# nv-tlabs/ASE

Measured on AMD Instinct MI355X. Metric: ASE PPO-update samples/sec (4096 envs x horizon 32), higher is better.
Workload: dtype f16; 1 GPU; BASELINE configs[1]: ASE agent, 4096 envs x horizon 32, obs 253 / act 31 / amp obs 1400 / latent 64, [1024,1024,512] MLPs + disc + shared-trunk encoder, minibatch 16384 (amp 4096) x 6 mini-epochs = 48 optimisation steps per update; random-init weights; precision_choice=auto without an oracle leg: the first candidate, replay=program, parallelism=single GPU

## Files before the change

### ase_amd/backend.py

```python
import ctypes as C

import torch

from . import lib as L


_HOSTFN = C.CFUNCTYPE(None, C.c_void_p)


def _ptr(t):
    return None if t is None else C.c_void_p(t.data_ptr())


def _ld(t):
    return 0 if t is None else int(t.stride(0))


def _code(dtype):
    if dtype == torch.bfloat16:
        return L.BF16
    if dtype == torch.float32:
        return L.F32
    if dtype == torch.float16:
        return L.F16
    raise L.AseHipError(f"unsupported storage dtype {dtype}")


class HipBackend:
    name = "hip"

    def __init__(self, device=None, x3=False):
        self.x3 = x3 if x3 == 'f16' else bool(x3)
        self._recording, self._host_keep, self._host_error = None, {}, None
        self.tn_workspace = True
        if not torch.cuda.is_available():
            raise L.AseHipError("HipBackend needs a ROCm GPU (torch.cuda.is_available() is False); "
                                "the update path has no CPU fallback")
        self.device = torch.device(device if device is not None else f"cuda:{torch.cuda.current_device()}")
        self.lib = L.get()
        self._head_scratch = torch.zeros(L.PPO_SCRATCH, dtype=torch.float64, device=self.device)
        self._head_scratch_ls = None

    def _stream(self):
        return C.c_void_p(torch.cuda.current_stream(self.device).cuda_stream)

    def zero_(self, t):
        assert t.is_contiguous()
        L.check(self.lib.ase_hip_memset(_ptr(t), 0, t.numel() * t.element_size(), self._stream()), "memset")

    def copy_(self, dst, src):
        assert dst.is_contiguous() and src.is_contiguous() and dst.dtype == src.dtype and dst.numel() == src.numel()
        L.check(self.lib.ase_hip_memcpy(_ptr(dst), _ptr(src), dst.numel() * dst.element_size(), self._stream()), "memcpy")

    def mark(self):
        ev = C.c_int(0)
        L.check(self.lib.ase_hip_mark(self._stream(), C.byref(ev)), "mark")
        return ev.value

    def wait(self, ev):
        L.check(self.lib.ase_hip_wait(self._stream(), int(ev)), "wait")

    def prog_create(self):
# ... 16 lines not shown
            return

        def trampoline(_arg, fn=fn):
            try:
                fn()
            except BaseException as e:
                self._host_error = e
        cb = _HOSTFN(trampoline)
        self._host_keep[self._recording].append(cb)
        L.check(self.lib.ase_hip_prog_host(C.cast(cb, C.c_void_p), None), "prog_host")

    def prog_launch(self, prog):
        L.check(self.lib.ase_hip_prog_launch(prog), "prog_launch")
        if self._host_error is not None:
            e, self._host_error = self._host_error, None
            raise e

    def prog_size(self, prog):
        return self.lib.ase_hip_prog_size(prog)

    def prog_destroy(self, prog):
        self.lib.ase_hip_prog_destroy(prog)
        self._host_keep.pop(prog.value, None)

    def _gemm_code(self, dtype, exps=None):
        c = _code(dtype)
        if self.x3 and c == L.F32:
            if self.x3 == 'f16' and exps is not None:
                return L.F32H3 | (int(exps[0]) << 8) | (int(exps[1]) << 16)
            return L.F32X3
        return c

    def gemm_nt(self, A, B, Cm, M, N, K, bias=None, aux=None, aux_mode=L.AUX_NONE, colsum=None, colsum_n=0,
                act=L.ACT_NONE, alpha=1.0, aux_split=0, aux_delta=0, mask_out=None, x3_exps=None, alpha_dev=None):
        dt = self._gemm_code(A.dtype, x3_exps)
        assert B.dtype == A.dtype
        if aux_mode == L.AUX_RELU_BITS:
            assert aux.dtype == torch.int32
        else:
            assert aux is None or aux.dtype == A.dtype
        assert mask_out is None or mask_out.dtype == (A.dtype if act >= L.ACT_SILU else torch.int32)
        out_f32 = int(Cm.dtype == torch.float32 and A.dtype != torch.float32)
        L.check(self.lib.ase_hip_gemm_nt(_ptr(A), _ld(A), _ptr(B), _ld(B), _ptr(Cm), _ld(Cm), _ptr(bias), _ptr(aux),
                                         _ld(aux), int(aux_split), int(aux_delta), _ptr(colsum), int(colsum_n),
                                         _ptr(mask_out), _ld(mask_out), M, N, K, act, aux_mode, out_f32,
                                         float(alpha), _ptr(alpha_dev), dt, self._stream()), "gemm_nt")

    def gemm_tn(self, A, B, G, M, N, K, n_real, k_real, split_src, split_dst, alpha=1.0, gbias=None, bias_rows=0, alpha_dev=None):
        L.check(self.lib.ase_hip_gemm_tn(_ptr(A), _ld(A), _ptr(B), _ld(B), _ptr(G), _ptr(gbias), int(bias_rows), M, N, K,
                                         n_real, k_real,
                                         split_src, split_dst, float(alpha), _ptr(alpha_dev), self._gemm_code(A.dtype), self._stream()),
                "gemm_tn")

    def grouped_tn_ok(self, dtype, M, n_real, K, bias_rows):
        return dtype in (torch.bfloat16, torch.float16) and M % 64 == 0 and bias_rows % 64 == 0

    def make_tn_plan(self, problems, target_wg=0, alpha_dev=None):
        import struct
        n = len(problems)
        tab = (C.c_int64 * (16 * n))()
        for i, (A, B, G, gb, br, M, N, K, nr, kr, ss, sd, alpha) in enumerate(problems):
            assert A.dtype in (torch.bfloat16, torch.float16) and B.dtype == A.dtype and G.dtype == torch.float32
            row = [A.data_ptr(), _ld(A), B.data_ptr(), _ld(B), G.data_ptr(), 0 if gb is None else gb.data_ptr(), int(br),
                   M, N, K, nr, kr, ss, sd, struct.unpack('<i', struct.pack('<f', float(alpha)))[0], 0]
            for j, v in enumerate(row):
                tab[16 * i + j] = int(v)
        max_work = 8192
        work = (C.c_int32 * (4 * max_work))()
        red = (C.c_int32 * (4 * max_work))()
        n_work, n_red = C.c_int(0), C.c_int(0)
        L.check(self.lib.ase_hip_gemm_tn_grouped_plan(tab, n, int(target_wg), work, max_work, C.byref(n_work), red, max_work,
                                                      C.byref(n_red)), "gemm_tn_grouped_plan")
        nw, nr = n_work.value, n_red.value
        dev_tab = torch.tensor(list(tab), dtype=torch.int64, device=self.device)
        dev_work = torch.tensor(list(work[:4 * nw]), dtype=torch.int32, device=self.device)
        dev_red = torch.tensor(list(red[:4 * nr]), dtype=torch.int32, device=self.device)
        ws = torch.empty(nw * L.TN_SLAB, dtype=torch.float32, device=self.device) if self.tn_workspace else None
        return {'problems': dev_tab, 'work': dev_work, 'n_work': nw, 'red': dev_red, 'n_red': nr, 'ws': ws, 'keep': problems,
                'dtype': _code(problems[0][0].dtype), 'alpha_dev': alpha_dev}

    def gemm_tn_grouped(self, plan):
        L.check(self.lib.ase_hip_gemm_tn_grouped(_ptr(plan['problems']), _ptr(plan['work']), plan['n_work'], _ptr(plan['red']),
                                                 plan['n_red'], _ptr(plan['ws']), _ptr(plan.get('alpha_dev')), plan['dtype'],
                                                 self._stream()),
                "gemm_tn_grouped")

    def refresh_shadow(self, W, Ws, Wts, split_src, split_dst, x3_exp=None):
        n, k = W.shape
        ref = Ws if Ws is not None else Wts
        code = _code(ref.dtype)
        if x3_exp is not None:
            assert ref.dtype == torch.float32
            code = L.F32H3 | (int(x3_exp) << 16)
        L.check(self.lib.ase_hip_refresh_shadow(_ptr(W), n, k, _ptr(Ws), _ld(Ws), _ptr(Wts), _ld(Wts), split_src,
                                                split_dst, code, self._stream()), "refresh_shadow")

    def refresh_shadow_multi(self, desc, items, dtype):
        L.check(self.lib.ase_hip_refresh_shadow_multi(_ptr(desc), desc.shape[0], _code(dtype), self._stream()),
                "refresh_shadow_multi")

    def apply_multi(self, desc, items, dtype, opt_state, acc):
        L.check(self.lib.ase_hip_apply_multi(_ptr(desc), desc.shape[0], _ptr(opt_state), _ptr(acc), _code(dtype),
                                             self._stream()), "apply_multi")

    def gather_multi(self, desc, items, idx, remap, M):
        L.check(self.lib.ase_hip_gather_multi(_ptr(desc), desc.shape[0], _ptr(idx), remap[0], remap[1], M,
                                              self._stream()), "gather_multi")

    def build_amp_obs(self, root_pos, root_rot, root_vel, root_ang_vel, dof_pos, dof_vel, key_body_pos, dof_offsets,
                      local_root_obs, root_height_obs, hist, shift=True):
        n, S, F = hist.shape
        offs = (C.c_int32 * len(dof_offsets))(*[int(x) for x in dof_offsets])
        for t in (root_pos, root_rot, root_vel, root_ang_vel, dof_pos, dof_vel, key_body_pos, hist):
            assert t.dtype == torch.float32 and t.is_contiguous()
        L.check(self.lib.ase_hip_build_amp_obs(_ptr(root_pos), _ptr(root_rot), _ptr(root_vel), _ptr(root_ang_vel), _ptr(dof_pos),
                                               _ptr(dof_vel), _ptr(key_body_pos), n, dof_pos.shape[1], key_body_pos.shape[1], offs,
                                               len(dof_offsets) - 1, int(local_root_obs), int(root_height_obs), _ptr(hist), S,
                                               int(shift), self._stream()), "build_amp_obs")

    def motion_state(self, clips, motion_ids, times):
        n, B = motion_ids.shape[0], clips['gts'].shape[1]
        D, J, K = clips['dof_offsets'][-1], len(clips['dof_body_ids']), len(clips['key_body_ids'])
        ia = lambda xs: (C.c_int32 * len(xs))(*[int(x) for x in xs])
        f = lambda *shape: torch.empty(*shape, dtype=torch.float32, device=self.device)
        out = (f(n, 3), f(n, 4), f(n, D), f(n, 3), f(n, 3), f(n, D), f(n, K, 3))
        assert motion_ids.dtype == torch.int32 and times.dtype == torch.float32
        L.check(self.lib.ase_hip_motion_state(_ptr(clips['gts']), _ptr(clips['grs']), _ptr(clips['lrs']), _ptr(clips['grvs']),
                                              _ptr(clips['gravs']), _ptr(clips['dvs']), B, _ptr(clips['lengths']),
                                              _ptr(clips['num_frames']), _ptr(clips['dt']), _ptr(clips['length_starts']),
                                              _ptr(motion_ids), _ptr(times), n, ia(clips['dof_body_ids']), ia(clips['dof_offsets']), J,
                                              ia(clips['key_body_ids']), K, *[_ptr(o) for o in out], self._stream()), "motion_state")
        return out

    def clip_frames(self, rotation, root_translation, root_velocity, root_angular_velocity, local_translation, parent_indices,
                    clip_first, clip_num_frames, clip_fps, frame_clip, dof_body_ids, dof_offsets, out=None):
        T, B = rotation.shape[0], rotation.shape[1]
# ... 116 lines not shown
                                           dof_pos.stride(1), _ptr(body_pos), _ptr(body_rot), _ptr(body_vel), _ptr(body_ang_vel), n,
                                           int(local_root_obs), int(root_height_obs), float(env_dt), _ptr(hist), S, self._stream()),
                "amp_reset")

    def rms_moments(self, src, D, idx, remap, M, state, sums):
        L.check(self.lib.ase_hip_rms_moments(_ptr(src), _ld(src), D, _ptr(idx), remap[0], remap[1], M, _ptr(state),
                                             _ptr(sums), self._stream()), "rms_moments")

    @staticmethod
    def _stream_arrays(streams):
        n = len(streams)
        srcs = (C.c_void_p * n)(*[s[0].data_ptr() for s in streams])
        lds = (C.c_int64 * n)(*[int(s[0].stride(0)) for s in streams])
        idxs = (C.c_void_p * n)(*[None if s[1] is None else s[1].data_ptr() for s in streams])
        rh = (C.c_int * n)(*[int(s[2][0]) for s in streams])
        rn = (C.c_int * n)(*[int(s[2][1]) for s in streams])
        return n, srcs, lds, idxs, rh, rn

    def rms_moments_multi(self, streams, D, M, state, sums_list):
        n, srcs, lds, idxs, rh, rn = self._stream_arrays(streams)
        sums = (C.c_void_p * n)(*[t.data_ptr() for t in sums_list])
        L.check(self.lib.ase_hip_rms_moments_multi(srcs, lds, idxs, rh, rn, sums, n, D, M, _ptr(state), self._stream()),
                "rms_moments_multi")

    def rms_normalize_multi(self, streams, D, M, means, stds, outs):
        n, srcs, lds, idxs, rh, rn = self._stream_arrays(streams)
        mp = (C.c_void_p * n)(*[t.data_ptr() for t in means])
        sp = (C.c_void_p * n)(*[t.data_ptr() for t in stds])
        op = (C.c_void_p * n)(*[t.data_ptr() for t in outs])
        lo = (C.c_int64 * n)(*[int(t.stride(0)) for t in outs])
        L.check(self.lib.ase_hip_rms_normalize_multi(srcs, lds, idxs, rh, rn, mp, sp, op, lo, n, D, M, _code(outs[0].dtype),
                                                     self._stream()), "rms_normalize_multi")

    def rms_finalize(self, state, D, sums, count, n_streams, mean_out, std_out):
        counts = (C.c_int32 * max(n_streams, 1))(*([int(count)] * max(n_streams, 1)))
        L.check(self.lib.ase_hip_rms_finalize(_ptr(state), D, _ptr(sums), counts, n_streams, _ptr(mean_out),
                                              _ptr(std_out), self._stream()), "rms_finalize")

    def rms_normalize(self, src, D, idx, remap, M, mean, std, outs):
        outs = list(outs) + [None] * (3 - len(outs))
        dt = _code(outs[0].dtype)
        L.check(self.lib.ase_hip_rms_normalize(_ptr(src), _ld(src), D, _ptr(idx), remap[0], remap[1], M, _ptr(mean),
                                               _ptr(std), _ptr(outs[0]), _ld(outs[0]), _ptr(outs[1]), _ld(outs[1]),
                                               _ptr(outs[2]), _ld(outs[2]), dt, self._stream()), "rms_normalize")

    def rms_unnormalize(self, state, x, y):
        L.check(self.lib.ase_hip_rms_unnormalize(_ptr(state), _ptr(x), _ptr(y), x.numel(), self._stream()),
                "rms_unnormalize")

    def gather_rows(self, src, D, idx, remap, M, dst):
        L.check(self.lib.ase_hip_gather_rows(_ptr(src), _ld(src), D, _ptr(idx), remap[0], remap[1], M, _ptr(dst),
                                             _ld(dst), _code(dst.dtype), self._stream()), "gather_rows")

    def reduce_sum(self, x, n, square, acc, slot):
        L.check(self.lib.ase_hip_reduce_sum(_ptr(x), n, int(square), _ptr(acc), slot, self._stream()), "reduce_sum")

    def ppo_head(self, mu, value, mb, new_z, logstd, d_mu, d_value, db_mu, db_value, acc, M, m_global, act_dim,
                 z_dim, masked, div_on, mu_tanh, clip_value, e_clip, critic_coef, bounds_coef, div_coef, div_tar,
                 mu_out=None, grad_scale=1.0, dyn=None, ls_mode=L.LS_FROZEN, d_logstd=None, db_logstd=None, entropy_coef=0.0):
        scratch = self._head_scratch if ls_mode == L.LS_FROZEN else self.reserve_learned_logstd()
        L.check(self.lib.ase_hip_ppo_head(
            _ptr(mu), _ld(mu), _ptr(value), _ld(value), _ptr(mb['actions']), _ptr(mb['mu']), _ptr(mb['sigma']),
            _ptr(mb['old_logp_actions']), _ptr(mb['advantages']), _ptr(mb.get('old_values')), _ptr(mb['returns']),
            _ptr(mb.get('rand_action_mask')), _ptr(mb.get('ase_latents')), _ptr(new_z), _ptr(logstd),
            _ptr(d_mu), _ld(d_mu), _ptr(d_value), _ld(d_value), _ptr(db_mu), _ptr(db_value), _ptr(mu_out), _ptr(acc),
            _ptr(scratch),
# ... 135 lines not shown
```

### ase_amd/csrc/common.h

```cpp
#pragma once
#include <hip/hip_runtime.h>
#include <hip/hip_bf16.h>
#include <stdint.h>
#include <stdio.h>
#include "../../include/ase_hip.h"
#include "prog.h"

typedef __bf16 bf16_t;
typedef __attribute__((ext_vector_type(8))) __bf16 bf16x8;
typedef __attribute__((ext_vector_type(4))) __bf16 bf16x4;
typedef _Float16 f16_t;
typedef __attribute__((ext_vector_type(8))) _Float16 f16x8;
typedef __attribute__((ext_vector_type(4))) _Float16 f16x4;
typedef __attribute__((ext_vector_type(16))) float f32x16;
typedef __attribute__((ext_vector_type(4))) float f32x4;

void ase_set_error(const char* fmt, ...);

#define ASE_CHECK_ARG(cond, ...)                 \
    do {                                         \
        if (!(cond)) {                           \
            ase_set_error(__VA_ARGS__);          \
            return ASE_EINVAL;                   \
        }                                        \
    } while (0)

#define ASE_CHECK_LAUNCH(name)                                              \
    do {                                                                    \
        hipError_t e__ = hipGetLastError();                                 \
        if (e__ != hipSuccess) {                                            \
            ase_set_error("%s: launch failed: %s", name, hipGetErrorString(e__)); \
            return ASE_ELAUNCH;                                             \
        }                                                                   \
    } while (0)

struct f32s_t { float v; };
struct f32h_t { float v; };

__device__ __forceinline__ float to_f32(float x) { return x; }
__device__ __forceinline__ float to_f32(bf16_t x) { return (float)x; }
__device__ __forceinline__ float to_f32(f32s_t x) { return x.v; }
__device__ __forceinline__ float to_f32(f32h_t x) { return x.v; }
__device__ __forceinline__ float to_f32(f16_t x) { return (float)x; }

template <typename T> __device__ __forceinline__ T from_f32(float x);
template <> __device__ __forceinline__ float from_f32<float>(float x) { return x; }
template <> __device__ __forceinline__ bf16_t from_f32<bf16_t>(float x) { return (bf16_t)x; }
template <> __device__ __forceinline__ f32s_t from_f32<f32s_t>(float x) { return f32s_t{x}; }
template <> __device__ __forceinline__ f32h_t from_f32<f32h_t>(float x) { return f32h_t{x}; }
template <> __device__ __forceinline__ f16_t from_f32<f16_t>(float x) { return (f16_t)__builtin_amdgcn_fmed3f(x, -65504.f, 65504.f); }

template <typename T> struct V16;
template <> struct V16<bf16_t> { typedef bf16x8 x8; typedef bf16x4 x4; };
template <> struct V16<f16_t> { typedef f16x8 x8; typedef f16x4 x4; };
template <> struct V16<float> { typedef bf16x8 x8; typedef bf16x4 x4; };
template <typename T> __device__ __forceinline__ f32x16 mfma16(typename V16<T>::x8 a, typename V16<T>::x8 b, f32x16 c);
template <> __device__ __forceinline__ f32x16 mfma16<bf16_t>(bf16x8 a, bf16x8 b, f32x16 c) {
    return __builtin_amdgcn_mfma_f32_32x32x16_bf16(a, b, c, 0, 0, 0);
}
template <> __device__ __forceinline__ f32x16 mfma16<f16_t>(f16x8 a, f16x8 b, f32x16 c) {
    return __builtin_amdgcn_mfma_f32_32x32x16_f16(a, b, c, 0, 0, 0);
}

template <typename T> struct StorageTag { typedef T type; };
template <typename F> inline int ase_dispatch_storage(int dtype, F&& f) {
    switch (dtype) {
        case ASE_F32: return f(StorageTag<float>{});
        case ASE_BF16: return f(StorageTag<bf16_t>{});
        case ASE_F16: return f(StorageTag<f16_t>{});
        default: return ASE_EUNSUPPORTED;
    }
}
inline int ase_elem_size(int dtype) { return (dtype == ASE_BF16 || dtype == ASE_F16) ? 2 : 4; }

__device__ __forceinline__ int64_t map_row(int r, const int32_t* __restrict__ idx, int remap_h, int remap_n) {
    uint32_t p = idx ? (uint32_t)idx[r] : (uint32_t)r;
    if (remap_h > 0) {
        const uint32_t env = p / (uint32_t)remap_h;
        const uint32_t t = p - env * (uint32_t)remap_h;
        p = t * (uint32_t)remap_n + env;
    }
    return (int64_t)p;
}
// ... 51 lines not shown
```

### ase_amd/csrc/gemm.hip

```cpp
#include "gemm_nt.h"
#include <math.h>

namespace ase_nt {

unsigned long long* g_nt_prof = nullptr;
int g_nt_prof_clk = 0;

int nt_choice(int M, int N, int K, int es, bool b16) {
    if (N <= 64) return 0;
    const int t256 = ((M + 255) / 256) * ((N + 255) / 256);
    const bool big = N % 256 == 0 && t256 >= 192 && (t256 <= 256 || t256 % 256 == 0 || t256 >= 1024);
    if (big) {
        if (!(b16 && (K * es) % 128 == 0)) return 3;
        const int t192 = ((M + 191) / 192) * (N / 256);
        return (t256 < 256 && t192 <= 256 && t192 > t256) ? 6 : 2;
    }
    if ((K * es) % 128 != 0) return 1;
    const int t128 = ((M + 127) / 128) * ((N + 127) / 128), t64x128 = ((M + 63) / 64) * ((N + 127) / 128);
    if (t128 >= 512) return 1;
    if (t64x128 >= 512) return 4;
    return 5;
}

}

using namespace ase_nt;

extern "C" int ase_hip_debug_nt_profile(void* buf) {
    g_nt_prof = reinterpret_cast<unsigned long long*>(buf);
    return ASE_OK;
}

extern "C" int ase_hip_debug_nt_profile_clock(int shader_clock) {
    g_nt_prof_clk = shader_clock ? 1 : 0;
    return ASE_OK;
}

extern "C" int ase_hip_gemm_nt_kernel_id(int M, int N, int K, int dtype) {
    dtype &= 0xFF;
    return nt_choice(M, N, K, ase_elem_size(dtype), ase_elem_size(dtype) == 2);
}

extern "C" int ase_hip_gemm_nt(const void* A, int64_t lda, const void* B, int64_t ldb, void* C, int64_t ldc,
                               const float* bias, const void* aux, int64_t ldaux, int aux_split, int aux_delta,
                               float* colsum, int colsum_n, void* mask_out, int64_t ldmask, int M, int N, int K, int act,
                               int aux_mode, int out_f32, float alpha, float* alpha_dev, int dtype_word, void* stream) {
    const int dtype = dtype_word & 0xFF, ea = (dtype_word >> 8) & 0xFF, eb = (dtype_word >> 16) & 0xFF;
    const int es = ase_elem_size(dtype);
    ASE_CHECK_ARG(dtype == ASE_F32 || dtype == ASE_BF16 || dtype == ASE_F32X3 || dtype == ASE_F16 || dtype == ASE_F32H3,
                  "gemm_nt: bad dtype %d", dtype);
    ASE_CHECK_ARG(ea >= 0 && ea <= 24 && eb >= 0 && eb <= 24 && (dtype == ASE_F32H3 || (ea | eb) == 0),
                  "gemm_nt: operand scale exponents (bits 8-15 / 16-23 of dtype) are 0..24 and belong to ASE_F32H3 only");
    ASE_CHECK_ARG(A && B && C && M > 0 && N > 0 && K > 0, "gemm_nt: null/empty operand (M=%d N=%d K=%d)", M, N, K);
    ASE_CHECK_ARG((K * es) % 64 == 0, "gemm_nt: K=%d is not a multiple of %d elements", K, 64 / es);
    ASE_CHECK_ARG(lda >= K && ldb >= K && ldc >= N, "gemm_nt: leading dimension too small");
    ASE_CHECK_ARG(((uintptr_t)A % 16) == 0 && ((uintptr_t)B % 16) == 0 && (lda * es) % 16 == 0 && (ldb * es) % 16 == 0,
                  "gemm_nt: A/B must be 16-byte aligned with 16-byte row pitch");
    ASE_CHECK_ARG(aux_mode == ASE_AUX_NONE || aux != nullptr, "gemm_nt: aux_mode %d without aux", aux_mode);
    const bool bits = aux_mode == ASE_AUX_RELU_BITS;
    ASE_CHECK_ARG(N % 4 == 0 && ((uintptr_t)C % 16) == 0 && (ldc * (out_f32 ? 4 : es)) % 8 == 0 &&
                      (aux == nullptr || bits || (((uintptr_t)aux % 8) == 0 && (ldaux * es) % 8 == 0)),
                  "gemm_nt: C / aux must allow 8/16-byte row-vector access (N %% 4 == 0, aligned pitches)");
    ASE_CHECK_ARG(!bits || (((uintptr_t)aux % 4) == 0 && ldaux * 32 >= N), "gemm_nt: bit mask needs ldaux >= N / 32 words");
    const bool smooth = act >= ASE_ACT_SILU;
    ASE_CHECK_ARG(act >= ASE_ACT_NONE && act <= ASE_ACT_SOFTPLUS, "gemm_nt: unknown activation %d", act);
    ASE_CHECK_ARG((aux_mode & 0xFF) <= ASE_AUX_PREACT && ((aux_mode & 0xFF) == ASE_AUX_PREACT || (aux_mode >> 8) == 0) &&
                      (aux_mode >> 8) <= ASE_ACT_SOFTPLUS, "gemm_nt: bad aux_mode 0x%x", aux_mode);
    ASE_CHECK_ARG(mask_out == nullptr || smooth || (N % 32 == 0 && ((uintptr_t)mask_out % 4) == 0 && ldmask * 32 >= N),
                  "gemm_nt: mask_out needs N %% 32 == 0 and ldmask >= N / 32 words");
    ASE_CHECK_ARG(mask_out == nullptr || !smooth || (ldmask >= N && ((uintptr_t)mask_out % 16) == 0 && (ldmask * es) % 8 == 0),
                  "gemm_nt: the pre-activation twin needs ldmask >= N elements, 16-byte alignment");
    NTParams p;
    p.A = (const char*)A; p.lda = lda * es;
    p.B = (const char*)B; p.ldb = ldb * es;
    p.C = (char*)C; p.ldc = ldc * (out_f32 ? 4 : es);
    p.mask_out = smooth ? nullptr : (uint32_t*)mask_out; p.ldmask = ldmask;
    p.pre_out = smooth ? (char*)mask_out : nullptr; p.ldpre = ldmask * es;
    p.bias = bias; p.aux = (const char*)aux; p.ldaux = bits ? ldaux * 4 : ldaux * es; p.aux_split = aux_split > 0 ? aux_split : M; p.aux_delta = aux_delta; p.colsum = colsum; p.colsum_n = colsum ? colsum_n : 0;
    p.M = M; p.N = N; p.K = K; p.act = act; p.aux_mode = aux_mode; p.out_f32 = out_f32; p.alpha = alpha; p.alpha_dev = alpha_dev;
    p.tiles_m = p.tiles_n = 0;
    p.prof = nullptr;
    p.prof_clk = 0;
    p.sa = 1.f;
    if (dtype == ASE_BF16) return dispatch_nt_bf16(p, (hipStream_t)stream);
    if (dtype == ASE_F16) return dispatch_nt_f16(p, (hipStream_t)stream);
    if (dtype == ASE_F32X3) return dispatch_nt_x3(p, (hipStream_t)stream);
    if (dtype == ASE_F32H3) {
        p.sa = ldexpf(1.f, ea);
        p.alpha = ldexpf(alpha, -(ea + eb));
        return dispatch_nt_h3(p, (hipStream_t)stream);
    }
    return dispatch_nt_f32(p, (hipStream_t)stream);
}
```

### ase_amd/csrc/gemm_nt.h

```cpp
#pragma once
#include "common.h"
#include "act.h"
#include <type_traits>

namespace ase_nt {


__device__ __forceinline__ int xcd_remap(int bid, int nwg) {
    const int q = nwg >> 3, r = nwg & 7, xcd = bid & 7, loc = bid >> 3;
    const int base = (xcd < r) ? xcd * (q + 1) : r * (q + 1) + (xcd - r) * q;
    return base + loc;
}


template <int RB> __device__ __forceinline__ int lds_swz(int r) { return RB == 128 ? ((r >> 1) & 7) : ((r >> 2) & 3); }

typedef __attribute__((address_space(1))) const void gptr_t;
typedef __attribute__((address_space(3))) void lptr_t;

template <int N> __device__ __forceinline__ void wait_vmcnt() { asm volatile("s_waitcnt vmcnt(%0)" ::"n"(N) : "memory"); }

struct NTParams {
    const char* A; int64_t lda;
    const char* B; int64_t ldb;
    char* C; int64_t ldc;
    const float* bias;
    const char* aux; int64_t ldaux;
    int aux_split, aux_delta;
    float* colsum; int colsum_n;
    uint32_t* mask_out; int64_t ldmask;
    char* pre_out; int64_t ldpre;
    int M, N, K;
    int act, aux_mode, out_f32;
    float alpha;
    float* alpha_dev;
    float sa;
    int tiles_m, tiles_n;
    unsigned long long* prof;
    int prof_clk;
};


typedef __attribute__((ext_vector_type(4))) int i32x4;

template <typename T, bool SW>
__device__ __forceinline__ f32x16 nt8_mfma(const i32x4& a, const i32x4& b, const f32x16& c) {
    typedef typename V16<T>::x8 x8;
    if constexpr (SW) return mfma16<T>(__builtin_bit_cast(x8, b), __builtin_bit_cast(x8, a), c);
    else return mfma16<T>(__builtin_bit_cast(x8, a), __builtin_bit_cast(x8, b), c);
}


#define NT8_BARRIER()                        \
    do {                                     \
        __builtin_amdgcn_sched_barrier(0);   \
        __builtin_amdgcn_s_barrier();        \
        __builtin_amdgcn_sched_barrier(0);   \
    } while (0)


typedef float f32x2 __attribute__((ext_vector_type(2)));
typedef short i16x2 __attribute__((ext_vector_type(2)));
typedef int i32x2 __attribute__((ext_vector_type(2)));
typedef unsigned short u16x2 __attribute__((ext_vector_type(2)));
typedef __bf16 bf16x2 __attribute__((ext_vector_type(2)));
typedef _Float16 f16x2 __attribute__((ext_vector_type(2)));

template <typename T> __device__ __forceinline__ uint32_t cvt_pk16(f32x2 v);
template <> __device__ __forceinline__ uint32_t cvt_pk16<bf16_t>(f32x2 v) {
    return __builtin_bit_cast(uint32_t, __builtin_convertvector(v, bf16x2));
}
template <> __device__ __forceinline__ uint32_t cvt_pk16<f16_t>(f32x2 v) {
// ... 136 lines not shown
```

### ase_amd/csrc/gemm_nt_kernels.h

```cpp
#pragma once
#include "gemm_nt.h"
#include <stdlib.h>

namespace {

using namespace ase_nt;

template <typename T> struct Mma;

template <typename T> struct Mma16 {
    typedef typename V16<T>::x8 x8;
    template <int FM, int FN, int RB, bool SW = false>
    static __device__ __forceinline__ void tile(const char* sA, const char* sB, int lane, f32x16 (&acc)[FM][FN]) {
        const int r = lane & 31, h = lane >> 5, sw = lds_swz<RB>(r);
#pragma unroll
        for (int ks = 0; ks < RB / 32; ++ks) {
            x8 a[FM], b[FN];
            const int off = r * RB + (((ks * 2 + h) ^ sw) << 4);
#pragma unroll
            for (int i = 0; i < FM; ++i)
                a[i] = *reinterpret_cast<const x8*>(sA + i * 32 * RB + off);
#pragma unroll
            for (int j = 0; j < FN; ++j)
                b[j] = *reinterpret_cast<const x8*>(sB + j * 32 * RB + off);
// ... 129 lines not shown
template <> struct AuxReg<f32s_t, 1> { f32x4 v; };
template <> struct AuxReg<f32h_t, 1> { f32x4 v; };
template <typename T> struct AuxReg<T, 2> { uint32_t v; };

__device__ __forceinline__ uint32_t or8_dpp(uint32_t x) {
    x |= (uint32_t)__builtin_amdgcn_update_dpp(0, (int)x, 0xB1, 0xF, 0xF, true);
    x |= (uint32_t)__builtin_amdgcn_update_dpp(0, (int)x, 0x4E, 0xF, 0xF, true);
    x |= (uint32_t)__builtin_amdgcn_update_dpp(0, (int)x, 0x141, 0xF, 0xF, true);
    return x;
}

template <typename T, int FM, int FN, int FMC, int FNC, int AUXK>
__device__ __forceinline__ void nt_aux_load(const NTParams& p, int ch, int lane, int mrow0, int ncol0,
                                            AuxReg<T, AUXK> (&dst)[(FMC * 32) / (64 / (FNC * 8))]) {
    constexpr int ELPR = FNC * 8, RPI = 64 / ELPR, NIT = (FMC * 32) / RPI;
    if constexpr (AUXK != 0) {
        const int c4 = lane % ELPR, rsub = lane / ELPR;
        const int jc = (ch / (FM / FMC)) * FNC, ic = (ch % (FM / FMC)) * FMC;
        const int n0 = ncol0 + jc * 32 + c4 * 4;
#pragma unroll
        for (int it = 0; it < NIT; ++it) {
            const int m = mrow0 + ic * 32 + it * RPI + rsub;
            if (n0 < p.N && m < p.M) {
                const int ma = (m >= p.aux_split) ? m - p.aux_delta : m;
                if constexpr (AUXK == 2)
                    dst[it].v = *reinterpret_cast<const uint32_t*>(p.aux + (int64_t)ma * p.ldaux + (n0 >> 5) * 4);
                else
                    dst[it].v = *reinterpret_cast<const decltype(dst[it].v)*>(p.aux + (int64_t)ma * p.ldaux + (int64_t)n0 * sizeof(T));
            }
        }
    }
}

template <typename T, int FM, int FN, int FMC, int FNC, int AUXK, bool PRE = false>
__device__ __forceinline__ void nt_epilogue_impl(const NTParams& p, f32x16 (&acc)[FM][FN], float* slab, int lane,
                                                 int mrow0, int ncol0,
                                                 AuxReg<T, AUXK> (*pre)[(FMC * 32) / (64 / (FNC * 8))] = nullptr) {
    constexpr int WCOLS = FNC * 32, WROWS = FMC * 32;
    const int col_in = lane & 31, row_hi = (lane >> 5) * 4;
    constexpr int ELPR = WCOLS / 4;
    constexpr int RPI = 64 / ELPR;
    constexpr int NIT = WROWS / RPI;
    constexpr int NCH = (FN / FNC) * (FM / FMC);
    constexpr bool AHEAD = AUXK != 0 && sizeof(AuxReg<T, AUXK>) <= 8;
    const int c4 = lane % ELPR, rsub = lane / ELPR;
    AuxReg<T, AUXK> areg[AHEAD ? 2 : 1][NIT];
    bool bad = false;

    auto load_aux = [&](int ch, AuxReg<T, AUXK> (&dst)[NIT]) {
        nt_aux_load<T, FM, FN, FMC, FNC, AUXK>(p, ch, lane, mrow0, ncol0, dst);
    };

    if constexpr (PRE) {
#pragma unroll
        for (int it = 0; it < NIT; ++it) areg[0][it] = (*pre)[it];
    } else if constexpr (AUXK != 0) {
        load_aux(0, areg[0]);
    }
#pragma unroll
    for (int ch = 0; ch < NCH; ++ch) {
        const int jc = (ch / (FM / FMC)) * FNC, ic = (ch % (FM / FMC)) * FMC;
        const int n0 = ncol0 + jc * 32 + c4 * 4;
        if constexpr (AHEAD) {
            if (ch + 1 < NCH) load_aux(ch + 1, areg[(ch + 1) & 1]);
        } else if constexpr (AUXK != 0) {
            if (ch > 0) load_aux(ch, areg[0]);
        }
        AuxReg<T, AUXK> (&cur)[NIT] = areg[AHEAD ? (ch & 1) : 0];
#pragma unroll
        for (int jj = 0; jj < FNC; ++jj) {
            const int j = jc + jj;
            const int n = ncol0 + j * 32 + col_in;
            const float bias = (p.bias && n < p.N) ? p.bias[n] : 0.f;
#pragma unroll
            for (int ii = 0; ii < FMC; ++ii) {
#pragma unroll
                for (int e = 0; e < 16; ++e) {
                    float v = p.alpha * acc[ic + ii][j][e] + bias;
                    if (p.act == ASE_ACT_RELU) v = fmaxf(v, 0.f);
                    else if (p.act == ASE_ACT_TANH) v = tanhf(v);
                    slab[(ii * 32 + row_hi + (e & 3) + 8 * (e >> 2)) * WCOLS + jj * 32 + col_in] = v;
                }
            }
        }
        float cs[4] = {0.f, 0.f, 0.f, 0.f};
        if (n0 < p.N) {
#pragma unroll
            for (int it = 0; it < NIT; ++it) {
                const int row = it * RPI + rsub;
                const int m = mrow0 + ic * 32 + row;
                if (m >= p.M) continue;
                f32x4 v = *reinterpret_cast<const f32x4*>(slab + row * WCOLS + c4 * 4);
                if (p.act >= ASE_ACT_SILU) {
                    if (p.pre_out) {
                        if constexpr (sizeof(T) == 2) {
                            typename V16<T>::x4 zt;
#pragma unroll
                            for (int q = 0; q < 4; ++q) {
                                zt[q] = from_f32<T>(v[q]);
                                bad |= ovf_hit1(zt[q]);
                            }
                            *reinterpret_cast<typename V16<T>::x4*>(p.pre_out + (int64_t)m * p.ldpre + (int64_t)n0 * 2) = zt;
                        } else {
#pragma unroll
                            for (int q = 0; q < 4; ++q) bad |= ovf_hit1(v[q]);
                            *reinterpret_cast<f32x4*>(p.pre_out + (int64_t)m * p.ldpre + (int64_t)n0 * 4) = v;
                        }
                    }
#pragma unroll
                    for (int q = 0; q < 4; ++q) v[q] = act_apply(p.act, v[q]);
                }
                if constexpr (AUXK == 2) {
                    const uint32_t nib = cur[it].v >> (n0 & 31);
#pragma unroll
                    for (int q = 0; q < 4; ++q) v[q] = ((nib >> q) & 1u) ? v[q] : 0.f;
                } else if constexpr (AUXK == 1) {
#pragma unroll
                    for (int q = 0; q < 4; ++q) {
                        const float a = (float)cur[it].v[q];
                        if (p.aux_mode == ASE_AUX_RELU_MASK) v[q] = a > 0.f ? v[q] : 0.f;
                        else if (p.aux_mode == ASE_AUX_TANH_GRAD) v[q] = v[q] * (1.f - a * a);
                        else v[q] = v[q] * act_grad(p.aux_mode >> 8, a);
                    }
                }
                if (p.out_f32 || sizeof(T) == 4) {
#pragma unroll
                    for (int q = 0; q < 4; ++q) bad |= ovf_hit1(v[q]);
                    *reinterpret_cast<f32x4*>(p.C + (int64_t)m * p.ldc + (int64_t)n0 * 4) = v;
                } else {
                    typedef typename std::conditional<sizeof(T) == 2, T, bf16_t>::type S;
                    typename V16<S>::x4 o;
#pragma unroll
                    for (int q = 0; q < 4; ++q) {
                        o[q] = from_f32<S>(v[q]);
                        bad |= ovf_hit1(o[q]);
                        v[q] = (float)o[q];
                    }
                    *reinterpret_cast<typename V16<S>::x4*>(p.C + (int64_t)m * p.ldc + (int64_t)n0 * 2) = o;
                }
#pragma unroll
                for (int q = 0; q < 4; ++q) cs[q] += v[q];
                if (p.mask_out) {
                    uint32_t bits = 0;
#pragma unroll
                    for (int q = 0; q < 4; ++q) bits |= (v[q] > 0.f ? 1u : 0u) << q;
                    bits = or8_dpp(bits << (n0 & 31));
                    if ((c4 & 7) == 0) p.mask_out[(int64_t)m * p.ldmask + (n0 >> 5)] = bits;
                }
            }
        }
        if (p.colsum) {
#pragma unroll
            for (int q = 0; q < 4; ++q) {
#pragma unroll
                for (int o = ELPR; o < 64; o <<= 1) cs[q] += __shfl_xor(cs[q], o, 64);
            }
            if (lane < ELPR) {
#pragma unroll
                for (int q = 0; q < 4; ++q)
                    if (n0 + q < p.colsum_n) atomic_add_f32(p.colsum + n0 + q, cs[q]);
            }
        }
    }
    ovf_report(p.alpha_dev, bad);
}

template <typename T, int FM, int FN, int FMC, int FNC>
__device__ __forceinline__ void nt_epilogue(const NTParams& p, f32x16 (&acc)[FM][FN], float* slab, int lane, int mrow0,
                                            int ncol0) {
    if (p.aux_mode == ASE_AUX_NONE) nt_epilogue_impl<T, FM, FN, FMC, FNC, 0>(p, acc, slab, lane, mrow0, ncol0);
    else if (p.aux_mode == ASE_AUX_RELU_BITS) nt_epilogue_impl<T, FM, FN, FMC, FNC, 2>(p, acc, slab, lane, mrow0, ncol0);
    else nt_epilogue_impl<T, FM, FN, FMC, FNC, 1>(p, acc, slab, lane, mrow0, ncol0);
}

template <typename T, int FM, int FN, int AUXK, bool MASK>
__device__ __forceinline__ void nt_epilogue_rows_impl(const NTParams& p, f32x16 (&acc)[FM][FN], int lane, int mrow0, int ncol0,
                                                      const uint32_t (&bits)[FM][FN]) {
    const int r = lane & 31, h = lane >> 5;
    const f32x2 al = {p.alpha, p.alpha};
    const short lo = (p.act == ASE_ACT_RELU) ? (short)0 : (short)-32768;
    const i16x2 relu_lo = {lo, lo};
    uint32_t ovf = 0;
#pragma unroll
    for (int j = 0; j < FN; ++j) {
        f32x4 bias[4];
#pragma unroll
        for (int g = 0; g < 4; ++g) {
            if (p.bias) bias[g] = *reinterpret_cast<const f32x4*>(p.bias + ncol0 + j * 32 + 8 * g + 4 * h);
            else bias[g] = f32x4{0.f, 0.f, 0.f, 0.f};
        }
#pragma unroll
        for (int i = 0; i < FM; ++i) {
            const int m = mrow0 + i * 32 + r;
            const bool row_ok = m < p.M;
            char* crow = p.C + (int64_t)m * p.ldc + (int64_t)(ncol0 + j * 32) * 2 + h * 16;
            uint32_t pk[4][2];
            const uint32_t mb = rows_frag<T, AUXK, MASK>(acc[i][j], bias, AUXK == 2 ? bits[i][j] >> (4 * h) : 0u, al, relu_lo, h, pk);
#pragma unroll
            for (int g = 0; g < 4; g += 2) {
                const auto s0 = __builtin_amdgcn_permlane32_swap(pk[g][0], pk[g + 1][0], false, false);
                const auto s1 = __builtin_amdgcn_permlane32_swap(pk[g][1], pk[g + 1][1], false, false);
                if (row_ok) *reinterpret_cast<uint4*>(crow + 8 * g * 2) = make_uint4(s0[0], s1[0], s0[1], s1[1]);
                ovf = ovf_fold(ovf_fold(ovf_fold(ovf_fold(ovf, s0[0]), s1[0]), s0[1]), s1[1]);
            }
            if constexpr (MASK) {
                const auto w = __builtin_amdgcn_permlane32_swap(mb, mb, false, false);
                if (row_ok && h == 0) p.mask_out[(int64_t)m * p.ldmask + ((ncol0 + j * 32) >> 5)] = w[0] | w[1];
            }
        }
    }
    ovf_report(p.alpha_dev, ovf_hit<T>(ovf));
}

template <typename T, int FM, int FN, int AUXK>
__device__ __forceinline__ void nt_epilogue_rows(const NTParams& p, f32x16 (&acc)[FM][FN], int lane, int mrow0, int ncol0,
                                                 const uint32_t (&bits)[FM][FN]) {
    if (ncol0 >= p.N) return;
    if (p.mask_out) nt_epilogue_rows_impl<T, FM, FN, AUXK, true>(p, acc, lane, mrow0, ncol0, bits);
    else nt_epilogue_rows_impl<T, FM, FN, AUXK, false>(p, acc, lane, mrow0, ncol0, bits);
}

template <typename T, int WGM, int WGN, int FM, int FN, int RB, int S, int WPE = 1, bool SW = false>
__global__ __launch_bounds__(WGM * WGN * 64, WPE) void gemm_nt_kernel(NTParams p) {
    constexpr int BM = WGM * FM * 32, BN = WGN * FN * 32;
    constexpr int BK = RB / (int)sizeof(T);
    constexpr int LPR = RB / 16;
    constexpr int RPW = 64 / LPR;
    constexpr int RPP = WGM * WGN * RPW;
    constexpr int A_PASSES = BM / RPP, B_PASSES = BN / RPP;
    constexpr int P = A_PASSES + B_PASSES;
    static_assert(BM % RPP == 0 && BN % RPP == 0, "tile rows must be a multiple of the rows staged per pass");
    extern __shared__ __attribute__((aligned(16))) char smem[];
    constexpr int kBuf = (BM + BN) * RB;
    if (p.alpha_dev) p.alpha *= *p.alpha_dev;

    const int tid = threadIdx.x, lane = tid & 63, wid = tid >> 6;
    const int wm = wid / WGN, wn = wid % WGN;
    const int nwg = p.tiles_m * p.tiles_n;
    const int tile = xcd_remap(blockIdx.x, nwg);
    const int bm0 = (tile / p.tiles_n) * BM, bn0 = (tile % p.tiles_n) * BN;

    const int srow = tid / LPR, sslot = tid % LPR;
    const char* srcA[A_PASSES];
    const char* srcB[B_PASSES];
#pragma unroll
    for (int i = 0; i < A_PASSES; ++i) {
        const int r = i * RPP + srow;
        srcA[i] = p.A + (int64_t)min(bm0 + r, p.M - 1) * p.lda + ((sslot ^ lds_swz<RB>(r)) << 4);
    }
#pragma unroll
    for (int i = 0; i < B_PASSES; ++i) {
        const int r = i * RPP + srow;
        srcB[i] = p.B + (int64_t)min(bn0 + r, p.N - 1) * p.ldb + ((sslot ^ lds_swz<RB>(r)) << 4);
    }
    char* const ldsA = smem + (wid * RPW) * RB;
// ... 29 lines not shown
            nt_stage<A_PASSES, RPP, RB>(srcA, (int64_t)t * RB, ldsA + t * kBuf);
            nt_stage<B_PASSES, RPP, RB>(srcB, (int64_t)t * RB, ldsB + t * kBuf);
        }
    }
    int buf = 0;
    for (int kt = 0; kt < nk; ++kt) {
        if (kt + S - 2 < nk) wait_vmcnt<P*(S - 2)>();
        else wait_vmcnt<0>();
        __builtin_amdgcn_s_barrier();
        if (kt + S - 1 < nk) {
            const int nb = (buf == 0) ? S - 1 : buf - 1;
            nt_stage<A_PASSES, RPP, RB>(srcA, (int64_t)(kt + S - 1) * RB, ldsA + nb * kBuf);
            nt_stage<B_PASSES, RPP, RB>(srcB, (int64_t)(kt + S - 1) * RB, ldsB + nb * kBuf);
        }
        const char* sA = smem + buf * kBuf + (wm * FM * 32) * RB;
        const char* sB = smem + buf * kBuf + (BM + wn * FN * 32) * RB;
        if constexpr (SW && sizeof(T) == 2) Mma<T>::template tile<FM, FN, RB, true>(sA, sB, lane, acc);
        else if constexpr (std::is_same<T, f32h_t>::value) Mma<T>::template tile<FM, FN, RB>(sA, sB, lane, acc, p.sa);
        else Mma<T>::template tile<FM, FN, RB>(sA, sB, lane, acc);
        buf = (buf + 1 == S) ? 0 : buf + 1;
    }
    if constexpr (SW) {
        if constexpr (S != 2) load_bits();
        if constexpr (sizeof(T) == 2) {
            if (p.aux_mode == ASE_AUX_RELU_BITS) nt_epilogue_rows<T, FM, FN, 2>(p, acc, lane, bm0 + wm * FM * 32, bn0 + wn * FN * 32, row_bits);
            else nt_epilogue_rows<T, FM, FN, 0>(p, acc, lane, bm0 + wm * FM * 32, bn0 + wn * FN * 32, row_bits);
        }
        return;
    }
    __syncthreads();

    constexpr int FNC = (FN > 2) ? 2 : FN;
    float* slab = reinterpret_cast<float*>(smem) + wid * (FM * 32 * FNC * 32);
    nt_epilogue<T, FM, FN, FM, FNC>(p, acc, slab, lane, bm0 + wm * FM * 32, bn0 + wn * FN * 32);
}

template <typename T, int WGM, int WGN, int FM, int FN, int RB, int S, int WPE = 1, bool SW = false>
int launch_nt(const NTParams& p0, hipStream_t stream) {
    constexpr int BM = WGM * FM * 32, BN = WGN * FN * 32;
    constexpr int ring = S * (BM + BN) * RB;
    constexpr int slab = WGM * WGN * (FM * 32) * ((FN > 2 ? 2 : FN) * 32) * 4;
    constexpr int lds = ring > slab ? ring : slab;
    static_assert(lds <= 160 * 1024, "LDS budget");
    static bool attr_done = false;
    auto kern = gemm_nt_kernel<T, WGM, WGN, FM, FN, RB, S, WPE, SW>;
    if (!attr_done) {
        hipError_t e = hipFuncSetAttribute(reinterpret_cast<const void*>(kern),
                                           hipFuncAttributeMaxDynamicSharedMemorySize, lds);
        if (e != hipSuccess) {
            ase_set_error("gemm_nt: hipFuncSetAttribute failed: %s", hipGetErrorString(e));
            return ASE_ELAUNCH;
        }
        attr_done = true;
    }
    NTParams p = p0;
    p.tiles_m = (p.M + BM - 1) / BM;
    p.tiles_n = (p.N + BN - 1) / BN;
    ASE_LAUNCH(kern, dim3(p.tiles_m * p.tiles_n), dim3(WGM * WGN * 64), lds, stream, p);
    ASE_CHECK_LAUNCH("gemm_nt");
    return ASE_OK;
}


struct NT8Lane {
    uint32_t voff[4][2];
    uint32_t dst[4][2];
    int roff[4];
    i32x4 rsA, rsB;
};

__device__ __forceinline__ void nt8_dma(uint32_t lds_s, uint32_t voff, i32x4 rs, uint32_t soff) {
    asm volatile("s_mov_b32 m0, %0\n\tbuffer_load_dwordx4 %1, %2, %3 offen lds" : : "s"(lds_s), "v"(voff), "s"(rs), "s"(soff) : "memory");
}
template <int KIND>
__device__ __forceinline__ void nt8_piece(const NT8Lane& L, int g, int tile) {
    constexpr bool isB = (KIND == 1 || KIND == 2);
    nt8_dma(__builtin_amdgcn_readfirstlane(L.dst[KIND][g] + (uint32_t)(tile & 1) * 65536u), L.voff[KIND][g], isB ? L.rsB : L.rsA,
            (uint32_t)tile * 128u);
// ... 215 lines not shown
    if (!attr_done) {
        hipError_t e = hipFuncSetAttribute(reinterpret_cast<const void*>(kern),
                                           hipFuncAttributeMaxDynamicSharedMemorySize, lds);
        if (e != hipSuccess) {
            ase_set_error("gemm_nt8: hipFuncSetAttribute failed: %s", hipGetErrorString(e));
            return ASE_ELAUNCH;
        }
        attr_done = true;
    }
    NTParams p = p0;
    p.prof = g_nt_prof;
    p.prof_clk = g_nt_prof_clk;
    p.tiles_m = (p.M + BM - 1) / BM;
    p.tiles_n = (p.N + 255) / 256;
    ASE_LAUNCH(kern, dim3(p.tiles_m * p.tiles_n), dim3(512), lds, stream, p);
    ASE_CHECK_LAUNCH("gemm_nt8");
    return ASE_OK;
}

}
#include "gemm_nt4.h"
namespace {

inline bool rows_epi(const NTParams& p, int wave_cols) {
    return !p.out_f32 && p.N % wave_cols == 0 && p.colsum == nullptr && p.act <= ASE_ACT_RELU &&
           (p.aux_mode == ASE_AUX_NONE || p.aux_mode == ASE_AUX_RELU_BITS);
}

template <typename T> int dispatch_nt(const NTParams& p, hipStream_t s) {
    const bool k128 = (p.K * (int)sizeof(T)) % 128 == 0;
    const bool fits32 = (int64_t)p.M * p.lda < (int64_t)0x7FFFFFFF && (int64_t)p.N * p.ldb < (int64_t)0x7FFFFFFF;
    int choice = nt_choice(p.M, p.N, p.K, (int)sizeof(T), sizeof(T) == 2);
    if ((choice == 2 || choice == 6) && !fits32) choice = 3;
    switch (choice) {
        case 0: return launch_nt<T, 2, 2, 1, 1, 64, 4>(p, s);
        case 6:
            if constexpr (sizeof(T) == 2) if (rows_epi(p, 64)) return launch_nt8<T, true, 192>(p, s);
            [[fallthrough]];
        case 2:
            if constexpr (sizeof(T) == 2) {
                if (p.M >= 65536 && rows_epi(p, 128)) return launch_nt4<T>(p, s);
                if (rows_epi(p, 64)) return launch_nt8<T, true>(p, s);
                return launch_nt8<T, false>(p, s);
            }
            [[fallthrough]];
        case 3:
            if (k128) return launch_nt<T, 4, 2, 2, 4, 128, 2>(p, s);
            return launch_nt<T, 4, 2, 2, 4, 64, 4>(p, s);
        case 4:
            if constexpr (sizeof(T) == 2) if (rows_epi(p, 64)) return launch_nt<T, 2, 2, 1, 2, 128, 2, 2, true>(p, s);
            return launch_nt<T, 2, 2, 1, 2, 128, 2, 2>(p, s);
        case 5:
            if constexpr (sizeof(T) == 2) if (rows_epi(p, 32)) return launch_nt<T, 2, 2, 1, 1, 128, 4, 2, true>(p, s);
            return launch_nt<T, 2, 2, 1, 1, 128, 4, 2>(p, s);
        default:
            if constexpr (sizeof(T) == 2) if (k128 && rows_epi(p, 64)) return launch_nt<T, 2, 2, 2, 2, 128, 2, 1, true>(p, s);
            if (k128) return launch_nt<T, 2, 2, 2, 2, 128, 2>(p, s);
            return launch_nt<T, 2, 2, 2, 2, 64, 4>(p, s);
    }
}

}
```

### ase_amd/csrc/gemm_tn.hip

```cpp
#include "gemm_nt.h"
#include <stdlib.h>
#include <math.h>
#include <algorithm>
#include <vector>

using namespace ase_nt;

namespace {

constexpr int kThreads = 256;

__device__ __forceinline__ void split_bf16(const f32x4& x0, const f32x4& x1, bf16x8& hi, bf16x8& lo) {
#pragma unroll
    for (int q = 0; q < 4; ++q) {
        hi[q] = (bf16_t)x0[q];
        hi[q + 4] = (bf16_t)x1[q];
        lo[q] = (bf16_t)(x0[q] - (float)hi[q]);
        lo[q + 4] = (bf16_t)(x1[q] - (float)hi[q + 4]);
    }
}

struct TNParams {
    const char* A; int64_t lda;
    const char* B; int64_t ldb;
// ... 660 lines not shown
    return ASE_OK;
}

template <typename T>
__global__ void refresh_shadow_kernel(const float* __restrict__ W, int n_real, int k_real, T* __restrict__ Ws,
                                      int64_t ldws, T* __restrict__ Wts, int64_t ldwts, int split_src, int gap) {
    __shared__ float tile[32][33];
    const int k0 = blockIdx.x * 32, n0 = blockIdx.y * 32;
    const int tx = threadIdx.x & 31, ty = threadIdx.x >> 5;
#pragma unroll
    for (int i = 0; i < 4; ++i) {
        const int n = n0 + ty + 8 * i, k = k0 + tx;
        float v = 0.f;
        if (n < n_real && k < k_real) v = W[(int64_t)n * k_real + k];
        tile[ty + 8 * i][tx] = v;
        if (Ws && n < n_real && k < k_real) {
            const int kd = (k < split_src) ? k : k + gap;
            Ws[(int64_t)n * ldws + kd] = from_f32<T>(v);
        }
    }
    __syncthreads();
    if (Wts) {
#pragma unroll
        for (int i = 0; i < 4; ++i) {
            const int k = k0 + ty + 8 * i, n = n0 + tx;
            if (k < k_real && n < n_real) {
                const int kd = (k < split_src) ? k : k + gap;
                Wts[(int64_t)kd * ldwts + n] = from_f32<T>(tile[tx][ty + 8 * i]);
            }
        }
    }
}

__device__ __forceinline__ void store_split(char* row, int col, float v, float scale) {
    const float s = __builtin_amdgcn_fmed3f(v * scale, -65504.f, 65504.f);
    const f16_t hi = (f16_t)s, lo = (f16_t)(s - (float)hi);
    char* g = row + (col >> 3) * 32 + (col & 7) * 2;
    *reinterpret_cast<f16_t*>(g) = hi;
    *reinterpret_cast<f16_t*>(g + 16) = lo;
}
__global__ void refresh_shadow_split_kernel(const float* __restrict__ W, int n_real, int k_real, char* __restrict__ Ws, int64_t ldws,
                                            char* __restrict__ Wts, int64_t ldwts, int split_src, int gap, float scale) {
    __shared__ float tile[32][33];
    const int k0 = blockIdx.x * 32, n0 = blockIdx.y * 32;
    const int tx = threadIdx.x & 31, ty = threadIdx.x >> 5;
#pragma unroll
    for (int i = 0; i < 4; ++i) {
        const int n = n0 + ty + 8 * i, k = k0 + tx;
        float v = 0.f;
        if (n < n_real && k < k_real) v = W[(int64_t)n * k_real + k];
        tile[ty + 8 * i][tx] = v;
        if (Ws && n < n_real && k < k_real) store_split(Ws + (int64_t)n * ldws * 4, (k < split_src) ? k : k + gap, v, scale);
    }
    __syncthreads();
    if (Wts) {
#pragma unroll
        for (int i = 0; i < 4; ++i) {
            const int k = k0 + ty + 8 * i, n = n0 + tx;
            if (k < k_real && n < n_real)
                store_split(Wts + (int64_t)((k < split_src) ? k : k + gap) * ldwts * 4, n, tile[tx][ty + 8 * i], scale);
        }
    }
}

template <typename T>
__global__ __launch_bounds__(256) void refresh_multi_kernel(const int64_t* __restrict__ desc) {
    __shared__ float tile[32][33];
    const int64_t* d = desc + 12 * blockIdx.y;
    const float* W = reinterpret_cast<const float*>(d[0]);
    const int n_real = (int)d[1], k_real = (int)d[2];
    T* Ws = reinterpret_cast<T*>(d[3]);
    const int64_t ldws = d[4];
    T* Wts = reinterpret_cast<T*>(d[5]);
// ... 243 lines not shown
```

### ase_amd/csrc/optim.hip

```cpp
#include "common.h"

namespace {

__global__ void begin_step_kernel(double* __restrict__ opt_state, double* __restrict__ acc, int n_acc,
                                  double* __restrict__ zero2, int n_zero2, unsigned long long* __restrict__ rng_bump) {
    for (int i = threadIdx.x; i < n_acc; i += blockDim.x) acc[i] = 0.0;
    for (int i = threadIdx.x; i < n_zero2; i += blockDim.x) zero2[i] = 0.0;
    if (threadIdx.x == 0 && rng_bump) rng_bump[1] += 1;
    if (threadIdx.x == 0 && opt_state) {
        const double step = opt_state[0] + 1.0;
        opt_state[0] = step;
        opt_state[5] = 1.0 - pow(opt_state[2], step);
        opt_state[6] = 1.0 - pow(opt_state[3], step);
    }
}

__global__ __launch_bounds__(256) void adam_kernel(float* __restrict__ w, const float* __restrict__ g,
                                                   float* __restrict__ m, float* __restrict__ v, int64_t n,
                                                   const double* __restrict__ st) {
    const float one_m_b1 = (float)(1.0 - st[2]);
    const float b2 = (float)st[3], one_m_b2 = (float)(1.0 - st[3]);
    const float eps = (float)st[4];
    const float step_size = (float)(st[1] / st[5]);
    const float bc2_sqrt = (float)sqrt(st[6]);
    for (int64_t i = blockIdx.x * (int64_t)blockDim.x + threadIdx.x; i < n; i += (int64_t)gridDim.x * blockDim.x) {
        const float gi = g[i];
        float mi = m[i], vi = v[i];
        mi = mi + one_m_b1 * (gi - mi);
        vi = vi * b2;
        vi = vi + one_m_b2 * (gi * gi);
        const float denom = sqrtf(vi) / bc2_sqrt + eps;
        w[i] = w[i] - step_size * (mi / denom);
        m[i] = mi;
// ... 4 lines not shown
__global__ __launch_bounds__(256) void axpy_kernel(float* __restrict__ g, const float* __restrict__ w, int64_t n, float c) {
    for (int64_t i = blockIdx.x * (int64_t)blockDim.x + threadIdx.x; i < n; i += (int64_t)gridDim.x * blockDim.x)
        g[i] = g[i] + c * w[i];
}

__device__ __forceinline__ float adam_elem(float w, float gi, float& mi, float& vi, float one_m_b1, float b2,
                                           float one_m_b2, float eps, float step_size, float bc2_sqrt) {
    mi = mi + one_m_b1 * (gi - mi);
    vi = vi * b2;
    vi = vi + one_m_b2 * (gi * gi);
    const float denom = sqrtf(vi) / bc2_sqrt + eps;
    return w - step_size * (mi / denom);
}

typedef float f4u __attribute__((ext_vector_type(4), aligned(4)));

template <typename T> __device__ __forceinline__ void store_shadow4(T* p, const float (&w)[4]);
template <> __device__ __forceinline__ void store_shadow4<bf16_t>(bf16_t* p, const float (&w)[4]) {
    bf16x4 v;
#pragma unroll
    for (int c = 0; c < 4; ++c) v[c] = (bf16_t)w[c];
    *reinterpret_cast<bf16x4*>(p) = v;
}
template <> __device__ __forceinline__ void store_shadow4<f16_t>(f16_t* p, const float (&w)[4]) {
    f16x4 v;
#pragma unroll
    for (int c = 0; c < 4; ++c) v[c] = from_f32<f16_t>(w[c]);
    *reinterpret_cast<f16x4*>(p) = v;
}
template <> __device__ __forceinline__ void store_shadow4<float>(float* p, const float (&w)[4]) {
    *reinterpret_cast<f32x4*>(p) = f32x4{w[0], w[1], w[2], w[3]};
}

template <typename T>
__global__ __launch_bounds__(256) void apply_multi_kernel(const int64_t* __restrict__ desc, const double* __restrict__ st,
                                                          double* __restrict__ acc) {
    __shared__ float tile[32][129];
    __shared__ double red[16];
    const int64_t* d = desc + 24 * blockIdx.y;
    float* W = reinterpret_cast<float*>(d[0]);
    const int n_real = (int)d[1], k_real = (int)d[2];
    T* Ws = reinterpret_cast<T*>(d[3]);
    const int64_t ldws = d[4];
    T* Wts = reinterpret_cast<T*>(d[5]);
    const int64_t ldwts = d[6];
    const int split_src = (int)d[7], gap = (int)d[8];
    const int tiles_k = (int)d[11];
    float* gW = reinterpret_cast<float*>(d[12]);
    float* mW = reinterpret_cast<float*>(d[13]);
    float* vW = reinterpret_cast<float*>(d[14]);
    const float wd = __builtin_bit_cast(float, (int)d[18]);
    const int slot_a = (int)d[19], slot_b = (int)d[20];
    const bool adam = st != nullptr;
    float one_m_b1 = 0.f, b2 = 0.f, one_m_b2 = 0.f, eps = 0.f, step_size = 0.f, bc2_sqrt = 1.f;
    if (adam) {
        one_m_b1 = (float)(1.0 - st[2]); b2 = (float)st[3]; one_m_b2 = (float)(1.0 - st[3]);
        eps = (float)st[4]; step_size = (float)(st[1] / st[5]); bc2_sqrt = (float)sqrt(st[6]);
    }
    const int tiles = tiles_k * ((n_real + 31) / 32);
    const int tx = threadIdx.x & 31, ty = threadIdx.x >> 5;
    if (blockIdx.x == 0 && d[9]) {
        float* b = reinterpret_cast<float*>(d[9]);
        float* bs = reinterpret_cast<float*>(d[10]);
        float* gb = reinterpret_cast<float*>(d[15]);
        float* mb = reinterpret_cast<float*>(d[16]);
        float* vb = reinterpret_cast<float*>(d[17]);
        for (int i = threadIdx.x; i < n_real; i += 256) {
            float w = b[i];
            if (adam) {
                float mi = mb[i], vi = vb[i];
                w = adam_elem(w, gb[i], mi, vi, one_m_b1, b2, one_m_b2, eps, step_size, bc2_sqrt);
                b[i] = w; mb[i] = mi; vb[i] = vi;
// ... 31 lines not shown
                            *reinterpret_cast<f4u*>(gW + o) = gv;
                        }
                        f4u wn;
#pragma unroll
                        for (int c = 0; c < 4; ++c) {
                            float mi = mv[c], vi = vv[c];
                            w[c] = adam_elem(w[c], gv[c], mi, vi, one_m_b1, b2, one_m_b2, eps, step_size, bc2_sqrt);
                            mv[c] = mi; vv[c] = vi; wn[c] = w[c];
                        }
                        *reinterpret_cast<f4u*>(W + o) = wn;
                        *reinterpret_cast<f4u*>(mW + o) = mv;
                        *reinterpret_cast<f4u*>(vW + o) = vv;
                    }
                    store_shadow4<T>(Ws + (int64_t)n * ldws + ((k < split_src) ? k : k + gap), w);
                }
#pragma unroll
                for (int c = 0; c < 4; ++c) tile[vy + 8 * i][4 * vx + c] = w[c];
            }
            __syncthreads();
            const int kk = threadIdx.x >> 1, half = threadIdx.x & 1;
            const int k = k0 + kk, nb = n0 + 16 * half;
            if (k < k_real && nb < n_real) {
                T* dst = Wts + (int64_t)((k < split_src) ? k : k + gap) * ldwts + nb;
                if (nb + 16 <= n_real) {
#pragma unroll
                    for (int q = 0; q < 16; q += 4) {
                        const float w4[4] = {tile[16 * half + q][kk], tile[16 * half + q + 1][kk], tile[16 * half + q + 2][kk],
                                             tile[16 * half + q + 3][kk]};
                        store_shadow4<T>(dst + q, w4);
                    }
                } else {
                    for (int q = 0; q < 16 && nb + q < n_real; ++q) dst[q] = from_f32<T>(tile[16 * half + q][kk]);
                }
            }
        }
    } else
    for (int t = blockIdx.x; t < tiles; t += gridDim.x) {
        const int k0 = (t % tiles_k) * 32, n0 = (t / tiles_k) * 32;
        __syncthreads();
#pragma unroll
        for (int i = 0; i < 4; ++i) {
            const int n = n0 + ty + 8 * i, k = k0 + tx;
            float w = 0.f;
            if (n < n_real && k < k_real) {
                const int64_t o = (int64_t)n * k_real + k;
                w = W[o];
                if (adam) {
                    if (slot_a >= 0) w2[0] += (double)w * (double)w;
                    float gi = gW[o];
                    if (wd != 0.f) {
                        gi = gi + wd * w;
                        gW[o] = gi;
                    }
                    float mi = mW[o], vi = vW[o];
                    w = adam_elem(w, gi, mi, vi, one_m_b1, b2, one_m_b2, eps, step_size, bc2_sqrt);
                    W[o] = w; mW[o] = mi; vW[o] = vi;
                }
                Ws[(int64_t)n * ldws + ((k < split_src) ? k : k + gap)] = from_f32<T>(w);
            }
            tile[ty + 8 * i][tx] = w;
        }
        __syncthreads();
#pragma unroll
        for (int i = 0; i < 4; ++i) {
            const int k = k0 + ty + 8 * i, n = n0 + tx;
            if (k < k_real && n < n_real)
                Wts[(int64_t)((k < split_src) ? k : k + gap) * ldwts + n] = from_f32<T>(tile[tx][ty + 8 * i]);
        }
    }
    if (adam && slot_a >= 0) {
        __syncthreads();
        block_sum<1>(w2, red);
        if (threadIdx.x == 0 && w2[0] != 0.0) {
            atomic_add_f64(acc + slot_a, w2[0]);
            if (slot_b >= 0) atomic_add_f64(acc + slot_b, w2[0]);
        }
    }
}

inline int grid_for(int64_t n) {
    int64_t g = (n + 255) / 256;
    return (int)(g < 1 ? 1 : (g > 4096 ? 4096 : g));
}

__global__ __launch_bounds__(256) void clip_scale_kernel(float* __restrict__ g, int64_t n, const double* __restrict__ sqnorm,
                                                         float max_norm) {
    const float total = (float)sqrt(*sqnorm);
    const float coef = fminf(max_norm / (total + 1e-6f), 1.0f);
    for (int64_t i = blockIdx.x * (int64_t)blockDim.x + threadIdx.x; i < n; i += (int64_t)gridDim.x * blockDim.x) g[i] *= coef;
}

}

extern "C" int ase_hip_clip_scale(float* g, int64_t n, const double* sqnorm, float max_norm, void* stream) {
    ASE_CHECK_ARG(g && sqnorm && n > 0 && max_norm > 0.f, "clip_scale: bad operand");
    ASE_LAUNCH(clip_scale_kernel, dim3(grid_for(n)), dim3(256), 0, (hipStream_t)stream, g, n, sqnorm, max_norm);
    ASE_CHECK_LAUNCH("clip_scale");
    return ASE_OK;
}

extern "C" int ase_hip_begin_step(double* opt_state, double* acc, int n_acc, double* zero2, int n_zero2,
                                  uint64_t* rng_bump, void* stream) {
    ASE_CHECK_ARG((opt_state || acc || zero2 || rng_bump) && n_acc >= 0 && n_zero2 >= 0, "begin_step: nothing to do");
    ASE_LAUNCH(begin_step_kernel, dim3(1), dim3(1024), 0, (hipStream_t)stream, opt_state, acc, acc ? n_acc : 0, zero2,
                       zero2 ? n_zero2 : 0, (unsigned long long*)rng_bump);
    ASE_CHECK_LAUNCH("begin_step");
    return ASE_OK;
}

extern "C" int ase_hip_adam(float* w, const float* g, float* m, float* v, int64_t n, const double* opt_state,
                            void* stream) {
    ASE_CHECK_ARG(w && g && m && v && opt_state && n > 0, "adam: null/empty operand");
    ASE_LAUNCH(adam_kernel, dim3(grid_for(n)), dim3(256), 0, (hipStream_t)stream, w, g, m, v, n, opt_state);
    ASE_CHECK_LAUNCH("adam");
    return ASE_OK;
}

extern "C" int ase_hip_axpy(float* g, const float* w, int64_t n, float c, void* stream) {
    ASE_CHECK_ARG(g && w && n > 0, "axpy: null/empty operand");
    ASE_LAUNCH(axpy_kernel, dim3(grid_for(n)), dim3(256), 0, (hipStream_t)stream, g, w, n, c);
    ASE_CHECK_LAUNCH("axpy");
    return ASE_OK;
}

extern "C" int ase_hip_apply_multi(const int64_t* desc, int n_layers, const double* opt_state, double* acc, int dtype,
                                   void* stream) {
    ASE_CHECK_ARG(desc && n_layers > 0, "apply_multi: null/empty operand");
    ASE_CHECK_ARG(opt_state == nullptr || acc != nullptr, "apply_multi: optimizer step without the accumulator array");
    const dim3 grid(256, n_layers);
    const int rc = ase_dispatch_storage(dtype, [&](auto tag) {
        typedef typename decltype(tag)::type T;
        ASE_LAUNCH(apply_multi_kernel<T>, grid, dim3(256), 0, (hipStream_t)stream, desc, opt_state, acc);
        return ASE_OK;
    });
    ASE_CHECK_ARG(rc == ASE_OK, "apply_multi: bad dtype %d", dtype);
    ASE_CHECK_LAUNCH("apply_multi");
    return ASE_OK;
}
```

### ase_amd/csrc/rms.hip

```cpp
#include "common.h"

namespace {

constexpr int kRowsPerBlock = 64;

__global__ __launch_bounds__(256) void rms_moments4_kernel(const float* __restrict__ src, int64_t ld_src, int D,
                                                           const int32_t* __restrict__ idx, int remap_h, int remap_n,
                                                           int M, const double* __restrict__ state,
                                                           double* __restrict__ sums) {
    __shared__ double red[3][8][64];
    const int tx = threadIdx.x & 63, ty = threadIdx.x >> 6;
    const int j = (blockIdx.x * 64 + tx) * 4;
    const int r0 = blockIdx.y * kRowsPerBlock;
    const int r1 = min(M, r0 + kRowsPerBlock);
    double s1[4] = {0, 0, 0, 0}, s2[4] = {0, 0, 0, 0};
    if (j < D) {
        float shift[4];
#pragma unroll
        for (int c = 0; c < 4; ++c) shift[c] = (float)state[j + c];
        for (int r = r0 + ty; r < r1; r += 16) {
            f32x4 x[4];
#pragma unroll
            for (int q = 0; q < 4; ++q) {
                const int rr = r + 4 * q;
// ... 6 lines not shown
#pragma unroll
            for (int q = 0; q < 4; ++q)
#pragma unroll
                for (int c = 0; c < 4; ++c) {
                    const double d = (double)(x[q][c] - shift[c]);
                    s1[c] += d;
                    s2[c] += d * d;
                }
        }
    }
    if (ty > 0) {
#pragma unroll
        for (int c = 0; c < 4; ++c) {
            red[ty - 1][c][tx] = s1[c];
            red[ty - 1][4 + c][tx] = s2[c];
        }
    }
    __syncthreads();
    if (ty == 0 && j < D) {
#pragma unroll
        for (int c = 0; c < 4; ++c) {
            const double a = ((s1[c] + red[0][c][tx]) + red[1][c][tx]) + red[2][c][tx];
            const double b = ((s2[c] + red[0][4 + c][tx]) + red[1][4 + c][tx]) + red[2][4 + c][tx];
            atomic_add_f64(sums + j + c, a);
            atomic_add_f64(sums + D + j + c, b);
        }
    }
}

struct RmsStreams {
    const float* src[4]; int64_t ld[4]; const int32_t* idx[4]; int rh[4], rn[4];
    double* sums[4];
    const float* mean[4]; const float* stdv[4]; void* out[4]; int64_t ld_out[4];
};

__global__ __launch_bounds__(256) void rms_moments_multi_kernel(RmsStreams S, int D, int M, const double* __restrict__ state) {
    __shared__ double red[2][4][64];
    const int s = blockIdx.z;
    const float* __restrict__ src = S.src[s];
    const int32_t* __restrict__ idx = S.idx[s];
    const int64_t ld_src = S.ld[s];
    const int tx = threadIdx.x & 63, ty = threadIdx.x >> 6;
    const int j = blockIdx.x * 64 + tx;
    const int r0 = blockIdx.y * kRowsPerBlock;
    const int r1 = min(M, r0 + kRowsPerBlock);
    double s1 = 0.0, s2 = 0.0;
    if (j < D) {
        const float shift = (float)state[j];
        int64_t p[16];
        float x[16];
#pragma unroll
        for (int q = 0; q < 16; ++q) {
            const int rr = r0 + ty + 4 * q;
            p[q] = (rr < r1) ? map_row(rr, idx, S.rh[s], S.rn[s]) : -1;
        }
#pragma unroll
        for (int q = 0; q < 16; ++q) x[q] = (p[q] >= 0) ? src[p[q] * ld_src + j] : shift;
#pragma unroll
        for (int q = 0; q < 16; ++q) {
            const double d = (double)(x[q] - shift);
            s1 += d;
            s2 += d * d;
        }
    }
    red[0][ty][tx] = s1;
    red[1][ty][tx] = s2;
    __syncthreads();
    if (ty == 0 && j < D) {
        s1 = red[0][0][tx] + red[0][1][tx] + red[0][2][tx] + red[0][3][tx];
        s2 = red[1][0][tx] + red[1][1][tx] + red[1][2][tx] + red[1][3][tx];
        atomic_add_f64(S.sums[s] + j, s1);
        atomic_add_f64(S.sums[s] + D + j, s2);
    }
}

template <typename T>
__global__ __launch_bounds__(256) void rms_normalize_multi_kernel(RmsStreams S, int D, int M) {
    const int s = blockIdx.z;
    const int tx = threadIdx.x & 63, ty = threadIdx.x >> 6;
    const int r = blockIdx.y * 4 + ty;
    const int j = (blockIdx.x * 64 + tx) * 4;
    if (r >= M || j >= D) return;
    const int64_t p = map_row(r, S.idx[s], S.rh[s], S.rn[s]);
    const f32x4 x = *reinterpret_cast<const f32x4*>(S.src[s] + p * S.ld[s] + j);
    const f32x4 mu = *reinterpret_cast<const f32x4*>(S.mean[s] + j), sd = *reinterpret_cast<const f32x4*>(S.stdv[s] + j);
    f32x4 y;
#pragma unroll
    for (int c = 0; c < 4; ++c) y[c] = fminf(fmaxf((x[c] - mu[c]) / sd[c], -5.f), 5.f);
    if constexpr (sizeof(T) == 2) {
        typename V16<T>::x4 v;
#pragma unroll
        for (int c = 0; c < 4; ++c) v[c] = from_f32<T>(y[c]);
        *reinterpret_cast<typename V16<T>::x4*>(reinterpret_cast<T*>(S.out[s]) + (int64_t)r * S.ld_out[s] + j) = v;
    } else {
        *reinterpret_cast<f32x4*>(reinterpret_cast<float*>(S.out[s]) + (int64_t)r * S.ld_out[s] + j) = y;
    }
}

__global__ __launch_bounds__(1024) void rms_finalize_kernel(double* __restrict__ state, int D,
                                                           const double* __restrict__ sums, int count,
                                                           int n_streams, float* __restrict__ mean_out,
                                                           float* __restrict__ std_out) {
    const double count0 = state[2 * D];
    __syncthreads();
    for (int j = threadIdx.x; j < D; j += blockDim.x) {
        double mean = state[j], var = state[D + j], cnt = count0;
        const float shift = (float)mean;
        if (n_streams == 0) {
            mean_out[j] = (float)mean;
            std_out[j] = sqrtf((float)var + 1e-5f);
        }
        for (int s = 0; s < n_streams; ++s) {
            const double n = (double)count;
            const double s1 = sums[(int64_t)s * 2 * D + j], s2 = sums[(int64_t)s * 2 * D + D + j];
            const double bm = (double)(float)((double)shift + s1 / n);
            const double bv = (double)(float)((s2 - s1 * s1 / n) / (n - 1.0));
            const double delta = bm - mean;
            const double tot = cnt + n;
            const double new_mean = mean + delta * n / tot;
            const double m2 = var * cnt + bv * n + delta * delta * cnt * n / tot;
            mean = new_mean;
// ... 160 lines not shown
extern "C" int ase_hip_rms_moments(const float* src, int64_t ld_src, int D, const int32_t* idx, int remap_h,
                                   int remap_n, int M, const double* state, double* sums, void* stream) {
    ASE_CHECK_ARG(src && state && sums && D > 0 && M > 0, "rms_moments: null/empty operand");
    if (idx == nullptr && D % 4 == 0 && ld_src % 4 == 0 && ((uintptr_t)src % 16) == 0) {
        const dim3 grid((D / 4 + 63) / 64, (M + kRowsPerBlock - 1) / kRowsPerBlock);
        ASE_LAUNCH(rms_moments4_kernel, grid, dim3(256), 0, (hipStream_t)stream, src, ld_src, D, idx, remap_h,
                           remap_n, M, state, sums);
    } else {
        RmsStreams S = {};
        S.src[0] = src; S.ld[0] = ld_src; S.idx[0] = idx; S.rh[0] = remap_h; S.rn[0] = remap_n; S.sums[0] = sums;
        const dim3 grid((D + 63) / 64, (M + kRowsPerBlock - 1) / kRowsPerBlock, 1);
        ASE_LAUNCH(rms_moments_multi_kernel, grid, dim3(256), 0, (hipStream_t)stream, S, D, M, state);
    }
    ASE_CHECK_LAUNCH("rms_moments");
    return ASE_OK;
}

extern "C" int ase_hip_rms_moments_multi(const float* const* srcs, const int64_t* ld_srcs, const int32_t* const* idxs,
                                         const int* remap_h, const int* remap_n, double* const* sums, int n_streams, int D,
                                         int M, const double* state, void* stream) {
    ASE_CHECK_ARG(srcs && ld_srcs && idxs && remap_h && remap_n && sums && state && n_streams >= 1 && n_streams <= 4 && D > 0 && M > 0,
                  "rms_moments_multi: null/empty operand (1..4 streams)");
    RmsStreams S = {};
    for (int s = 0; s < n_streams; ++s) {
        ASE_CHECK_ARG(srcs[s] && sums[s], "rms_moments_multi: stream %d: null operand", s);
        S.src[s] = srcs[s]; S.ld[s] = ld_srcs[s]; S.idx[s] = idxs[s]; S.rh[s] = remap_h[s]; S.rn[s] = remap_n[s]; S.sums[s] = sums[s];
    }
    const dim3 grid((D + 63) / 64, (M + kRowsPerBlock - 1) / kRowsPerBlock, n_streams);
    ASE_LAUNCH(rms_moments_multi_kernel, grid, dim3(256), 0, (hipStream_t)stream, S, D, M, state);
    ASE_CHECK_LAUNCH("rms_moments_multi");
    return ASE_OK;
}

extern "C" int ase_hip_rms_normalize_multi(const float* const* srcs, const int64_t* ld_srcs, const int32_t* const* idxs,
                                           const int* remap_h, const int* remap_n, const float* const* means,
                                           const float* const* stds, void* const* outs, const int64_t* ld_outs, int n_streams,
                                           int D, int M, int dtype, void* stream) {
    ASE_CHECK_ARG(srcs && ld_srcs && idxs && remap_h && remap_n && means && stds && outs && ld_outs && n_streams >= 1 &&
                      n_streams <= 4 && D > 0 && M > 0, "rms_normalize_multi: null/empty operand (1..4 streams)");
    ASE_CHECK_ARG(dtype == ASE_BF16 || dtype == ASE_F32 || dtype == ASE_F16, "rms_normalize_multi: bad dtype %d", dtype);
    const int es = ase_elem_size(dtype);
    RmsStreams S = {};
    for (int s = 0; s < n_streams; ++s) {
        ASE_CHECK_ARG(srcs[s] && means[s] && stds[s] && outs[s], "rms_normalize_multi: stream %d: null operand", s);
        ASE_CHECK_ARG(D % 4 == 0 && ld_srcs[s] % 4 == 0 && ((uintptr_t)srcs[s] % 16) == 0 && ((uintptr_t)means[s] % 16) == 0 &&
                          ((uintptr_t)stds[s] % 16) == 0 && ld_outs[s] % 4 == 0 && ((uintptr_t)outs[s] % (4 * es)) == 0,
                      "rms_normalize_multi: stream %d needs 16-byte rows (D %% 4 == 0, aligned pointers / pitches)", s);
        S.src[s] = srcs[s]; S.ld[s] = ld_srcs[s]; S.idx[s] = idxs[s]; S.rh[s] = remap_h[s]; S.rn[s] = remap_n[s];
        S.mean[s] = means[s]; S.stdv[s] = stds[s]; S.out[s] = outs[s]; S.ld_out[s] = ld_outs[s];
    }
    const dim3 grid((D / 4 + 63) / 64, (M + 3) / 4, n_streams);
    ase_dispatch_storage(dtype, [&](auto tag) {
        typedef typename decltype(tag)::type T;
        ASE_LAUNCH(rms_normalize_multi_kernel<T>, grid, dim3(256), 0, (hipStream_t)stream, S, D, M);
        return ASE_OK;
    });
    ASE_CHECK_LAUNCH("rms_normalize_multi");
    return ASE_OK;
}

extern "C" int ase_hip_rms_finalize(double* state, int D, const double* sums, const int32_t* counts, int n_streams,
                                    float* mean_out, float* std_out, void* stream) {
    ASE_CHECK_ARG(state && mean_out && std_out && D > 0 && n_streams >= 0, "rms_finalize: null/empty operand");
    int count = 0;
    if (n_streams > 0) {
        ASE_CHECK_ARG(sums && counts, "rms_finalize: sums/counts missing");
        count = counts[0];
        for (int s = 1; s < n_streams; ++s)
            ASE_CHECK_ARG(counts[s] == count, "rms_finalize: all streams of one call must have the same row count");
        ASE_CHECK_ARG(count > 1, "rms_finalize: need at least 2 rows for an unbiased variance");
    }
    ASE_LAUNCH(rms_finalize_kernel, dim3(1), dim3(D > 256 ? 1024 : 256), 0, (hipStream_t)stream, state, D, sums, count,
                       n_streams, mean_out, std_out);
    ASE_CHECK_LAUNCH("rms_finalize");
    return ASE_OK;
}

extern "C" int ase_hip_rms_normalize(const float* src, int64_t ld_src, int D, const int32_t* idx, int remap_h,
                                     int remap_n, int M, const float* mean, const float* stdv, void* out0,
                                     int64_t ld0, void* out1, int64_t ld1, void* out2, int64_t ld2, int dtype,
                                     void* stream) {
    ASE_CHECK_ARG(src && mean && stdv && out0 && D > 0 && M > 0, "rms_normalize: null/empty operand");
    const int es = ase_elem_size(dtype);
    auto ok = [&](void* o, int64_t ld) { return o == nullptr || (ld % 4 == 0 && ((uintptr_t)o % (4 * es)) == 0); };
    const bool wide = D % 4 == 0 && ld_src % 4 == 0 && ((uintptr_t)src % 16) == 0 && ((uintptr_t)mean % 16) == 0 &&
                      ((uintptr_t)stdv % 16) == 0 && ok(out0, ld0) && ok(out1, ld1) && ok(out2, ld2);
    const dim3 g4((D / 4 + 63) / 64, (M + 3) / 4), grid((D + 255) / 256, (M + 3) / 4);
    const int rc = ase_dispatch_storage(dtype, [&](auto tag) {
        typedef typename decltype(tag)::type T;
        if (wide)
            ASE_LAUNCH(rms_normalize4_kernel<T>, g4, dim3(256), 0, (hipStream_t)stream, src, ld_src, D, idx, remap_h, remap_n, M, mean,
// ... 36 lines not shown
```

### ase_amd/engine.py

```python
import math

import torch

from . import lib as L


def P(x, m=64):
    return (int(x) + m - 1) // m * m


_ACT = {'relu': L.ACT_RELU, 'tanh': L.ACT_TANH, 'None': L.ACT_NONE, 'none': L.ACT_NONE, None: L.ACT_NONE,
        'swish': L.ACT_SILU, 'silu': L.ACT_SILU, 'elu': L.ACT_ELU, 'gelu': L.ACT_GELU, 'sigmoid': L.ACT_SIGMOID,
        'selu': L.ACT_SELU, 'softplus': L.ACT_SOFTPLUS}
_AUX = {L.ACT_RELU: L.AUX_RELU_MASK, L.ACT_TANH: L.AUX_TANH_GRAD, L.ACT_NONE: L.AUX_NONE}
_AUX.update({a: L.AUX_PREACT | (a << 8) for a in range(L.ACT_SILU, L.ACT_SOFTPLUS + 1)})


class Dense:

    def __init__(self, parts, k_in, act, split=None):
        self.parts = parts
        self.K = k_in
        self.act = _ACT[act] if not isinstance(act, int) else act
        if split is None:
            self.split_src = self.split_dst = k_in
            self.k_pad = P(k_in)
        else:
            self.split_src, self.split_dst, self.k_pad = split
        self.n_pad = max(off + P(n) for _, n, off in parts)
        self.N = parts[0][1]

    @property
# ... 35 lines not shown
                assert sc[k] > 0 and math.log2(sc[k]) == round(math.log2(sc[k])), f"loss_scaler.{k} must be a power of two"
            assert sc['growth_factor'] >= 1.0 and sc['backoff_factor'] <= 1.0 and int(sc['growth_interval']) >= 1
            self.loss_scaler = sc
            if not scale_given:
                grad_scale = float(sc['init_scale'])
        self._gs_init = float(grad_scale)
        self.gs = 1.0 if self.dyn_scale else float(grad_scale)
        self.truncate = bool(cfg.get('truncate_grads', False))
        self.grad_norm = float(cfg.get('grad_norm', 1.0))
        self.norm_value = bool(cfg.get('normalize_value', False))
        self.bounds_coef = float(cfg.get('bounds_loss_coef') or 0.0)
        self.adaptive_lr = cfg.get('lr_schedule', 'constant') == 'adaptive'
        self.kl_threshold = float(cfg.get('kl_threshold', 0.008))
        self.obs, self.act = net.obs_size, net.actions_num
        self.z = net.latent_dim if kind == 'ase' else 0
        self.amp = net.amp_obs_size if kind in ('amp', 'ase') else 0
        self.masked = kind in ('amp', 'ase')
        self.has_disc = kind in ('amp', 'ase')
        self.has_enc = kind == 'ase'
        self.div_on = kind == 'ase' and cfg.get('amp_diversity_bonus', 0) != 0
        self.enc_sep = bool(getattr(net, 'enc_separate', False))
        self.enc_gp = kind == 'ase' and cfg.get('enc_grad_penalty', 0) != 0 and cfg.get('enc_coef', 0) != 0
        self.mu_tanh = kind == 'ppo' and getattr(net, 'mu_tanh', False)
        self.sigma_mode = getattr(net, 'sigma_mode', 'frozen')
        self.ls_mode = {'frozen': L.LS_FROZEN, 'vector': L.LS_VECTOR, 'head': L.LS_ROWS}[self.sigma_mode]
        self.gp32 = bool(cfg.get('gp_f32', False)) and self.has_disc and dtype in (torch.float16, torch.bfloat16) and \
            cfg.get('disc_coef', 0) * cfg.get('disc_grad_penalty', 0) != 0
        self._scratch = {}
        self.multi_stream = bool(cfg.get('multi_stream', True)) and getattr(backend, 'name', '') == 'hip'
        self._side_streams = None
        o = dict(tn_grouped=True, tn_wg_side=64, tn_early=False, disc_early=True, short_prologue=True, style_early=False,
                 relu_bits=True, fused_apply=True, apply_wide=True, side_streams=2, gp_scale_split=True, xstep=True,
                 gp_stream='auto', style_side=0, style_wg=0, side_priority=None, prefetch=True, disc_after_style=False, gp_split='f16',
                 stream_offset=0, gp_value_late=False)
        unknown = set(cfg.get('engine_opts', {}) or {}) - set(o)
        assert not unknown, f"unknown engine_opts {sorted(unknown)}"
        o.update(cfg.get('engine_opts', {}) or {})
        self.engine_opts = o
        self._tn_defer = bool(getattr(backend, 'grouped_tn_ok', None)) and bool(o['tn_grouped'])
        self._tn_queue, self._tn_plans = [], {}
        self._tn_wg_side = int(o['tn_wg_side'])
        self._tn_early = bool(o['tn_early'])
        self._disc_early = bool(o['disc_early'])
        self._early_fork = None
        self._short_prologue = bool(o['short_prologue']) and cfg.get('graph_capture') != 'hipgraph'
        self._prep = self._lat_ready = self._fill_done = None
        self._style_early = bool(o['style_early'])
        self._n_side = max(1, min(int(o['side_streams']), 2))
        self._apply_groups = None
        self._use_bits = bool(o['relu_bits'])
        self._fused_apply = hasattr(backend, 'apply_multi') and bool(o['fused_apply'])
        self._xstep = bool(o['xstep']) and cfg.get('graph_capture') != 'hipgraph'
        gp_side = (self.dyn_scale or self.M < 8192) if o['gp_stream'] == 'auto' else bool(o['gp_stream'])
        self._gp_side = gp_side and cfg.get('graph_capture') != 'hipgraph'
        self._style_side = int(o['style_side'])
        self._disc_after_style = bool(o['disc_after_style'])
        self._disc_split = False
        self._enc_z_ready = False
        self._prefetch = bool(o['prefetch'])
        self._par, self._par_set, self._last_par, self._fenced = 0, False, None, False
        self._stats_exchanged = False
        self._style_wg = int(o['style_wg'])
        sp = o['side_priority']
        if sp is None:
            sp = [0, -1, 0] if (self.gp32 or self.dyn_scale) else [-1, 0, 0]
        self._side_prio = [int(x) for x in sp] if isinstance(sp, (list, tuple)) else [int(sp)] * 3
        self._gp_stream_obj = None
        self._xs = False
        self._disc_fwd_out = self._gp_value_done = self._pre_done = None
        self._apply_wide = bool(o['apply_wide'])
        self._apply_desc = self._apply_items = None
        self.force_dist = bool(cfg.get('force_dist', False))
        self.dp_grad_dtype = cfg.get('dp_grad_dtype', 'f32')
        assert self.dp_grad_dtype in ('f32', 'bf16'), self.dp_grad_dtype
        self._xbuf = {}
        self._disc_acc_mark = None
        self._merged_stats = False
        self._acc_in_bucket = False
        self._refresh_desc = None
        self._mb_desc = None
        self._mb_desc_key = None
        self._build_layers()
        self._bind_params()
        self._alloc(infer_rows)
        self.refresh_shadows()

    def _build_layers(self):
# ... 137 lines not shown
        self.dMU = zt(Ra, self.mu_head.n_pad)
        self.V = zt(M, self.value_head.n_pad, f32)
        self.dV = zt(M, self.value_head.n_pad)
        if self.style:
            self._Zs2 = [zt(Ra, P(self.z)) for _ in range(nset)]
            self.Zs = self._Zs2[0]
            self.Hs, self.dZs = chain_bufs(self.style[:-1], Ra)
            self.dStyle = zt(Ra, P(self.z))
            self.new_z = zt(M, self.z, f32)
            seed = int(self.cfg.get('seed', 0)) + (0 if self.shard else 7919 * self.rank)
            self.rng_state = torch.tensor([seed ^ 0x5EED, 0], dtype=torch.int64, device=dev)
            self.div_rng = torch.tensor([seed ^ 0xD1755EED, 0], dtype=torch.int64, device=dev)
        if self.has_disc:
            Rd = 3 * AMB
            self.Xd4 = zt(4 * AMB, self.disc[0].k_pad)
            self.Xd = self.Xd4[:Rd]
            self.G0 = self.Xd4[Rd:]
            self.Hd4 = [with_bits(zt(4 * AMB, d.n_pad), d) for d in self.disc]
            self.dZd4 = [zt(4 * AMB, d.n_pad) for d in self.disc]
            self.Hd = [h[:Rd] for h in self.Hd4]
            self.dGp = [h[Rd:] for h in self.Hd4]
            self.dZd = [z[:Rd] for z in self.dZd4]
            self.Gp = [z[Rd:] for z in self.dZd4]
            self.HD = zt(Rd, self.disc_head.n_pad, f32)
            self.dHD = zt(Rd, self.disc_head.n_pad)
            self.GpTop = zt(AMB, self.disc[-1].n_pad, f32)
            if self.gp32:
                assert all(d.act == L.ACT_RELU for d in self.disc), "gp_f32 is built for ReLU discriminators"
                import types
                g = self._gp32 = types.SimpleNamespace()
                g.X = zt(AMB, self.disc[0].k_pad, f32)
                g.Ws = [zt(d.n_pad, d.k_pad, f32) for d in self.disc]
                g.Wts = [zt(d.k_pad, d.n_pad, f32) for d in self.disc]
                g.H = [zt(AMB, d.n_pad, f32) for d in self.disc]
                g.bits = [torch.zeros(AMB, d.n_pad // 32, dtype=torch.int32, device=dev) for d in self.disc]
                g.Gp = [zt(AMB, d.n_pad, f32) for d in self.disc]
                g.G0 = zt(AMB, self.disc[0].k_pad, f32)
                g.cast = None
            if self.enc_chain:
                self.He, self.dZe = chain_bufs(self.enc_chain, AMB)
                self.E = zt(AMB, self.enc_head.n_pad, f32)
                self.dE = zt(AMB, self.enc_head.n_pad)
            if self.has_enc:
                self.enc_z = zt(AMB, self.z, f32)
            if self.enc_gp:
                ech = self.enc_chain if self.enc_chain else self.disc
                ehead = self.enc_head if self.enc_chain else self.disc_head
                self.Ue = zt(AMB, ehead.n_pad)
                self.Re = [zt(AMB, d.n_pad) for d in ech]
                self.Ge = zt(AMB, ech[0].k_pad)
                self.Qe = [zt(AMB, d.n_pad) for d in ech]
                self.DUe = zt(AMB, ehead.n_pad, f32)
            self.amp_mean = zt(3, self.amp, f32)
            self.amp_std = zt(3, self.amp, f32)
            self.amp_state = torch.zeros(2 * self.amp + 1, dtype=torch.float64, device=dev)
            self.amp_state[self.amp:] = 1.0
        n_amp = 3 * 2 * self.amp if self.has_disc else 0
        self.stats_flat = torch.zeros(n_amp + 2 * self.obs + 1, dtype=torch.float64, device=dev)
        self.obs_sums = self.stats_flat[n_amp:n_amp + 2 * self.obs]
        if self.has_disc:
            self.amp_sums_flat = self.stats_flat[:n_amp]
            self.amp_sums = self.amp_sums_flat.view(3, 2 * self.amp)
        self.obs_mean = zt(1, self.obs, f32)
        self.obs_std = zt(1, self.obs, f32)
        self.obs_state = torch.zeros(2 * self.obs + 1, dtype=torch.float64, device=dev)
        self.obs_state[self.obs:] = 1.0
        self.val_state = torch.tensor([0.0, 1.0, 1.0], dtype=torch.float64, device=dev)
        self.acc = torch.zeros(L.ACC_COUNT, dtype=torch.float64, device=dev)
        self.set_result_slots(1)
        self.mb = {'actions': zt(M, self.act, f32), 'mu': zt(M, self.act, f32), 'sigma': zt(M, self.act, f32),
# ... 5 lines not shown
            self.mb['ase_latents'] = zt(M, self.z, f32)

    def set_result_slots(self, n):
        dev = self.dev
        self.res_ring = torch.zeros(n, L.RES_COUNT, dtype=torch.float32, device=dev)
        self.logit_ring = torch.zeros(n, 3 * self.AMB, dtype=torch.float32, device=dev) if self.has_disc else None
        self.use_slot(0)

    def use_slot(self, i):
        self.slot = i
        self.use_parity(i)
        self.res = self.res_ring[i]
        self.logit_slot = self.logit_ring[i].view(-1, 1) if self.logit_ring is not None else None

    def use_parity(self, p):
        self._par = p = p % len(self._Xa2)
        self._par_set = True
        self.Xa, self.Xc = self._Xa2[p], self._Xc2[p]
        if self.style:
            self.Zs = self._Zs2[p]

    def refresh_shadows(self):
        if self._refresh_desc is None:
            rows, items = [], []
            for d in self.layers:
                for (name, nr, off), W, b in zip(d.parts, d.W, d.b):
                    ws, wts, bs = d.Ws[off:], d.Wts[:, off:], d.bs[off:off + nr]
                    rows.append([W.data_ptr(), nr, d.K, ws.data_ptr(), ws.stride(0), wts.data_ptr(), wts.stride(0),
                                 d.split_src, d.split_dst - d.split_src, b.data_ptr(), bs.data_ptr(), (d.K + 31) // 32])
                    items.append((W, ws, wts, d.split_src, d.split_dst, b, bs))
            self._refresh_desc = torch.tensor(rows, dtype=torch.int64, device=self.dev)
            self._refresh_items = items
        self.be.refresh_shadow_multi(self._refresh_desc, self._refresh_items, self.dtype)

    def _build_apply_desc(self):
        if self._apply_desc is not None:
            return
        import struct
        c = self.cfg
        terms = {}
        for W, gW, coef, slot in self.l2_terms:
            t = terms.setdefault(W.data_ptr(), [0.0, []])
            t[0] += coef
            if slot is not None and slot not in t[1]:
                t[1].append(slot)
        if self.has_disc:
            t = terms.setdefault(self.disc_head.W[0].data_ptr(), [0.0, []])
            t[1].insert(0, L.ACC_LOGIT_W2)
            if c['disc_weight_decay'] != 0 and L.ACC_DISC_W2 not in t[1]:
                t[1].append(L.ACC_DISC_W2)
        base = self.params.data_ptr()
        rows, items = [], []
        for d in self.layers:
            for (name, nr, off), W, b, gW, gb in zip(d.parts, d.W, d.b, d.gW, d.gb):
                ws, wts, bs = d.Ws[off:], d.Wts[:, off:], d.bs[off:off + nr]
                ow, ob = (W.data_ptr() - base) // 4, (b.data_ptr() - base) // 4
                mW, vW = self.adam_m[ow:ow + W.numel()], self.adam_v[ow:ow + W.numel()]
                mb, vb = self.adam_m[ob:ob + nr], self.adam_v[ob:ob + nr]
                coef, slots = terms.get(W.data_ptr(), [0.0, []])
                assert len(slots) <= 2, slots
                sa = slots[0] if len(slots) > 0 else -1
                sb = slots[1] if len(slots) > 1 else -1
                gap = d.split_dst - d.split_src
                wide = int(self._apply_wide and d.K % 4 == 0 and ws.stride(0) % 4 == 0 and wts.stride(0) % 4 == 0
                           and (d.split_src >= d.K or (d.split_src % 4 == 0 and gap % 4 == 0))
                           and ws.data_ptr() % 16 == 0 and wts.data_ptr() % 16 == 0)
                rows.append([W.data_ptr(), nr, d.K, ws.data_ptr(), ws.stride(0), wts.data_ptr(), wts.stride(0), d.split_src,
                             gap, b.data_ptr(), bs.data_ptr(), (d.K + 31) // 32, gW.data_ptr(),
                             mW.data_ptr(), vW.data_ptr(), gb.data_ptr(), mb.data_ptr(), vb.data_ptr(),
                             struct.unpack('<i', struct.pack('<f', float(coef)))[0], sa, sb, wide, 0, 0])
                items.append((W, ws, wts, d.split_src, d.split_dst, b, bs, gW.view(-1).view_as(W), mW.view_as(W), vW.view_as(W),
                              gb, mb, vb, float(coef), sa, sb))
        n_pol = sum(len(d.parts) for d in self.style + self.actor + [self.mu_head] + self.critic + [self.value_head])
        if self.sigma_mode == 'vector':
            b = self.logstd
            ob = (b.data_ptr() - base) // 4
            gb, mb, vb = self.glogstd, self.adam_m[ob:ob + b.numel()], self.adam_v[ob:ob + b.numel()]
            W = self.params[ob:ob]
            rows.insert(n_pol, [W.data_ptr(), b.numel(), 0, 0, 0, 0, 0, 0, 0, b.data_ptr(), b.data_ptr(), 0, gb.data_ptr(),
                                mb.data_ptr(), vb.data_ptr(), gb.data_ptr(), mb.data_ptr(), vb.data_ptr(), 0, -1, -1, 0, 0, 0])
            items.insert(n_pol, (W.view(0, 0), None, None, 0, 0, b, b, self.grads[ob:ob].view(0, 0), self.adam_m[ob:ob].view(0, 0),
                                 self.adam_v[ob:ob].view(0, 0), gb, mb, vb, 0.0, -1, -1))
            n_pol += 1
        n_cov = sum(it[0].numel() + it[5].numel() for it in items)
        assert n_cov == self.n_train, (n_cov, self.n_train)
        self._apply_desc = torch.tensor(rows, dtype=torch.int64, device=self.dev)
        self._apply_items = items

        def span(its):
            ts = [t for it in its for t in (it[0], it[5]) if t.numel()]
            lo = min((t.data_ptr() - base) // 4 for t in ts)
            hi = max((t.data_ptr() - base) // 4 + t.numel() for t in ts)
            assert hi - lo == sum(it[0].numel() + it[5].numel() for it in its), "a parameter bucket must be contiguous"
            return lo, hi
        self._apply_groups = {'policy': (0, n_pol) + span(items[:n_pol])}
        if len(items) > n_pol:
            self._apply_groups['disc'] = (n_pol, len(items)) + span(items[n_pol:])

    def _fwd(self, d, X, Y, rows, act=None):
        act = d.act if act is None else act
        self._nt(X, d.Ws, Y, rows, d.n_pad, d.k_pad, bias=d.bs, act=act,
                        mask_out=self._mask_of(Y) if (act == L.ACT_RELU or act >= L.ACT_SILU) else None)

    def _aux(self, aux, mode):
        if mode == L.AUX_RELU_MASK:
            bits = self._mask_of(aux)
            if bits is not None:
                return bits, L.AUX_RELU_BITS
        elif (mode & 0xFF) == L.AUX_PREACT:
            pre = self._mask_of(aux)
            assert pre is not None, "a smooth activation's data gradient needs the pre-activation twin of its buffer"
            return pre, mode
        return (aux if mode else None), mode

    def _mask_of(self, h):
        e = self._bits.get(h.untyped_storage().data_ptr()) if h is not None else None
        if e is None:
            return None
        base, bits = e
        off = (h.data_ptr() - base.data_ptr()) // base.element_size()
# ... 300 lines not shown
                if after is not None:
                    self.eng.be.wait(after)
            return self

        def __exit__(self, *a):
            if self.stream is not None:
                self.done = self.eng.be.mark()
                self.ctx.__exit__(*a)

    def _join_branch(self, br):
        if br.stream is not None:
            self.be.wait(br.done)

    def _mark(self):
        return self.be.mark() if self.multi_stream else None

    def _finish_branch(self, group, inline_apply, last=False):
        self._flush_tn(0 if last else self._tn_wg_side)
        if inline_apply:
            a, b, lo, hi = self._apply_groups[group]
            if self._dist_on():
                with_acc = bool(last and self.shard and self.dp_grad_dtype == 'f32')
                if with_acc and self._disc_acc_mark is not None:
                    self.be.wait(self._disc_acc_mark)
                self._exchange_bucket(group, lo, hi, with_acc)
                self._acc_in_bucket = with_acc
                if not self.shard:
                    self._host(lambda: self.grads[lo:hi].mul_(1.0 / self.R))
            if self.dyn_scale:
                self._dyn_check(group, lo, hi)
                if last:
                    self._dyn_apply()
            else:
                self.be.apply_multi(self._apply_desc[a:b], self._apply_items[a:b], self.dtype, self.opt_state, self.acc)

    def _disc_forward(self, amp_streams, ds=None):
        self._disc_inputs(amp_streams, ds)
        return self._disc_matrices()

    def _disc_inputs(self, amp_streams, ds=None):
        be, c, AMB = self.be, self.cfg, self.AMB
        Rd = 3 * AMB
        norm_amp = self.has_disc and c.get('normalize_amp_input', True)
        amb_den = self.AMBg if self.shard else self.AMB
        if self._amp_stats_in_branch():
            self._amp_moments(amp_streams)
            self._exchange_amp_sums()
        if norm_amp:
            be.rms_finalize(self.amp_state, self.amp, self.amp_sums, amb_den, 3, self.amp_mean, self.amp_std)
        else:
            self._identity_stats(self.amp_mean, self.amp_std)
        gp_fork = self._mark() if (self.gp32 and self._gp_side) else None
        self._enc_z_ready = False
        if self.has_enc and ds is not None:
            src, sidx, srm = amp_streams[0]
            zsrc = ds['ase_latents'].view(ds['ase_latents'].shape[0], -1)
            be.gather_rows(zsrc, self.z, sidx, srm, AMB, self.enc_z)
            self._enc_z_ready = True
        xd = [self.Xd[s * AMB:(s + 1) * AMB] for s in range(3)]
        if self.amp % 4 == 0 and all(src.stride(0) % 4 == 0 for src, _, _ in amp_streams):
            be.rms_normalize_multi(amp_streams, self.amp, AMB, [self.amp_mean[s] for s in range(3)],
                                   [self.amp_std[s] for s in range(3)], xd)
        else:
            for s, (src, sidx, srm) in enumerate(amp_streams):
                be.rms_normalize(src, self.amp, sidx, srm, AMB, self.amp_mean[s], self.amp_std[s], [xd[s]])
        self._gp_value_done = None
        if self.gp32:
            gp_coef = c['disc_coef'] * c['disc_grad_penalty']
            if gp_fork is not None:
                with self._Branch(self, self._gp_stream(), gp_fork) as br:
                    self._gp_value(amp_streams, gp_coef)
                self._gp_value_done = br
            elif self.engine_opts['gp_value_late']:
                self._gp_value_pending = (amp_streams, gp_coef)
            else:
                self._gp_value(amp_streams, gp_coef)

    def _disc_matrices(self):
        be, AMB = self.be, self.AMB
        Rd = 3 * AMB
        hd = self._fwd_chain(self.disc, self.Xd, self.Hd, Rd)
        self._fwd(self.disc_head, hd, self.HD, Rd)
        if self.logit_slot is not None:
            be.gather_rows(self.HD, 1, None, (0, 0), Rd, self.logit_slot)
        he = None
        if self.enc_chain:
            he = self._fwd_chain(self.enc_chain, self.Xd[:AMB], self.He, AMB)
            self._fwd(self.enc_head, he, self.E, AMB)
        return hd, he

    def _gp_stream(self):
        if not self.multi_stream:
            return None
# ... 152 lines not shown
                    defer, self._tn_defer = self._tn_defer, False
                    style_backward()
                    self._tn_defer = defer
                else:
                    style_backward()
                    self._flush_tn(self._style_wg)
            self._tn_queue = wide
            self._flush_tn(0)
            self._join_branch(br_style)
        else:
            if self.style:
                style_backward()
            self._join_branch(br_cb)
            if not self._tn_early:
                self._tn_queue = tn_actor + self._tn_queue
        self._finish_branch('policy', inline_apply, last=True)
        if br_disc is not None:
            self._join_branch(br_disc)

    def phase_finish(self):
        c = self.cfg
        if self._dist_on() and self.shard and not self._acc_in_bucket:
            self._ar(self.acc[1:L.ACC_LOGIT_W2])
        self._acc_in_bucket = False
        self._average_kl()
        self.be.finalize_scalars(self.acc, self.res, self.Mg if self.shard else self.M, self.AMBg if self.shard else self.AMB,
                                 self.masked, self.has_disc, self.has_enc, self.div_on, c,
                                 opt_state=self.opt_state if (self.adaptive_lr and self._lr_live) else None, kl_threshold=self.kl_threshold)

    def phase_apply(self, apply=True):
        be, c = self.be, self.cfg
        if apply and self._fused_apply and not self.truncate and not self.dyn_scale:
            self._build_apply_desc()
            be.apply_multi(self._apply_desc, self._apply_items, self.dtype, self.opt_state, self.acc)
        else:
            if self.has_disc:
                for W, gW, coef, slot in self.l2_terms:
                    if coef != 0:
                        be.axpy(gW.view(-1), W.view(-1), coef)
                wl = self.disc_head.W[0]
                be.reduce_sum(wl.view(-1), wl.numel(), True, self.acc, L.ACC_LOGIT_W2)
                if c['disc_weight_decay'] != 0:
                    for d in self.disc:
                        be.reduce_sum(d.W[0].view(-1), d.W[0].numel(), True, self.acc, L.ACC_DISC_W2)
                    be.reduce_sum(wl.view(-1), wl.numel(), True, self.acc, L.ACC_DISC_W2)
                if self.has_enc and c.get('enc_weight_decay', 0) != 0:
                    for W, gW, coef, slot in self.l2_terms:
                        if slot == L.ACC_ENC_W2:
                            be.reduce_sum(W.view(-1), W.numel(), True, self.acc, L.ACC_ENC_W2)
            if apply and self.dyn_scale:
                g = self.grads[:self.n_train]
                self._dyn_check('all', 0, self.n_train)
                if self._dist_on():
                    be.scaler_fold(self.scaler, self.scale_tab)
                    self._ar(self.scaler[:1])
                be.scaler_step(self.scaler, self.opt_state, self.opt_eff, g, scale_tab=self.scale_tab)
            elif self.dyn_scale:
                self._host(lambda: self.scale_tab[1::2].zero_())
            if apply and self.truncate:
                g = self.grads[:self.n_train]
                be.reduce_sum(g, g.numel(), True, self.acc, L.ACC_GRAD_SQ)
                be.clip_scale(g, self.acc, L.ACC_GRAD_SQ, self.grad_norm)
            if apply:
                be.adam(self.params[:self.n_train], self.grads[:self.n_train], self.adam_m[:self.n_train],
                        self.adam_v[:self.n_train], self.opt_eff if self.dyn_scale else self.opt_state)
                self.refresh_shadows()
        self._average_kl()
# ... 19 lines not shown
            elif gp_on:
                need += ['Gp']
                if any(d.act != L.ACT_RELU for d in self.disc):
                    need += ['dZd4']
            if self.enc_gp:
                need += ['Ue']
            for name in need:
                assert hasattr(self, name), f"_scaler_bufs: the engine has no buffer '{name}' (renamed?)"
                add(getattr(self, name))
            if gp_on and self.gp32:
                add(self._gp32.Gp[-1])
            self._scaler_list = {'disc': out, 'policy': []}
        return self._scaler_list

    def _dyn_check(self, group, lo, hi):
        bufs = self._scaler_bufs()
        key = (group, lo, hi)
        tab = self._check_tabs.get(key)
        if tab is None:
            lst = (bufs['disc'] + bufs['policy']) if group == 'all' else list(bufs[group])
            lst.append(self.grads[lo:hi])
            tab = self._check_tabs[key] = (lst, self.be.make_check_table(lst) if hasattr(self.be, 'make_check_table') else None)
        self.be.scaler_check_multi(tab[0], self.scaler, table=tab[1])

    def _dyn_apply(self):
        be = self.be
        g = self.grads[:self.n_train]
        side = self._side(1) if (self.multi_stream and self.has_disc) else None
        with self._Branch(self, side) as br:
            if self._dist_on():
                be.scaler_fold(self.scaler, self.scale_tab)
                self._ar(self.scaler[:1])
            be.scaler_step(self.scaler, self.opt_state, self.opt_eff, g, scale_tab=self.scale_tab)
            be.apply_multi(self._apply_desc, self._apply_items, self.dtype, self.opt_eff, self.acc)
        self._join_branch(br)

    @property
    def _dS(self):
        return self.scale_tab[0:2] if self.dyn_scale else None

    @property
    def _dI(self):
        return self.scale_tab[2:4] if self.dyn_scale else None

    @property
    def _dI2(self):
        return self.scale_tab[4:6] if self.dyn_scale else None

    @property
    def _dOne(self):
        return self.scale_tab[6:8] if self.dyn_scale else None

    def _nt(self, *a, alpha_dev=None, **kw):
        if alpha_dev is None and self.dyn_scale:
            alpha_dev = self._dOne
        self.be.gemm_nt(*a, alpha_dev=alpha_dev, **kw)

    def set_grad_scale(self, s):
        assert s > 0 and math.log2(s) == round(math.log2(s)), s
        if self.dyn_scale:
            s = float(s)
            self.scaler[4:5] = torch.tensor([s], dtype=torch.float64)
            self.scale_tab.copy_(torch.tensor([s, 0.0, 1.0 / s, 0.0, 1.0 / (s * s), 0.0, 1.0, 0.0], dtype=torch.float32))
        else:
            self.gs = float(s)

    def scaler_state(self):
# ... 74 lines not shown
        s = math.sqrt(cg)
        top = self.disc[-1]
        Sc, Sr = self._gp_scales()
        be.gp_seed(self.Hd[-1][2 * AMB:], self.disc_head.W[0].view(-1), self.Gp[-1], AMB, top.N, scale=s * Sc)
        for l in range(nl - 1, 0, -1):
            d, pl = self.disc[l], self.disc[l - 1]
            aux, mode = self._aux(self.Hd4[l - 1], _AUX[pl.act])
            self._nt(self.dZd4[l], d.Wts, self.dZd4[l - 1], 4 * AMB, d.k_pad, d.n_pad, aux=aux, aux_mode=mode,
                       aux_split=Rd, aux_delta=AMB)
        d0 = self.disc[0]
        self._nt(self.Gp[0], d0.Wts, self.G0, AMB, d0.k_pad, d0.n_pad, alpha=Sr / Sc, alpha_dev=self._dS)
        be.sqnorm(self.G0, AMB, d0.k_pad, self.acc, L.ACC_GP, scale=1.0 / (cg * Sr * Sr), dyn=self._dI2)
        aux, mode = self._aux(self.Hd[0][2 * AMB:], L.AUX_RELU_MASK)
        self._nt(self.G0, d0.Ws, self.dGp[0], AMB, d0.n_pad, d0.k_pad, aux=aux, aux_mode=mode)
        for l in range(1, nl):
            d = self.disc[l]
            last = l == nl - 1
            aux, mode = self._aux(self.Hd[l][2 * AMB:], L.AUX_RELU_MASK)
            self._nt(self.dGp[l - 1], d.Ws, self.GpTop if last else self.dGp[l], AMB, d.n_pad, d.k_pad, aux=aux,
                       aux_mode=mode, alpha=s / Sr if last else 1.0, alpha_dev=self._dI if last else None)
            if last:
                be.colsum(self.GpTop, AMB, d.N, self.disc_head.gW[0].view(-1))
        for l in range(nl):
            d = self.disc[l]
            X = self.Xd4 if l == 0 else self.Hd4[l - 1]
            self._tn(self.dZd4[l], X, d.gW[0], 4 * AMB, d.n_pad, d.k_pad, d.N, d.K, d.split_src, d.split_dst,
                     gbias=d.gb[0], bias_rows=Rd)

    def _gp_value(self, amp_streams, gp_coef):
        be, AMB, g = self.be, self.AMB, self._gp32
        nl, S = len(self.disc), self.gs
        s = math.sqrt(gp_coef * 2.0 / self.AMBg)
        bits = L.AUX_RELU_BITS
        src, sidx, srm = amp_streams[2]
        be.rms_normalize(src, self.amp, sidx, srm, AMB, self.amp_mean[2], self.amp_std[2], [g.X])
        x3_prev = getattr(be, 'x3', None)
        mode = self.cfg.get('gp_f32')
        half = mode == 'x3' and x3_prev is not None and self.engine_opts['gp_split'] == 'f16'
        if mode == 'x3' and x3_prev is not None:
            be.x3 = 'f16' if half else True
        ex = (lambda ea: {'x3_exps': (ea, 11)}) if half else (lambda ea: {})
        for l, d in enumerate(self.disc):
            be.refresh_shadow(d.W[0], g.Ws[l], g.Wts[l], d.split_src, d.split_dst, **({'x3_exp': 11} if half else {}))
        x = g.X
        for l, d in enumerate(self.disc):
            self._nt(x, g.Ws[l], g.H[l], AMB, d.n_pad, d.k_pad, bias=d.bs, act=L.ACT_RELU, mask_out=g.bits[l],
                       **ex(12 if l == 0 else 6))
            x = g.H[l]
        top = self.disc[-1]
        be.gp_seed(g.H[-1], self.disc_head.W[0].view(-1), g.Gp[-1], AMB, top.N, scale=s)
        for l in range(nl - 1, 0, -1):
            d = self.disc[l]
            self._nt(g.Gp[l], g.Wts[l], g.Gp[l - 1], AMB, d.k_pad, d.n_pad, aux=g.bits[l - 1], aux_mode=bits, **ex(12))
        d0 = self.disc[0]
        self._nt(g.Gp[0], g.Wts[0], g.G0, AMB, d0.k_pad, d0.n_pad, alpha=S, alpha_dev=self._dS, **ex(12))
        if x3_prev is not None:
            be.x3 = x3_prev

    def _gp_f32(self, gp_coef):
        be, AMB, g = self.be, self.AMB, self._gp32
        Rd, nl, S = 3 * AMB, len(self.disc), self.gs
        cg = gp_coef * 2.0 / self.AMBg
        s = math.sqrt(cg)
        bits = L.AUX_RELU_BITS
        d0 = self.disc[0]
        if self._gp_value_done is not None:
            self._join_branch(self._gp_value_done)
            self._gp_value_done = None
        if getattr(self, '_gp_value_pending', None) is not None:
            self._gp_value(*self._gp_value_pending)
            self._gp_value_pending = None
        be.sqnorm(g.G0, AMB, d0.k_pad, self.acc, L.ACC_GP, scale=1.0 / (cg * S * S), dyn=self._dI2)
        if g.cast is None:
            code = {torch.bfloat16: L.BF16, torch.float16: L.F16}[self.dtype]
            items = [(g.Gp[l], self.disc[l].n_pad, self.Gp[l]) for l in range(nl)] + [(g.G0, d0.k_pad, self.G0)]
            rows = [[src.data_ptr(), src.stride(0), c, dst.data_ptr(), dst.stride(0), code] for src, c, dst in items]
            g.cast = (torch.tensor(rows, dtype=torch.int64, device=self.dev), items)
        be.gather_multi(g.cast[0], g.cast[1], None, (0, 0), AMB)
        for l in range(nl - 1, 0, -1):
            self._dgrad(self.disc[l], self.dZd[l], self.dZd[l - 1], Rd, self.Hd[l - 1], self.disc[l - 1].act)
        self._nt(self.G0, d0.Ws, self.dGp[0], AMB, d0.n_pad, d0.k_pad, aux=g.bits[0], aux_mode=bits)
        for l in range(1, nl):
            d = self.disc[l]
            last = l == nl - 1
            self._nt(self.dGp[l - 1], d.Ws, self.GpTop if last else self.dGp[l], AMB, d.n_pad, d.k_pad, aux=g.bits[l],
                       aux_mode=bits, alpha=s / S if last else 1.0, alpha_dev=self._dI if last else None)
            if last:
                be.colsum(self.GpTop, AMB, d.N, self.disc_head.gW[0].view(-1))
        for l in range(nl):
            d = self.disc[l]
            X = self.Xd4 if l == 0 else self.Hd4[l - 1]
            self._tn(self.dZd4[l], X, d.gW[0], 4 * AMB, d.n_pad, d.k_pad, d.N, d.K, d.split_src, d.split_dst,
                     gbias=d.gb[0], bias_rows=Rd)

    def _disc_backward_curved(self, gp_coef):
        be, c, AMB = self.be, self.cfg, self.AMB
        Rd, nl, S = 3 * AMB, len(self.disc), self.gs
        cg = gp_coef * 2.0 / self.AMBg
        s = math.sqrt(cg)
        demo = slice(2 * AMB, 3 * AMB)
        top = self.disc[-1]
        Sc, Sr = self._gp_scales()
        be.gp_seed(self._twin(self.Hd[-1][demo], top), self.disc_head.W[0].view(-1), self.Gp[-1], AMB, top.N, scale=s * Sc,
                   act=top.act)
        for l in range(nl - 1, 0, -1):
            d, pl = self.disc[l], self.disc[l - 1]
            aux, mode = self._aux(self.Hd[l - 1][demo], _AUX[pl.act])
            self._nt(self.Gp[l], d.Wts, self.Gp[l - 1], AMB, d.k_pad, d.n_pad, aux=aux, aux_mode=mode)
        d0 = self.disc[0]
        self._nt(self.Gp[0], d0.Wts, self.G0, AMB, d0.k_pad, d0.n_pad, alpha=Sr / Sc, alpha_dev=self._dS)
        be.sqnorm(self.G0, AMB, d0.k_pad, self.acc, L.ACC_GP, scale=1.0 / (cg * Sr * Sr), dyn=self._dI2)
# ... 328 lines not shown
```

### ase_amd/lib.py

```python
import ctypes as C
import os

_HERE = os.path.dirname(os.path.abspath(__file__))
LIB_PATH = os.path.join(_HERE, "csrc", "libase_hip.so")

ABI_VERSION = 9
PPO_SCRATCH = 1024 * 72 + 8
PPO_SCRATCH_LS = 1024 * 136 + 8
LS_FROZEN, LS_VECTOR, LS_ROWS = 0, 1, 2
TN_SLAB = 65536 + 256
F32, BF16, F32X3, F16, F32H3 = 0, 1, 2, 3, 4
ACT_NONE, ACT_RELU, ACT_TANH, ACT_SILU, ACT_ELU, ACT_GELU, ACT_SIGMOID, ACT_SELU, ACT_SOFTPLUS = range(9)
AUX_NONE, AUX_RELU_MASK, AUX_TANH_GRAD, AUX_RELU_BITS, AUX_PREACT = 0, 1, 2, 3, 4
TASK_HEADING, TASK_LOCATION, TASK_REACH, TASK_STRIKE = range(4)
TASK_OBS_COLS = (5, 2, 3, 15)
RESET_FRAME, RESET_TABLE, RESET_MOTION = range(3)
RESET_HAS_TABLE, RESET_HAS_MOTION = 1, 2

(ACC_MASK_SUM, ACC_A_LOSS, ACC_B_LOSS, ACC_ENTROPY, ACC_CLIPPED, ACC_C_LOSS, ACC_KL, ACC_DIV, ACC_BCE_AGENT,
 ACC_BCE_DEMO, ACC_AGENT_ACC, ACC_DEMO_ACC, ACC_GP, ACC_ENC, ACC_ENC_GP, ACC_LOGIT_W2, ACC_DISC_W2, ACC_ENC_W2,
 ACC_GRAD_SQ) = range(19)
ACC_COUNT = 24
(RES_A_LOSS, RES_C_LOSS, RES_B_LOSS, RES_ENTROPY, RES_CLIP_FRAC, RES_KL, RES_DISC_LOSS, RES_DISC_GP,
 RES_DISC_LOGIT_LOSS, RES_DISC_AGENT_ACC, RES_DISC_DEMO_ACC, RES_ENC_LOSS, RES_DIV_LOSS, RES_LOSS,
 RES_MASK_SUM, RES_ENC_GP, RES_LR) = range(17)
RES_COUNT = 20

_p, _i, _i64, _f, _d = C.c_void_p, C.c_int, C.c_int64, C.c_float, C.c_double

SIGNATURES = {
    "ase_hip_gemm_nt": [_p, _i64, _p, _i64, _p, _i64, _p, _p, _i64, _i, _i, _p, _i, _p, _i64, _i, _i, _i, _i, _i, _i, _f, _p, _i, _p],
    "ase_hip_gemm_tn": [_p, _i64, _p, _i64, _p, _p, _i, _i, _i, _i, _i, _i, _i, _i, _f, _p, _i, _p],
    "ase_hip_refresh_shadow": [_p, _i, _i, _p, _i64, _p, _i64, _i, _i, _i, _p],
    "ase_hip_refresh_shadow_multi": [_p, _i, _i, _p],
    "ase_hip_gather_multi": [_p, _i, _p, _i, _i, _i, _p],
    "ase_hip_rms_moments": [_p, _i64, _i, _p, _i, _i, _i, _p, _p, _p],
    "ase_hip_rms_finalize": [_p, _i, _p, _p, _i, _p, _p, _p],
    "ase_hip_rms_normalize": [_p, _i64, _i, _p, _i, _i, _i, _p, _p, _p, _i64, _p, _i64, _p, _i64, _i, _p],
    "ase_hip_rms_unnormalize": [_p, _p, _p, _i64, _p],
    "ase_hip_gather_rows": [_p, _i64, _i, _p, _i, _i, _i, _p, _i64, _i, _p],
    "ase_hip_reduce_sum": [_p, _i64, _i, _p, _i, _p],
    "ase_hip_ppo_head": [_p, _i64, _p, _i64] + [_p] * 11 + [_p, _i64, _p, _i64, _p, _p, _p, _p, _p] + [_i] * 8 + [_f] * 6 + [_p]
                        + [_i, _i64, _p, _i64, _p, _f] + [_i, _p],
    "ase_hip_disc_head": [_p, _i64, _p, _i64, _p, _p, _i, _i, _f, _f, _p, _i, _p],
    "ase_hip_enc_head": [_p, _i64, _p, _i64, _p, _i64, _p, _p, _p, _i, _i, _i, _f, _f, _p, _i, _p],
    "ase_hip_gp_seed": [_p, _i64, _p, _p, _i64, _i, _i, _f, _i, _i, _p],
    "ase_hip_gp_second": [_p, _i64, _p, _i64, _p, _i64, _p, _i64, _i, _i, _i, _i, _p],
    "ase_hip_colsum": [_p, _i64, _i, _i, _f, _p, _p],
    "ase_hip_sqnorm": [_p, _i64, _i, _i, _p, _i, _d, _p, _i, _p],
    "ase_hip_finalize_scalars": [_p, _p, _i, _i, _i, _i, _i, _i] + [_f] * 11 + [_p, _f, _p],
    "ase_hip_enc_gp_seed": [_p, _i64, _p, _i64, _p, _i64, _i, _i, _f, _i, _p],
    "ase_hip_enc_gp_back": [_p, _i64, _p, _i64, _p, _i64, _p, _i64, _p, _i, _i, _f, _p, _i, _p],
    "ase_hip_clip_scale": [_p, _i64, _p, _f, _p],
    "ase_hip_begin_step": [_p, _p, _i, _p, _i, _p, _p],
    "ase_hip_adam": [_p, _p, _p, _p, _i64, _p, _p],
    "ase_hip_axpy": [_p, _p, _i64, _f, _p],
    "ase_hip_scaler_check": [_p, _i64, _i, _p, _p],
    "ase_hip_scaler_check_multi": [_p, _i, _i, _p, _p],
    "ase_hip_scaler_fold": [_p, _p, _p],
    "ase_hip_scaler_step": [_p, _p, _p, _p, _i64, _p, _p],
    "ase_hip_disc_reward": [_p, _i64, _p, _i64, _f, _p],
    "ase_hip_enc_reward": [_p, _i64, _p, _i64, _p, _i64, _i, _f, _p],
    "ase_hip_gae": [_p, _p, _p, _p, _p, _p, _f, _f, _f, _d, _d, _p, _p, _i, _i, _p],
    "ase_hip_adv_norm": [_p, _p, _p, _p, _p, _i64, _i, _i, _p],
    "ase_hip_ring_store": [_p, _i64, _i, _p, _i, _i, _i, _p, _i64, _i64, _p],
    "ase_hip_sample_latents": [_p, _i, _i, _p, _i64, _i, _p, _i64, _i, _p],
    "ase_hip_rms_moments_multi": [_p, _p, _p, _p, _p, _p, _i, _i, _i, _p, _p],
    "ase_hip_rms_normalize_multi": [_p, _p, _p, _p, _p, _p, _p, _p, _p, _i, _i, _i, _i, _p],
    "ase_hip_normalize_rows": [_p, _i64, _p, _i64, _i, _i, _p],
    "ase_hip_sample_actions": [_p, _i64, _p, _i64, _p, _p, _p, _p, _p, _p, _p, _i, _i, _i, _p],
    "ase_hip_debug_nt_profile": [_p],
    "ase_hip_debug_nt_profile_clock": [_i],
    "ase_hip_motion_state": [_p] * 6 + [_i] + [_p] * 6 + [_i, _p, _p, _i, _p, _i] + [_p] * 8,
    "ase_hip_build_amp_obs": [_p, _p, _p, _p, _p, _p, _p, _i, _i, _i, _p, _i, _i, _i, _p, _i, _i, _p],
    "ase_hip_humanoid_obs_max": [_p, _p, _p, _p, _i, _i, _i, _i, _p, _i, _p, _i64, _i, _p],
    "ase_hip_humanoid_reset": [_p, _p, _p, _p, _p, _i, _p, _p, _i, _i, _i, _f, _i, _p, _p, _p],
    "ase_hip_task_obs": [_i, _p, _p, _p, _p, _p, _i, _p, _i, _p, _i64, _i, _p],
    "ase_hip_task_reward": [_i, _p, _p, _p, _p, _p, _f, _p, _p, _i, _i, _f, _i, _p, _p],
    "ase_hip_amp_reset": [_p] * 6 + [_i] + [_p] * 6 + [_i, _p, _i] + [_p] * 5 + [_i, _i, _p, _p, _p, _i, _p, _i64, _p, _p, _i64, _i,
                          _p, _p, _p, _p, _i, _i, _i, _f, _p, _i, _p],
    "ase_hip_clip_frames": [_p] * 6 + [_i] + [_p] * 4 + [_i, _i, _p, _p, _i] + [_p] * 7,
    "ase_hip_gemm_nt_kernel_id": [_i, _i, _i, _i],
    "ase_hip_apply_multi": [_p, _i, _p, _p, _i, _p],
    "ase_hip_gemm_tn_grouped_plan": [_p, _i, _i, _p, _i, _p, _p, _i, _p],
    "ase_hip_prog_create": [_p],
    "ase_hip_prog_destroy": [_p],
    "ase_hip_prog_begin": [_p],
    "ase_hip_prog_end": [_p],
    "ase_hip_prog_size": [_p],
    "ase_hip_prog_launch": [_p],
    "ase_hip_prog_host": [_p, _p],
    "ase_hip_mark": [_p, _p],
    "ase_hip_wait": [_p, _i],
    "ase_hip_memset": [_p, _i, _i64, _p],
    "ase_hip_memcpy": [_p, _p, _i64, _p],
    "ase_hip_gemm_tn_grouped": [_p, _p, _i, _p, _i, _p, _p, _i, _p],
}


class AseHipError(RuntimeError):
    pass


def load():
    import torch
    if not os.path.exists(LIB_PATH):
        raise AseHipError(
            f"{LIB_PATH} is missing: build it with `python -c 'import __graft_entry__ as g; g.build()'` "
            "or `make -C ase_amd/csrc`.  There is no CPU or PyTorch fallback for the update path.")
    lib = C.CDLL(LIB_PATH)
    lib.ase_hip_abi_version.restype = C.c_int
    lib.ase_hip_last_error.restype = C.c_char_p
    for name, argtypes in SIGNATURES.items():
        fn = getattr(lib, name)
        fn.argtypes = argtypes
        fn.restype = C.c_int
# ... 19 lines not shown
```

### include/ase_hip.h

```cpp
#ifndef ASE_HIP_H
#define ASE_HIP_H

#include <stdint.h>

#ifdef __cplusplus
extern "C" {
#endif

#define ASE_HIP_ABI_VERSION 9

enum { ASE_F32 = 0, ASE_BF16 = 1, ASE_F32X3 = 2 ,
       ASE_F32H3 = 4 ,
       ASE_F16 = 3  };
enum { ASE_ACT_NONE = 0, ASE_ACT_RELU = 1, ASE_ACT_TANH = 2, ASE_ACT_SILU = 3, ASE_ACT_ELU = 4, ASE_ACT_GELU = 5,
       ASE_ACT_SIGMOID = 6, ASE_ACT_SELU = 7, ASE_ACT_SOFTPLUS = 8 };
enum { ASE_AUX_NONE = 0, ASE_AUX_RELU_MASK = 1, ASE_AUX_TANH_GRAD = 2, ASE_AUX_RELU_BITS = 3 ,
       ASE_AUX_PREACT = 4  };
enum { ASE_OK = 0, ASE_EINVAL = -1, ASE_ELAUNCH = -2, ASE_EUNSUPPORTED = -3 };

int ase_hip_abi_version(void);
const char* ase_hip_last_error(void);

int ase_hip_gemm_nt_kernel_id(int M, int N, int K, int dtype);

int ase_hip_debug_nt_profile(void* buf);
int ase_hip_debug_nt_profile_clock(int shader_clock);


int ase_hip_gemm_nt(const void* A, int64_t lda, const void* B, int64_t ldb, void* C, int64_t ldc,
                    const float* bias, const void* aux, int64_t ldaux, int aux_split, int aux_delta,
                    float* colsum, int colsum_n, void* mask_out, int64_t ldmask, int M, int N, int K, int act,
                    int aux_mode, int out_f32, float alpha, float* alpha_dev, int dtype, void* stream);

int ase_hip_gemm_tn(const void* A, int64_t lda, const void* B, int64_t ldb, float* G, float* gbias,
                    int bias_rows, int M, int N, int K, int n_real, int k_real, int split_src, int split_dst,
                    float alpha, const float* alpha_dev, int dtype, void* stream);

#define ASE_TN_SLAB (65536 + 256)
int ase_hip_gemm_tn_grouped_plan(int64_t* problems, int n_problems, int target_wg, int32_t* work, int max_work,
                                 int* n_work, int32_t* red, int max_red, int* n_red);
int ase_hip_gemm_tn_grouped(const int64_t* problems, const int32_t* work, int n_work, const int32_t* red, int n_red,
                            float* workspace, const float* alpha_dev, int dtype, void* stream);

int ase_hip_refresh_shadow(const float* W, int n_real, int k_real, void* Ws, int64_t ldws,
                           void* Wts, int64_t ldwts, int split_src, int split_dst, int dtype,
                           void* stream);

int ase_hip_refresh_shadow_multi(const int64_t* desc, int n_layers, int dtype, void* stream);


int ase_hip_rms_moments(const float* src, int64_t ld_src, int D, const int32_t* idx, int remap_h,
                        int remap_n, int M, const double* state, double* sums, void* stream);

int ase_hip_rms_moments_multi(const float* const* srcs, const int64_t* ld_srcs, const int32_t* const* idxs,
                              const int* remap_h, const int* remap_n, double* const* sums, int n_streams, int D, int M,
                              const double* state, void* stream);
int ase_hip_rms_normalize_multi(const float* const* srcs, const int64_t* ld_srcs, const int32_t* const* idxs,
                                const int* remap_h, const int* remap_n, const float* const* means,
                                const float* const* stds, void* const* outs, const int64_t* ld_outs, int n_streams, int D,
                                int M, int dtype, void* stream);

int ase_hip_rms_finalize(double* state, int D, const double* sums, const int32_t* counts ,
                         int n_streams, float* mean_out, float* std_out, void* stream);

int ase_hip_rms_normalize(const float* src, int64_t ld_src, int D, const int32_t* idx, int remap_h,
                          int remap_n, int M, const float* mean, const float* std,
                          void* out0, int64_t ld0, void* out1, int64_t ld1, void* out2, int64_t ld2,
                          int dtype, void* stream);

int ase_hip_rms_unnormalize(const double* state, const float* x, float* y, int64_t n, void* stream);

int ase_hip_gather_rows(const float* src, int64_t ld_src, int D, const int32_t* idx, int remap_h,
                        int remap_n, int M, void* dst, int64_t ld_dst, int dst_dtype, void* stream);

int ase_hip_gather_multi(const int64_t* desc, int n_fields, const int32_t* idx, int remap_h, int remap_n,
                         int M, void* stream);

enum {
    ASE_ACC_MASK_SUM = 0,
    ASE_ACC_A_LOSS,
    ASE_ACC_B_LOSS,
    ASE_ACC_ENTROPY,
    ASE_ACC_CLIPPED,
    ASE_ACC_C_LOSS,
    ASE_ACC_KL,
    ASE_ACC_DIV,
    ASE_ACC_BCE_AGENT,
    ASE_ACC_BCE_DEMO,
    ASE_ACC_AGENT_ACC,
    ASE_ACC_DEMO_ACC,
    ASE_ACC_GP,
    ASE_ACC_ENC,
    ASE_ACC_ENC_GP,
// ... 72 lines not shown
int ase_hip_axpy(float* g, const float* w, int64_t n, float c, void* stream);

int ase_hip_scaler_check(const void* buf, int64_t n, int dtype, double* scaler, void* stream);
int ase_hip_scaler_check_multi(const int64_t* table, int n_bufs, int wg_per_buf, double* scaler, void* stream);
int ase_hip_scaler_fold(double* scaler, float* scale_tab, void* stream);
int ase_hip_scaler_step(double* scaler, double* opt_state, double* opt_eff, float* grads, int64_t n, float* scale_tab,
                        void* stream);


int ase_hip_disc_reward(const float* logit, int64_t ld_l, float* r, int64_t n, float scale, void* stream);
int ase_hip_enc_reward(const float* e, int64_t ld_e, const float* z, int64_t ld_z, float* r, int64_t n,
                       int z_dim, float scale, void* stream);
int ase_hip_gae(const uint8_t* dones, const float* values, const float* next_values,
                const float* r_task, const float* r_disc, const float* r_enc, float w_task, float w_disc,
                float w_enc, double gamma, double tau, float* advs, float* returns, int H, int N, void* stream);
int ase_hip_adv_norm(const float* returns, const float* values, const float* mask, float* adv,
                     double* acc3, int64_t n, int normalize, int phase, void* stream);

int ase_hip_ring_store(const float* src, int64_t ld_src, int D, const int32_t* idx, int remap_h,
                       int remap_n, int n, float* dst, int64_t size, int64_t head, void* stream);

int ase_hip_normalize_rows(const float* x, int64_t ld_x, float* y, int64_t ld_y, int n, int dim, void* stream);

int ase_hip_sample_actions(const float* mu, int64_t ld_mu, const float* logstd, int64_t ld_logstd, const float* rand_probs,
                           uint64_t* rng_state, float* mu_out, float* sigma_out, float* actions, float* neglogp,
                           float* rand_mask, int n, int act_dim, int mu_tanh, void* stream);

int ase_hip_sample_latents(float* z, int rows, int dim, uint64_t* rng_state, int64_t row_offset, int advance,
                           void* z2 ,
                           int64_t ld_z2, int z2_dtype, void* stream);

int ase_hip_apply_multi(const int64_t* desc, int n_layers, const double* opt_state, double* acc, int dtype,
                        void* stream);


int ase_hip_build_amp_obs(const float* root_pos, const float* root_rot, const float* root_vel,
                          const float* root_ang_vel, const float* dof_pos, const float* dof_vel,
                          const float* key_body_pos, int n_envs, int n_dof, int n_key, const int32_t* dof_offsets,
                          int n_joints, int local_root_obs, int root_height_obs, float* hist, int n_steps, int shift,
                          void* stream);

int ase_hip_motion_state(const float* gts, const float* grs, const float* lrs, const float* grvs, const float* gravs,
                         const float* dvs, int n_bodies, const float* lengths, const int32_t* num_frames, const float* dt,
                         const int32_t* length_starts, const int32_t* motion_ids, const float* times, int n,
                         const int32_t* dof_body_ids, const int32_t* dof_offsets, int n_joints,
                         const int32_t* key_body_ids, int n_key, float* root_pos, float* root_rot, float* dof_pos,
                         float* root_vel, float* root_ang_vel, float* dof_vel, float* key_pos, void* stream);


int ase_hip_humanoid_obs_max(const float* body_pos, const float* body_rot, const float* body_vel,
                             const float* body_ang_vel, int n_envs, int n_bodies, int local_root_obs,
                             int root_height_obs, const int32_t* env_ids, int n_ids, float* obs, int64_t ld_obs,
                             int col_offset, void* stream);

int ase_hip_humanoid_reset(const int64_t* progress_buf, const float* contact_forces, const float* body_pos,
                           const float* termination_heights, const int32_t* contact_body_ids, int n_contact,
                           const float* tar_contact_forces, const int32_t* strike_body_ids, int n_strike, int n_envs,
                           int n_bodies, float max_episode_length, int enable_early_termination, int64_t* reset,
                           int64_t* terminated, void* stream);

enum { ASE_TASK_HEADING = 0, ASE_TASK_LOCATION = 1, ASE_TASK_REACH = 2, ASE_TASK_STRIKE = 3 };

int ase_hip_task_obs(int kind, const float* root_states, const float* tar_a, const float* tar_b, const float* tar_speed,
                     const float* tar_states, int n_envs, const int32_t* env_ids, int n_ids, float* obs, int64_t ld_obs,
                     int col_offset, void* stream);

// ... 42 lines not shown
```

Measured before the change: 1.745 million samples/s.

## Fuse gradient-penalty seed, half-precision twin and sum-of-squares into GEMM epilogues

Adds an extended NT GEMM entry point whose epilogue can apply the discriminator-head seed, write an f16/bf16 twin copy, and accumulate a squared norm. This lets the gradient-penalty path drop the separate gp_seed, sqnorm and cast/gather launches. It also adds twin-output RMS normalization and a split-descriptor optimizer apply. The aim is fewer kernel launches and less memory traffic, at the cost of more epilogue register pressure and code complexity.

```diff
diff --git a/ase_amd/backend.py b/ase_amd/backend.py
--- a/ase_amd/backend.py
+++ b/ase_amd/backend.py
@@ -28,6 +28,7 @@
 
 class HipBackend:
     name = "hip"
+    nt_fused_epilogue = True
 
     def __init__(self, device=None, x3=False):
         self.x3 = x3 if x3 == 'f16' else bool(x3)
@@ -110,7 +111,8 @@
         return c
 
     def gemm_nt(self, A, B, Cm, M, N, K, bias=None, aux=None, aux_mode=L.AUX_NONE, colsum=None, colsum_n=0,
-                act=L.ACT_NONE, alpha=1.0, aux_split=0, aux_delta=0, mask_out=None, x3_exps=None, alpha_dev=None):
+                act=L.ACT_NONE, alpha=1.0, aux_split=0, aux_delta=0, mask_out=None, x3_exps=None, alpha_dev=None,
+                seed=None, twin=None, sq=None, store=True):
         dt = self._gemm_code(A.dtype, x3_exps)
         assert B.dtype == A.dtype
         if aux_mode == L.AUX_RELU_BITS:
@@ -118,6 +120,21 @@
         else:
             assert aux is None or aux.dtype == A.dtype
         assert mask_out is None or mask_out.dtype == (A.dtype if act >= L.ACT_SILU else torch.int32)
+        if seed is not None or twin is not None or sq is not None:
+            assert (dt & 0xFF) == L.F32H3, "seed / twin / sq belong to the half-split f32 launches (x3 = 'f16', x3_exps)"
+            assert Cm.dtype == torch.float32 and (store or twin is not None)
+            sw, ss = seed if seed is not None else (None, 0.0)
+            acc, slot, sscale, dyn = sq if sq is not None else (None, 0, 0.0, None)
+            assert acc is None or acc.dtype == torch.float64
+            L.check(self.lib.ase_hip_gemm_nt_ex(_ptr(A), _ld(A), _ptr(B), _ld(B), _ptr(Cm) if store else None, _ld(Cm), _ptr(bias), _ptr(aux),
+                                                _ld(aux), int(aux_split), int(aux_delta), _ptr(colsum), int(colsum_n),
+                                                _ptr(mask_out), _ld(mask_out), M, N, K, act, aux_mode, 0,
+                                                float(alpha), _ptr(alpha_dev), dt,
+                                                _ptr(sw), 0 if sw is None else sw.numel(), float(ss),
+                                                _ptr(twin), _ld(twin), 0 if twin is None else _code(twin.dtype),
+                                                None if acc is None else C.c_void_p(acc.data_ptr() + 8 * int(slot)), float(sscale),
+                                                _ptr(dyn), self._stream()), "gemm_nt_ex")
+            return
         out_f32 = int(Cm.dtype == torch.float32 and A.dtype != torch.float32)
         L.check(self.lib.ase_hip_gemm_nt(_ptr(A), _ld(A), _ptr(B), _ld(B), _ptr(Cm), _ld(Cm), _ptr(bias), _ptr(aux),
                                          _ld(aux), int(aux_split), int(aux_delta), _ptr(colsum), int(colsum_n),
@@ -180,6 +197,11 @@
     def apply_multi(self, desc, items, dtype, opt_state, acc):
         L.check(self.lib.ase_hip_apply_multi(_ptr(desc), desc.shape[0], _ptr(opt_state), _ptr(acc), _code(dtype),
                                              self._stream()), "apply_multi")
+
+    def apply_multi_split(self, desc, items, dtype, opt_state, acc, desc2, items2):
+        assert desc2.shape == (desc.shape[0], 8) and desc2.is_contiguous()
+        L.check(self.lib.ase_hip_apply_multi_v2(_ptr(desc), desc.shape[0], _ptr(desc2), _ptr(opt_state), _ptr(acc), _code(dtype),
+                                                self._stream()), "apply_multi_v2")
 
     def gather_multi(self, desc, items, idx, remap, M):
         L.check(self.lib.ase_hip_gather_multi(_ptr(desc), desc.shape[0], _ptr(idx), remap[0], remap[1], M,
@@ -362,6 +384,18 @@
         L.check(self.lib.ase_hip_rms_normalize_multi(srcs, lds, idxs, rh, rn, mp, sp, op, lo, n, D, M, _code(outs[0].dtype),
                                                      self._stream()), "rms_normalize_multi")
 
+    def rms_normalize_multi_twin(self, streams, D, M, means, stds, outs, outs32):
+        n, srcs, lds, idxs, rh, rn = self._stream_arrays(streams)
+        mp = (C.c_void_p * n)(*[t.data_ptr() for t in means])
+        sp = (C.c_void_p * n)(*[t.data_ptr() for t in stds])
+        op = (C.c_void_p * n)(*[t.data_ptr() for t in outs])
+        lo = (C.c_int64 * n)(*[int(t.stride(0)) for t in outs])
+        assert all(t is None or t.dtype == torch.float32 for t in outs32)
+        op32 = (C.c_void_p * n)(*[None if t is None else t.data_ptr() for t in outs32])
+        lo32 = (C.c_int64 * n)(*[0 if t is None else int(t.stride(0)) for t in outs32])
+        L.check(self.lib.ase_hip_rms_normalize_multi_v2(srcs, lds, idxs, rh, rn, mp, sp, op, lo, op32, lo32, n, D, M,
+                                                        _code(outs[0].dtype), self._stream()), "rms_normalize_multi_v2")
+
     def rms_finalize(self, state, D, sums, count, n_streams, mean_out, std_out):
         counts = (C.c_int32 * max(n_streams, 1))(*([int(count)] * max(n_streams, 1)))
         L.check(self.lib.ase_hip_rms_finalize(_ptr(state), D, _ptr(sums), counts, n_streams, _ptr(mean_out),
diff --git a/ase_amd/csrc/common.h b/ase_amd/csrc/common.h
--- a/ase_amd/csrc/common.h
+++ b/ase_amd/csrc/common.h
@@ -49,6 +49,19 @@
 template <> __device__ __forceinline__ f32s_t from_f32<f32s_t>(float x) { return f32s_t{x}; }
 template <> __device__ __forceinline__ f32h_t from_f32<f32h_t>(float x) { return f32h_t{x}; }
 template <> __device__ __forceinline__ f16_t from_f32<f16_t>(float x) { return (f16_t)__builtin_amdgcn_fmed3f(x, -65504.f, 65504.f); }
+
+__device__ __forceinline__ void split_half(float v, float scale, f16_t& hi, f16_t& lo) {
+    const float s = __builtin_amdgcn_fmed3f(v * scale, -65504.f, 65504.f);
+    hi = (f16_t)s;
+    lo = (f16_t)(s - (float)hi);
+}
+__device__ __forceinline__ void store_split(char* row, int col, float v, float scale) {
+    f16_t hi, lo;
+    split_half(v, scale, hi, lo);
+    char* g = row + (col >> 3) * 32 + (col & 7) * 2;
+    *reinterpret_cast<f16_t*>(g) = hi;
+    *reinterpret_cast<f16_t*>(g + 16) = lo;
+}
 
 template <typename T> struct V16;
 template <> struct V16<bf16_t> { typedef bf16x8 x8; typedef bf16x4 x4; };
diff --git a/ase_amd/csrc/gemm.hip b/ase_amd/csrc/gemm.hip
--- a/ase_amd/csrc/gemm.hip
+++ b/ase_amd/csrc/gemm.hip
@@ -41,19 +41,39 @@
     return nt_choice(M, N, K, ase_elem_size(dtype), ase_elem_size(dtype) == 2);
 }
 
-extern "C" int ase_hip_gemm_nt(const void* A, int64_t lda, const void* B, int64_t ldb, void* C, int64_t ldc,
-                               const float* bias, const void* aux, int64_t ldaux, int aux_split, int aux_delta,
-                               float* colsum, int colsum_n, void* mask_out, int64_t ldmask, int M, int N, int K, int act,
-                               int aux_mode, int out_f32, float alpha, float* alpha_dev, int dtype_word, void* stream) {
+namespace {
+
+struct NTFused {
+    const float* seed_w = nullptr; int seed_n = 0; float seed_scale = 0.f;
+    void* twin = nullptr; int64_t ldtwin = 0; int twin_dtype = 0;
+    double* sq_acc = nullptr; double sq_scale = 0.0; const float* sq_dyn = nullptr;
+    bool any() const { return seed_w || twin || sq_acc; }
+};
+
+int gemm_nt_impl(const void* A, int64_t lda, const void* B, int64_t ldb, void* C, int64_t ldc,
+                 const float* bias, const void* aux, int64_t ldaux, int aux_split, int aux_delta,
+                 float* colsum, int colsum_n, void* mask_out, int64_t ldmask, int M, int N, int K, int act,
+                 int aux_mode, int out_f32, float alpha, float* alpha_dev, int dtype_word, const NTFused& fu, void* stream) {
     const int dtype = dtype_word & 0xFF, ea = (dtype_word >> 8) & 0xFF, eb = (dtype_word >> 16) & 0xFF;
     const int es = ase_elem_size(dtype);
     ASE_CHECK_ARG(dtype == ASE_F32 || dtype == ASE_BF16 || dtype == ASE_F32X3 || dtype == ASE_F16 || dtype == ASE_F32H3,
                   "gemm_nt: bad dtype %d", dtype);
     ASE_CHECK_ARG(ea >= 0 && ea <= 24 && eb >= 0 && eb <= 24 && (dtype == ASE_F32H3 || (ea | eb) == 0),
                   "gemm_nt: operand scale exponents (bits 8-15 / 16-23 of dtype) are 0..24 and belong to ASE_F32H3 only");
-    ASE_CHECK_ARG(A && B && C && M > 0 && N > 0 && K > 0, "gemm_nt: null/empty operand (M=%d N=%d K=%d)", M, N, K);
+    ASE_CHECK_ARG(A && B && (C || fu.twin) && M > 0 && N > 0 && K > 0, "gemm_nt: null/empty operand (M=%d N=%d K=%d)", M, N, K);
+    if (fu.any()) {
+        ASE_CHECK_ARG(dtype == ASE_F32H3 && colsum == nullptr && act <= ASE_ACT_RELU &&
+                          (aux_mode == ASE_AUX_NONE || aux_mode == ASE_AUX_RELU_BITS),
+                      "gemm_nt_ex: seed / twin / sum of squares belong to ASE_F32H3 launches without column sums, with no activation or "
+                      "ReLU and no mask operand or a bit matrix");
+        ASE_CHECK_ARG(fu.seed_w == nullptr || (fu.seed_n >= 0 && fu.seed_n <= N), "gemm_nt_ex: seed_n=%d outside [0, N]", fu.seed_n);
+        ASE_CHECK_ARG(fu.twin == nullptr || ((fu.twin_dtype == ASE_F16 || fu.twin_dtype == ASE_BF16) && fu.ldtwin >= N &&
+                                             ((uintptr_t)fu.twin % 8) == 0 && (fu.ldtwin * 2) % 8 == 0),
+                      "gemm_nt_ex: the twin is f16 / bf16, 8-byte aligned, ldtwin >= N in whole 8-byte steps");
+        ASE_CHECK_ARG(fu.sq_acc == nullptr || ((uintptr_t)fu.sq_acc % 8) == 0, "gemm_nt_ex: misaligned sq_acc");
+    }
     ASE_CHECK_ARG((K * es) % 64 == 0, "gemm_nt: K=%d is not a multiple of %d elements", K, 64 / es);
-    ASE_CHECK_ARG(lda >= K && ldb >= K && ldc >= N, "gemm_nt: leading dimension too small");
+    ASE_CHECK_ARG(lda >= K && ldb >= K && (ldc >= N || C == nullptr), "gemm_nt: leading dimension too small");
     ASE_CHECK_ARG(((uintptr_t)A % 16) == 0 && ((uintptr_t)B % 16) == 0 && (lda * es) % 16 == 0 && (ldb * es) % 16 == 0,
                   "gemm_nt: A/B must be 16-byte aligned with 16-byte row pitch");
     ASE_CHECK_ARG(aux_mode == ASE_AUX_NONE || aux != nullptr, "gemm_nt: aux_mode %d without aux", aux_mode);
@@ -82,6 +102,9 @@
     p.prof = nullptr;
     p.prof_clk = 0;
     p.sa = 1.f;
+    p.seed_w = fu.seed_w; p.seed_n = fu.seed_n; p.seed_scale = fu.seed_scale;
+    p.twin = (char*)fu.twin; p.ldtwin = fu.ldtwin * 2; p.twin_dtype = fu.twin_dtype;
+    p.sq_acc = fu.sq_acc; p.sq_scale = fu.sq_scale; p.sq_dyn = fu.sq_dyn;
     if (dtype == ASE_BF16) return dispatch_nt_bf16(p, (hipStream_t)stream);
     if (dtype == ASE_F16) return dispatch_nt_f16(p, (hipStream_t)stream);
     if (dtype == ASE_F32X3) return dispatch_nt_x3(p, (hipStream_t)stream);
@@ -92,3 +115,27 @@
     }
     return dispatch_nt_f32(p, (hipStream_t)stream);
 }
+
+}
+
+extern "C" int ase_hip_gemm_nt(const void* A, int64_t lda, const void* B, int64_t ldb, void* C, int64_t ldc,
+                               const float* bias, const void* aux, int64_t ldaux, int aux_split, int aux_delta,
+                               float* colsum, int colsum_n, void* mask_out, int64_t ldmask, int M, int N, int K, int act,
+                               int aux_mode, int out_f32, float alpha, float* alpha_dev, int dtype_word, void* stream) {
+    return gemm_nt_impl(A, lda, B, ldb, C, ldc, bias, aux, ldaux, aux_split, aux_delta, colsum, colsum_n, mask_out, ldmask, M, N, K,
+                        act, aux_mode, out_f32, alpha, alpha_dev, dtype_word, NTFused{}, stream);
+}
+
+extern "C" int ase_hip_gemm_nt_ex(const void* A, int64_t lda, const void* B, int64_t ldb, void* C, int64_t ldc,
+                                  const float* bias, const void* aux, int64_t ldaux, int aux_split, int aux_delta,
+                                  float* colsum, int colsum_n, void* mask_out, int64_t ldmask, int M, int N, int K, int act,
+                                  int aux_mode, int out_f32, float alpha, float* alpha_dev, int dtype_word,
+                                  const float* seed_w, int seed_n, float seed_scale, void* twin, int64_t ldtwin, int twin_dtype,
+                                  double* sq_acc, double sq_scale, const float* sq_dyn, void* stream) {
+    NTFused fu;
+    fu.seed_w = seed_w; fu.seed_n = seed_n; fu.seed_scale = seed_scale;
+    fu.twin = twin; fu.ldtwin = ldtwin; fu.twin_dtype = twin_dtype;
+    fu.sq_acc = sq_acc; fu.sq_scale = sq_scale; fu.sq_dyn = sq_dyn;
+    return gemm_nt_impl(A, lda, B, ldb, C, ldc, bias, aux, ldaux, aux_split, aux_delta, colsum, colsum_n, mask_out, ldmask, M, N, K,
+                        act, aux_mode, out_f32, alpha, alpha_dev, dtype_word, fu, stream);
+}
diff --git a/ase_amd/csrc/gemm_nt.h b/ase_amd/csrc/gemm_nt.h
--- a/ase_amd/csrc/gemm_nt.h
+++ b/ase_amd/csrc/gemm_nt.h
@@ -38,6 +38,9 @@
     int tiles_m, tiles_n;
     unsigned long long* prof;
     int prof_clk;
+    const float* seed_w; int seed_n; float seed_scale;
+    char* twin; int64_t ldtwin; int twin_dtype;
+    double* sq_acc; double sq_scale; const float* sq_dyn;
 };
 
 
diff --git a/ase_amd/csrc/gemm_nt_kernels.h b/ase_amd/csrc/gemm_nt_kernels.h
--- a/ase_amd/csrc/gemm_nt_kernels.h
+++ b/ase_amd/csrc/gemm_nt_kernels.h
@@ -185,10 +185,10 @@
     }
 }
 
-template <typename T, int FM, int FN, int FMC, int FNC, int AUXK, bool PRE = false>
-__device__ __forceinline__ void nt_epilogue_impl(const NTParams& p, f32x16 (&acc)[FM][FN], float* slab, int lane,
-                                                 int mrow0, int ncol0,
-                                                 AuxReg<T, AUXK> (*pre)[(FMC * 32) / (64 / (FNC * 8))] = nullptr) {
+template <typename T, int FM, int FN, int FMC, int FNC, int AUXK, bool PRE = false, bool FUSE = false>
+__device__ __forceinline__ double nt_epilogue_impl(const NTParams& p, f32x16 (&acc)[FM][FN], float* slab, int lane,
+                                                   int mrow0, int ncol0,
+                                                   AuxReg<T, AUXK> (*pre)[(FMC * 32) / (64 / (FNC * 8))] = nullptr) {
     constexpr int WCOLS = FNC * 32, WROWS = FMC * 32;
     const int col_in = lane & 31, row_hi = (lane >> 5) * 4;
     constexpr int ELPR = WCOLS / 4;
@@ -199,6 +199,7 @@
     const int c4 = lane % ELPR, rsub = lane / ELPR;
     AuxReg<T, AUXK> areg[AHEAD ? 2 : 1][NIT];
     bool bad = false;
+    double sq = 0.0;
 
     auto load_aux = [&](int ch, AuxReg<T, AUXK> (&dst)[NIT]) {
         nt_aux_load<T, FM, FN, FMC, FNC, AUXK>(p, ch, lane, mrow0, ncol0, dst);
@@ -237,6 +238,13 @@
             }
         }
         float cs[4] = {0.f, 0.f, 0.f, 0.f};
+        f32x4 seed = {0.f, 0.f, 0.f, 0.f};
+        if constexpr (FUSE) {
+            if (p.seed_w && n0 < p.N) {
+#pragma unroll
+                for (int q = 0; q < 4; ++q) seed[q] = p.seed_scale * (n0 + q < p.seed_n ? p.seed_w[n0 + q] : 0.f);
+            }
+        }
         if (n0 < p.N) {
 #pragma unroll
             for (int it = 0; it < NIT; ++it) {
@@ -276,7 +284,36 @@
                         else v[q] = v[q] * act_grad(p.aux_mode >> 8, a);
                     }
                 }
-                if (p.out_f32 || sizeof(T) == 4) {
+                if constexpr (FUSE) {
+                    f32x4 sv = v;
+                    if (p.seed_w) {
+#pragma unroll
+                        for (int q = 0; q < 4; ++q) sv[q] = seed[q] * (v[q] > 0.f ? 1.f : 0.f);
+                    }
+#pragma unroll
+                    for (int q = 0; q < 4; ++q) bad |= ovf_hit1(sv[q]);
+                    if (p.C) *reinterpret_cast<f32x4*>(p.C + (int64_t)m * p.ldc + (int64_t)n0 * 4) = sv;
+                    if (p.twin) {
+                        char* t = p.twin + (int64_t)m * p.ldtwin + (int64_t)n0 * 2;
+                        if (p.twin_dtype == ASE_F16) {
+                            f16x4 o;
+#pragma unroll
+                            for (int q = 0; q < 4; ++q) o[q] = from_f32<f16_t>(sv[q]);
+                            *reinterpret_cast<f16x4*>(t) = o;
+                        } else {
+                            bf16x4 o;
+#pragma unroll
+                            for (int q = 0; q < 4; ++q) o[q] = from_f32<bf16_t>(sv[q]);
+                            *reinterpret_cast<bf16x4*>(t) = o;
+                        }
+                    }
+                    if (p.sq_acc) {
+                        float s = 0.f;
+#pragma unroll
+                        for (int q = 0; q < 4; ++q) s = __fadd_rn(s, __fmul_rn(sv[q], sv[q]));
+                        sq += (double)s;
+                    }
+                } else if (p.out_f32 || sizeof(T) == 4) {
 #pragma unroll
                     for (int q = 0; q < 4; ++q) bad |= ovf_hit1(v[q]);
                     *reinterpret_cast<f32x4*>(p.C + (int64_t)m * p.ldc + (int64_t)n0 * 4) = v;
@@ -316,14 +353,16 @@
         }
     }
     ovf_report(p.alpha_dev, bad);
-}
-
-template <typename T, int FM, int FN, int FMC, int FNC>
-__device__ __forceinline__ void nt_epilogue(const NTParams& p, f32x16 (&acc)[FM][FN], float* slab, int lane, int mrow0,
-                                            int ncol0) {
-    if (p.aux_mode == ASE_AUX_NONE) nt_epilogue_impl<T, FM, FN, FMC, FNC, 0>(p, acc, slab, lane, mrow0, ncol0);
-    else if (p.aux_mode == ASE_AUX_RELU_BITS) nt_epilogue_impl<T, FM, FN, FMC, FNC, 2>(p, acc, slab, lane, mrow0, ncol0);
-    else nt_epilogue_impl<T, FM, FN, FMC, FNC, 1>(p, acc, slab, lane, mrow0, ncol0);
+    return sq;
+}
+
+template <typename T, int FM, int FN, int FMC, int FNC, bool FUSE = false>
+__device__ __forceinline__ double nt_epilogue(const NTParams& p, f32x16 (&acc)[FM][FN], float* slab, int lane, int mrow0,
+                                              int ncol0) {
+    if (p.aux_mode == ASE_AUX_NONE) return nt_epilogue_impl<T, FM, FN, FMC, FNC, 0, false, FUSE>(p, acc, slab, lane, mrow0, ncol0);
+    if (p.aux_mode == ASE_AUX_RELU_BITS) return nt_epilogue_impl<T, FM, FN, FMC, FNC, 2, false, FUSE>(p, acc, slab, lane, mrow0, ncol0);
+    if constexpr (FUSE) return 0.0;
+    else return nt_epilogue_impl<T, FM, FN, FMC, FNC, 1>(p, acc, slab, lane, mrow0, ncol0);
 }
 
 template <typename T, int FM, int FN, int AUXK, bool MASK>
@@ -373,7 +412,7 @@
     else nt_epilogue_rows_impl<T, FM, FN, AUXK, false>(p, acc, lane, mrow0, ncol0, bits);
 }
 
-template <typename T, int WGM, int WGN, int FM, int FN, int RB, int S, int WPE = 1, bool SW = false>
+template <typename T, int WGM, int WGN, int FM, int FN, int RB, int S, int WPE = 1, bool SW = false, bool FUSE = false>
 __global__ __launch_bounds__(WGM * WGN * 64, WPE) void gemm_nt_kernel(NTParams p) {
     constexpr int BM = WGM * FM * 32, BN = WGN * FN * 32;
     constexpr int BK = RB / (int)sizeof(T);
@@ -469,10 +508,26 @@
 
     constexpr int FNC = (FN > 2) ? 2 : FN;
     float* slab = reinterpret_cast<float*>(smem) + wid * (FM * 32 * FNC * 32);
-    nt_epilogue<T, FM, FN, FM, FNC>(p, acc, slab, lane, bm0 + wm * FM * 32, bn0 + wn * FN * 32);
-}
-
-template <typename T, int WGM, int WGN, int FM, int FN, int RB, int S, int WPE = 1, bool SW = false>
+    const double sq = nt_epilogue<T, FM, FN, FM, FNC, FUSE>(p, acc, slab, lane, bm0 + wm * FM * 32, bn0 + wn * FN * 32);
+    if constexpr (FUSE) {
+        if (p.sq_acc) {
+            const double w = wave_sum(sq);
+            __syncthreads();
+            double* red = reinterpret_cast<double*>(smem);
+            if (lane == 0) red[wid] = w;
+            __syncthreads();
+            if (tid == 0) {
+                double t = 0.0;
+                for (int i = 0; i < WGM * WGN; ++i) t += red[i];
+                double scale = p.sq_scale;
+                if (p.sq_dyn) scale *= (double)*p.sq_dyn;
+                atomic_add_f64(p.sq_acc, t * scale);
+            }
+        }
+    }
+}
+
+template <typename T, int WGM, int WGN, int FM, int FN, int RB, int S, int WPE = 1, bool SW = false, bool FUSE = false>
 int launch_nt(const NTParams& p0, hipStream_t stream) {
     constexpr int BM = WGM * FM * 32, BN = WGN * FN * 32;
     constexpr int ring = S * (BM + BN) * RB;
@@ -480,7 +535,7 @@
     constexpr int lds = ring > slab ? ring : slab;
     static_assert(lds <= 160 * 1024, "LDS budget");
     static bool attr_done = false;
-    auto kern = gemm_nt_kernel<T, WGM, WGN, FM, FN, RB, S, WPE, SW>;
+    auto kern = gemm_nt_kernel<T, WGM, WGN, FM, FN, RB, S, WPE, SW, FUSE>;
     if (!attr_done) {
         hipError_t e = hipFuncSetAttribute(reinterpret_cast<const void*>(kern),
                                            hipFuncAttributeMaxDynamicSharedMemorySize, lds);
@@ -762,6 +817,21 @@
     const bool fits32 = (int64_t)p.M * p.lda < (int64_t)0x7FFFFFFF && (int64_t)p.N * p.ldb < (int64_t)0x7FFFFFFF;
     int choice = nt_choice(p.M, p.N, p.K, (int)sizeof(T), sizeof(T) == 2);
     if ((choice == 2 || choice == 6) && !fits32) choice = 3;
+    if constexpr (std::is_same<T, f32h_t>::value) {
+        if (p.seed_w || p.twin || p.sq_acc) {
+            switch (choice) {
+                case 0: return launch_nt<T, 2, 2, 1, 1, 64, 4, 1, false, true>(p, s);
+                case 2: case 3: case 6:
+                    if (k128) return launch_nt<T, 4, 2, 2, 4, 128, 2, 1, false, true>(p, s);
+                    return launch_nt<T, 4, 2, 2, 4, 64, 4, 1, false, true>(p, s);
+                case 4: return launch_nt<T, 2, 2, 1, 2, 128, 2, 2, false, true>(p, s);
+                case 5: return launch_nt<T, 2, 2, 1, 1, 128, 4, 2, false, true>(p, s);
+                default:
+                    if (k128) return launch_nt<T, 2, 2, 2, 2, 128, 2, 2, false, true>(p, s);
+                    return launch_nt<T, 2, 2, 2, 2, 64, 4, 2, false, true>(p, s);
+            }
+        }
+    }
     switch (choice) {
         case 0: return launch_nt<T, 2, 2, 1, 1, 64, 4>(p, s);
         case 6:
diff --git a/ase_amd/csrc/gemm_tn.hip b/ase_amd/csrc/gemm_tn.hip
--- a/ase_amd/csrc/gemm_tn.hip
+++ b/ase_amd/csrc/gemm_tn.hip
@@ -716,13 +716,6 @@
     }
 }
 
-__device__ __forceinline__ void store_split(char* row, int col, float v, float scale) {
-    const float s = __builtin_amdgcn_fmed3f(v * scale, -65504.f, 65504.f);
-    const f16_t hi = (f16_t)s, lo = (f16_t)(s - (float)hi);
-    char* g = row + (col >> 3) * 32 + (col & 7) * 2;
-    *reinterpret_cast<f16_t*>(g) = hi;
-    *reinterpret_cast<f16_t*>(g + 16) = lo;
-}
 __global__ void refresh_shadow_split_kernel(const float* __restrict__ W, int n_real, int k_real, char* __restrict__ Ws, int64_t ldws,
                                             char* __restrict__ Wts, int64_t ldwts, int split_src, int gap, float scale) {
     __shared__ float tile[32][33];
diff --git a/ase_amd/csrc/optim.hip b/ase_amd/csrc/optim.hip
--- a/ase_amd/csrc/optim.hip
+++ b/ase_amd/csrc/optim.hip
@@ -1,4 +1,5 @@
 #include "common.h"
+#include <type_traits>
 
 namespace {
 
@@ -69,12 +70,13 @@
     *reinterpret_cast<f32x4*>(p) = f32x4{w[0], w[1], w[2], w[3]};
 }
 
-template <typename T>
-__global__ __launch_bounds__(256) void apply_multi_kernel(const int64_t* __restrict__ desc, const double* __restrict__ st,
-                                                          double* __restrict__ acc) {
+template <typename T, bool SPLIT>
+__global__ __launch_bounds__(256, SPLIT ? 8 : 1) void apply_multi_kernel(const int64_t* __restrict__ desc, const double* __restrict__ st,
+                                                          double* __restrict__ acc, const int64_t* __restrict__ desc2) {
     __shared__ float tile[32][129];
     __shared__ double red[16];
     const int64_t* d = desc + 24 * blockIdx.y;
+    const int64_t* e3 = (SPLIT && desc2) ? desc2 + 8 * blockIdx.y : nullptr;
     float* W = reinterpret_cast<float*>(d[0]);
     const int n_real = (int)d[1], k_real = (int)d[2];
     T* Ws = reinterpret_cast<T*>(d[3]);
@@ -172,6 +174,53 @@
                 } else {
                     for (int q = 0; q < 16 && nb + q < n_real; ++q) dst[q] = from_f32<T>(tile[16 * half + q][kk]);
                 }
+                if (SPLIT && e3 && e3[2]) {
+                    const float sc3 = ldexpf(1.f, (int)e3[4]);
+                    char* row = reinterpret_cast<char*>(e3[2]) + (int64_t)((k < split_src) ? k : k + gap) * (e3[3] * 4);
+                    if (nb + 16 <= n_real) {
+#pragma unroll
+                        for (int q = 0; q < 16; q += 4) {
+                            f16x4 h, l;
+#pragma unroll
+                            for (int c = 0; c < 4; ++c) {
+                                f16_t hh, ll;
+                                split_half(tile[16 * half + q + c][kk], sc3, hh, ll);
+                                h[c] = hh; l[c] = ll;
+                            }
+                            char* g = row + ((nb + q) >> 3) * 32 + ((nb + q) & 7) * 2;
+                            *reinterpret_cast<f16x4*>(g) = h;
+                            *reinterpret_cast<f16x4*>(g + 16) = l;
+                        }
+                    } else {
+                        for (int q = 0; q < 16 && nb + q < n_real; ++q) store_split(row, nb + q, tile[16 * half + q][kk], sc3);
+                    }
+                }
+            }
+            if (SPLIT && e3 && e3[0]) {
+                const float sc3 = ldexpf(1.f, (int)e3[4]);
+                char* Ws3 = reinterpret_cast<char*>(e3[0]);
+                const int64_t ld3 = e3[1] * 4;
+                const int rr = threadIdx.x >> 3, kc = (threadIdx.x & 7) * 16;
+                const int n = n0 + rr;
+                if (n < n_real) {
+#pragma unroll
+                    for (int u = 0; u < 16; u += 4) {
+                        const int k4 = k0 + kc + u;
+                        if (k4 < k_real) {
+                            const int kd = (k4 < split_src) ? k4 : k4 + gap;
+                            f16x4 h, l;
+#pragma unroll
+                            for (int c = 0; c < 4; ++c) {
+                                f16_t hh, ll;
+                                split_half(tile[rr][kc + u + c], sc3, hh, ll);
+                                h[c] = hh; l[c] = ll;
+                            }
+                            char* g = Ws3 + (int64_t)n * ld3 + (kd >> 3) * 32 + (kd & 7) * 2;
+                            *reinterpret_cast<f16x4*>(g) = h;
+                            *reinterpret_cast<f16x4*>(g + 16) = l;
+                        }
+                    }
+                }
             }
         }
     } else
@@ -197,6 +246,8 @@
                     W[o] = w; mW[o] = mi; vW[o] = vi;
                 }
                 Ws[(int64_t)n * ldws + ((k < split_src) ? k : k + gap)] = from_f32<T>(w);
+                if (SPLIT && e3 && e3[0])
+                    store_split(reinterpret_cast<char*>(e3[0]) + (int64_t)n * (e3[1] * 4), (k < split_src) ? k : k + gap, w, ldexpf(1.f, (int)e3[4]));
             }
             tile[ty + 8 * i][tx] = w;
         }
@@ -204,8 +255,12 @@
 #pragma unroll
         for (int i = 0; i < 4; ++i) {
             const int k = k0 + ty + 8 * i, n = n0 + tx;
-            if (k < k_real && n < n_real)
+            if (k < k_real && n < n_real) {
                 Wts[(int64_t)((k < split_src) ? k : k + gap) * ldwts + n] = from_f32<T>(tile[tx][ty + 8 * i]);
+                if (SPLIT && e3 && e3[2])
+                    store_split(reinterpret_cast<char*>(e3[2]) + (int64_t)((k < split_src) ? k : k + gap) * (e3[3] * 4), n, tile[tx][ty + 8 * i],
+                                ldexpf(1.f, (int)e3[4]));
+            }
         }
     }
     if (adam && slot_a >= 0) {
@@ -263,17 +318,36 @@
     return ASE_OK;
 }
 
-extern "C" int ase_hip_apply_multi(const int64_t* desc, int n_layers, const double* opt_state, double* acc, int dtype,
-                                   void* stream) {
+namespace {
+int apply_multi_impl(const int64_t* desc, int n_layers, const int64_t* desc2, const double* opt_state, double* acc, int dtype,
+                     void* stream) {
     ASE_CHECK_ARG(desc && n_layers > 0, "apply_multi: null/empty operand");
     ASE_CHECK_ARG(opt_state == nullptr || acc != nullptr, "apply_multi: optimizer step without the accumulator array");
+    ASE_CHECK_ARG(desc2 == nullptr || dtype == ASE_F16, "apply_multi_v2: the half-split shadow pair is built for ASE_F16 storage (dtype %d)",
+                  dtype);
     const dim3 grid(256, n_layers);
     const int rc = ase_dispatch_storage(dtype, [&](auto tag) {
         typedef typename decltype(tag)::type T;
-        ASE_LAUNCH(apply_multi_kernel<T>, grid, dim3(256), 0, (hipStream_t)stream, desc, opt_state, acc);
+        if constexpr (std::is_same<T, f16_t>::value) if (desc2) {
+            ASE_LAUNCH((apply_multi_kernel<T, true>), grid, dim3(256), 0, (hipStream_t)stream, desc, opt_state, acc, desc2);
+            return ASE_OK;
+        }
+        ASE_LAUNCH((apply_multi_kernel<T, false>), grid, dim3(256), 0, (hipStream_t)stream, desc, opt_state, acc, desc2);
         return ASE_OK;
     });
     ASE_CHECK_ARG(rc == ASE_OK, "apply_multi: bad dtype %d", dtype);
     ASE_CHECK_LAUNCH("apply_multi");
     return ASE_OK;
 }
+}
+
+extern "C" int ase_hip_apply_multi(const int64_t* desc, int n_layers, const double* opt_state, double* acc, int dtype,
+                                   void* stream) {
+    return apply_multi_impl(desc, n_layers, nullptr, opt_state, acc, dtype, stream);
+}
+
+extern "C" int ase_hip_apply_multi_v2(const int64_t* desc, int n_layers, const int64_t* desc2, const double* opt_state, double* acc,
+                                      int dtype, void* stream) {
+    ASE_CHECK_ARG(desc2 != nullptr, "apply_multi_v2: null table of the second shadow pairs");
+    return apply_multi_impl(desc, n_layers, desc2, opt_state, acc, dtype, stream);
+}
diff --git a/ase_amd/csrc/rms.hip b/ase_amd/csrc/rms.hip
--- a/ase_amd/csrc/rms.hip
+++ b/ase_amd/csrc/rms.hip
@@ -62,6 +62,7 @@
     const float* src[4]; int64_t ld[4]; const int32_t* idx[4]; int rh[4], rn[4];
     double* sums[4];
     const float* mean[4]; const float* stdv[4]; void* out[4]; int64_t ld_out[4];
+    float* out32[4]; int64_t ld_out32[4];
 };
 
 __global__ __launch_bounds__(256) void rms_moments_multi_kernel(RmsStreams S, int D, int M, const double* __restrict__ state) {
@@ -117,6 +118,7 @@
     f32x4 y;
 #pragma unroll
     for (int c = 0; c < 4; ++c) y[c] = fminf(fmaxf((x[c] - mu[c]) / sd[c], -5.f), 5.f);
+    if (S.out32[s]) *reinterpret_cast<f32x4*>(S.out32[s] + (int64_t)r * S.ld_out32[s] + j) = y;
     if constexpr (sizeof(T) == 2) {
         typename V16<T>::x4 v;
 #pragma unroll
@@ -343,13 +345,16 @@
     return ASE_OK;
 }
 
-extern "C" int ase_hip_rms_normalize_multi(const float* const* srcs, const int64_t* ld_srcs, const int32_t* const* idxs,
-                                           const int* remap_h, const int* remap_n, const float* const* means,
-                                           const float* const* stds, void* const* outs, const int64_t* ld_outs, int n_streams,
-                                           int D, int M, int dtype, void* stream) {
+namespace {
+
+int rms_normalize_multi_impl(const float* const* srcs, const int64_t* ld_srcs, const int32_t* const* idxs,
+                             const int* remap_h, const int* remap_n, const float* const* means,
+                             const float* const* stds, void* const* outs, const int64_t* ld_outs, float* const* outs32,
+                             const int64_t* ld_outs32, int n_streams, int D, int M, int dtype, void* stream) {
     ASE_CHECK_ARG(srcs && ld_srcs && idxs && remap_h && remap_n && means && stds && outs && ld_outs && n_streams >= 1 &&
                       n_streams <= 4 && D > 0 && M > 0, "rms_normalize_multi: null/empty operand (1..4 streams)");
     ASE_CHECK_ARG(dtype == ASE_BF16 || dtype == ASE_F32 || dtype == ASE_F16, "rms_normalize_multi: bad dtype %d", dtype);
+    ASE_CHECK_ARG(outs32 == nullptr || ld_outs32 != nullptr, "rms_normalize_multi: f32 twins without their pitches");
     const int es = ase_elem_size(dtype);
     RmsStreams S = {};
     for (int s = 0; s < n_streams; ++s) {
@@ -359,6 +364,11 @@
                       "rms_normalize_multi: stream %d needs 16-byte rows (D %% 4 == 0, aligned pointers / pitches)", s);
         S.src[s] = srcs[s]; S.ld[s] = ld_srcs[s]; S.idx[s] = idxs[s]; S.rh[s] = remap_h[s]; S.rn[s] = remap_n[s];
         S.mean[s] = means[s]; S.stdv[s] = stds[s]; S.out[s] = outs[s]; S.ld_out[s] = ld_outs[s];
+        if (outs32 && outs32[s]) {
+            ASE_CHECK_ARG(ld_outs32[s] >= D && ld_outs32[s] % 4 == 0 && ((uintptr_t)outs32[s] % 16) == 0,
+                          "rms_normalize_multi: stream %d: the f32 twin needs 16-byte rows of at least D elements", s);
+            S.out32[s] = outs32[s]; S.ld_out32[s] = ld_outs32[s];
+        }
     }
     const dim3 grid((D / 4 + 63) / 64, (M + 3) / 4, n_streams);
     ase_dispatch_storage(dtype, [&](auto tag) {
@@ -368,6 +378,25 @@
     });
     ASE_CHECK_LAUNCH("rms_normalize_multi");
     return ASE_OK;
+}
+
+}
+
+extern "C" int ase_hip_rms_normalize_multi(const float* const* srcs, const int64_t* ld_srcs, const int32_t* const* idxs,
+                                           const int* remap_h, const int* remap_n, const float* const* means,
+                                           const float* const* stds, void* const* outs, const int64_t* ld_outs, int n_streams,
+                                           int D, int M, int dtype, void* stream) {
+    return rms_normalize_multi_impl(srcs, ld_srcs, idxs, remap_h, remap_n, means, stds, outs, ld_outs, nullptr, nullptr, n_streams, D, M,
+                                    dtype, stream);
+}
+
+extern "C" int ase_hip_rms_normalize_multi_v2(const float* const* srcs, const int64_t* ld_srcs, const int32_t* const* idxs,
+                                              const int* remap_h, const int* remap_n, const float* const* means,
+                                              const float* const* stds, void* const* outs, const int64_t* ld_outs,
+                                              float* const* outs32, const int64_t* ld_outs32, int n_streams, int D, int M, int dtype,
+                                              void* stream) {
+    return rms_normalize_multi_impl(srcs, ld_srcs, idxs, remap_h, remap_n, means, stds, outs, ld_outs, outs32, ld_outs32, n_streams, D, M,
+                                    dtype, stream);
 }
 
 extern "C" int ase_hip_rms_finalize(double* state, int D, const double* sums, const int32_t* counts, int n_streams,
diff --git a/ase_amd/engine.py b/ase_amd/engine.py
--- a/ase_amd/engine.py
+++ b/ase_amd/engine.py
@@ -1,3 +1,4 @@
+import contextlib
 import math
 
 import torch
@@ -99,7 +100,7 @@
         o = dict(tn_grouped=True, tn_wg_side=64, tn_early=False, disc_early=True, short_prologue=True, style_early=False,
                  relu_bits=True, fused_apply=True, apply_wide=True, side_streams=2, gp_scale_split=True, xstep=True,
                  gp_stream='auto', style_side=0, style_wg=0, side_priority=None, prefetch=True, disc_after_style=False, gp_split='f16',
-                 stream_offset=0, gp_value_late=False)
+                 stream_offset=0, gp_value_late=False, gp_fuse='auto')
         unknown = set(cfg.get('engine_opts', {}) or {}) - set(o)
         assert not unknown, f"unknown engine_opts {sorted(unknown)}"
         o.update(cfg.get('engine_opts', {}) or {})
@@ -120,6 +121,11 @@
         self._xstep = bool(o['xstep']) and cfg.get('graph_capture') != 'hipgraph'
         gp_side = (self.dyn_scale or self.M < 8192) if o['gp_stream'] == 'auto' else bool(o['gp_stream'])
         self._gp_side = gp_side and cfg.get('graph_capture') != 'hipgraph'
+        self._gp_fuse = bool(self.gp32 and getattr(backend, 'nt_fused_epilogue', False) and cfg.get('gp_f32') == 'x3'
+                             and getattr(backend, 'x3', None) is not None and o['gp_split'] == 'f16'
+                             and (o['gp_fuse'] == 'auto' or bool(o['gp_fuse'])))
+        self._gp_split = self._gp_fuse and hasattr(backend, 'apply_multi_split') and self._fused_apply and dtype == torch.float16
+        self._gp_x_done = False
         self._style_side = int(o['style_side'])
         self._disc_after_style = bool(o['disc_after_style'])
         self._disc_split = False
@@ -323,10 +329,11 @@
                 g.X = zt(AMB, self.disc[0].k_pad, f32)
                 g.Ws = [zt(d.n_pad, d.k_pad, f32) for d in self.disc]
                 g.Wts = [zt(d.k_pad, d.n_pad, f32) for d in self.disc]
-                g.H = [zt(AMB, d.n_pad, f32) for d in self.disc]
+                g.H = [None if (self._gp_fuse and d is self.disc[-1]) else zt(AMB, d.n_pad, f32) for d in self.disc]
                 g.bits = [torch.zeros(AMB, d.n_pad // 32, dtype=torch.int32, device=dev) for d in self.disc]
                 g.Gp = [zt(AMB, d.n_pad, f32) for d in self.disc]
-                g.G0 = zt(AMB, self.disc[0].k_pad, f32)
+                g.G0 = (torch.empty(AMB, self.disc[0].k_pad, dtype=f32, device='meta') if self._gp_fuse
+                        else zt(AMB, self.disc[0].k_pad, f32))
                 g.cast = None
             if self.enc_chain:
                 self.He, self.dZe = chain_bufs(self.enc_chain, AMB)
@@ -398,6 +405,21 @@
             self._refresh_desc = torch.tensor(rows, dtype=torch.int64, device=self.dev)
             self._refresh_items = items
         self.be.refresh_shadow_multi(self._refresh_desc, self._refresh_items, self.dtype)
+        if self._gp_split:
+            self._gp_refresh()
+
+    def _gp_refresh(self):
+        g = self._gp32
+        half = self.cfg.get('gp_f32') == 'x3' and getattr(self.be, 'x3', None) is not None and self.engine_opts['gp_split'] == 'f16'
+        for l, d in enumerate(self.disc):
+            self.be.refresh_shadow(d.W[0], g.Ws[l], g.Wts[l], d.split_src, d.split_dst, **({'x3_exp': 11} if half else {}))
+
+    def _apply(self, opt_state, a=None, b=None):
+        desc, items = self._apply_desc[a:b], self._apply_items[a:b]
+        if self._gp_split:
+            self.be.apply_multi_split(desc, items, self.dtype, opt_state, self.acc, self._apply_desc2[a:b], self._apply_items2[a:b])
+        else:
+            self.be.apply_multi(desc, items, self.dtype, opt_state, self.acc)
 
     def _build_apply_desc(self):
         if self._apply_desc is not None:
@@ -452,6 +474,16 @@
         assert n_cov == self.n_train, (n_cov, self.n_train)
         self._apply_desc = torch.tensor(rows, dtype=torch.int64, device=self.dev)
         self._apply_items = items
+        if self._gp_split:
+            g, rows2, items2 = self._gp32, [[0] * 8 for _ in rows], [None] * len(rows)
+            for l, d in enumerate(self.disc):
+                assert len(d.parts) == 1
+                i = [j for j, it in enumerate(items) if it[0].data_ptr() == d.W[0].data_ptr() and it[0].numel()]
+                assert len(i) == 1
+                rows2[i[0]] = [g.Ws[l].data_ptr(), g.Ws[l].stride(0), g.Wts[l].data_ptr(), g.Wts[l].stride(0), 11, 0, 0, 0]
+                items2[i[0]] = (g.Ws[l], g.Wts[l], 11)
+            self._apply_desc2 = torch.tensor(rows2, dtype=torch.int64, device=self.dev)
+            self._apply_items2 = items2
 
         def span(its):
             ts = [t for it in its for t in (it[0], it[5]) if t.numel()]
@@ -818,7 +850,7 @@
                 if last:
                     self._dyn_apply()
             else:
-                self.be.apply_multi(self._apply_desc[a:b], self._apply_items[a:b], self.dtype, self.opt_state, self.acc)
+                self._apply(self.opt_state, a, b)
 
     def _disc_forward(self, amp_streams, ds=None):
         self._disc_inputs(amp_streams, ds)
@@ -836,7 +868,9 @@
             be.rms_finalize(self.amp_state, self.amp, self.amp_sums, amb_den, 3, self.amp_mean, self.amp_std)
         else:
             self._identity_stats(self.amp_mean, self.amp_std)
-        gp_fork = self._mark() if (self.gp32 and self._gp_side) else None
+        x_twin = self._gp_fuse and hasattr(be, 'rms_normalize_multi_twin') and self.amp % 4 == 0 and \
+            all(src.stride(0) % 4 == 0 for src, _, _ in amp_streams)
+        gp_fork = self._mark() if (self.gp32 and self._gp_side and not x_twin) else None
         self._enc_z_ready = False
         if self.has_enc and ds is not None:
             src, sidx, srm = amp_streams[0]
@@ -844,7 +878,12 @@
             be.gather_rows(zsrc, self.z, sidx, srm, AMB, self.enc_z)
             self._enc_z_ready = True
         xd = [self.Xd[s * AMB:(s + 1) * AMB] for s in range(3)]
-        if self.amp % 4 == 0 and all(src.stride(0) % 4 == 0 for src, _, _ in amp_streams):
+        self._gp_x_done = x_twin
+        if x_twin:
+            be.rms_normalize_multi_twin(amp_streams, self.amp, AMB, [self.amp_mean[s] for s in range(3)],
+                                        [self.amp_std[s] for s in range(3)], xd, [None, None, self._gp32.X])
+            gp_fork = self._mark() if self._gp_side else None
+        elif self.amp % 4 == 0 and all(src.stride(0) % 4 == 0 for src, _, _ in amp_streams):
             be.rms_normalize_multi(amp_streams, self.amp, AMB, [self.amp_mean[s] for s in range(3)],
                                    [self.amp_std[s] for s in range(3)], xd)
         else:
@@ -1063,7 +1102,7 @@
         be, c = self.be, self.cfg
         if apply and self._fused_apply and not self.truncate and not self.dyn_scale:
             self._build_apply_desc()
-            be.apply_multi(self._apply_desc, self._apply_items, self.dtype, self.opt_state, self.acc)
+            self._apply(self.opt_state)
         else:
             if self.has_disc:
                 for W, gW, coef, slot in self.l2_terms:
@@ -1149,7 +1188,7 @@
                 be.scaler_fold(self.scaler, self.scale_tab)
                 self._ar(self.scaler[:1])
             be.scaler_step(self.scaler, self.opt_state, self.opt_eff, g, scale_tab=self.scale_tab)
-            be.apply_multi(self._apply_desc, self._apply_items, self.dtype, self.opt_eff, self.acc)
+            self._apply(self.opt_eff)
         self._join_branch(br)
 
     @property
@@ -1290,30 +1329,46 @@
         nl, S = len(self.disc), self.gs
         s = math.sqrt(gp_coef * 2.0 / self.AMBg)
         bits = L.AUX_RELU_BITS
-        src, sidx, srm = amp_streams[2]
-        be.rms_normalize(src, self.amp, sidx, srm, AMB, self.amp_mean[2], self.amp_std[2], [g.X])
+        if not self._gp_x_done:
+            src, sidx, srm = amp_streams[2]
+            be.rms_normalize(src, self.amp, sidx, srm, AMB, self.amp_mean[2], self.amp_std[2], [g.X])
+        fuse = self._gp_fuse
+        with self._gp_mode() as ex:
+            if not self._gp_split:
+                self._gp_refresh()
+            top = self.disc[-1]
+            x = g.X
+            for l, d in enumerate(self.disc):
+                if fuse and l == nl - 1:
+                    self._nt(x, g.Ws[l], g.Gp[-1], AMB, d.n_pad, d.k_pad, bias=d.bs, act=L.ACT_RELU, mask_out=g.bits[l],
+                             seed=(self.disc_head.W[0].view(-1), s), twin=self.Gp[-1], **ex(12 if l == 0 else 6))
+                    break
+                self._nt(x, g.Ws[l], g.H[l], AMB, d.n_pad, d.k_pad, bias=d.bs, act=L.ACT_RELU, mask_out=g.bits[l],
+                           **ex(12 if l == 0 else 6))
+                x = g.H[l]
+            if not fuse:
+                be.gp_seed(g.H[-1], self.disc_head.W[0].view(-1), g.Gp[-1], AMB, top.N, scale=s)
+            for l in range(nl - 1, 0, -1):
+                d = self.disc[l]
+                self._nt(g.Gp[l], g.Wts[l], g.Gp[l - 1], AMB, d.k_pad, d.n_pad, aux=g.bits[l - 1], aux_mode=bits,
+                         **({'twin': self.Gp[l - 1]} if fuse else {}), **ex(12))
+            if not fuse:
+                d0 = self.disc[0]
+                self._nt(g.Gp[0], g.Wts[0], g.G0, AMB, d0.k_pad, d0.n_pad, alpha=S, alpha_dev=self._dS, **ex(12))
+
+    @contextlib.contextmanager
+    def _gp_mode(self):
+        be = self.be
         x3_prev = getattr(be, 'x3', None)
         mode = self.cfg.get('gp_f32')
         half = mode == 'x3' and x3_prev is not None and self.engine_opts['gp_split'] == 'f16'
         if mode == 'x3' and x3_prev is not None:
             be.x3 = 'f16' if half else True
-        ex = (lambda ea: {'x3_exps': (ea, 11)}) if half else (lambda ea: {})
-        for l, d in enumerate(self.disc):
-            be.refresh_shadow(d.W[0], g.Ws[l], g.Wts[l], d.split_src, d.split_dst, **({'x3_exp': 11} if half else {}))
-        x = g.X
-        for l, d in enumerate(self.disc):
-            self._nt(x, g.Ws[l], g.H[l], AMB, d.n_pad, d.k_pad, bias=d.bs, act=L.ACT_RELU, mask_out=g.bits[l],
-                       **ex(12 if l == 0 else 6))
-            x = g.H[l]
-        top = self.disc[-1]
-        be.gp_seed(g.H[-1], self.disc_head.W[0].view(-1), g.Gp[-1], AMB, top.N, scale=s)
-        for l in range(nl - 1, 0, -1):
-            d = self.disc[l]
-            self._nt(g.Gp[l], g.Wts[l], g.Gp[l - 1], AMB, d.k_pad, d.n_pad, aux=g.bits[l - 1], aux_mode=bits, **ex(12))
-        d0 = self.disc[0]
-        self._nt(g.Gp[0], g.Wts[0], g.G0, AMB, d0.k_pad, d0.n_pad, alpha=S, alpha_dev=self._dS, **ex(12))
-        if x3_prev is not None:
-            be.x3 = x3_prev
+        try:
+            yield (lambda ea: {'x3_exps': (ea, 11)}) if half else (lambda ea: {})
+        finally:
+            if x3_prev is not None:
+                be.x3 = x3_prev
 
     def _gp_f32(self, gp_coef):
         be, AMB, g = self.be, self.AMB, self._gp32
@@ -1328,6 +1383,17 @@
         if getattr(self, '_gp_value_pending', None) is not None:
             self._gp_value(*self._gp_value_pending)
             self._gp_value_pending = None
+        if self._gp_fuse:
+            with self._gp_mode() as ex:
+                self._nt(g.Gp[0], g.Wts[0], g.G0, AMB, d0.k_pad, d0.n_pad, alpha=S, alpha_dev=self._dS, twin=self.G0, store=False,
+                         sq=(self.acc, L.ACC_GP, 1.0 / (cg * S * S), self._dI2), **ex(12))
+        else:
+            self._gp_convert(cg)
+        self._gp_backward(s)
+
+    def _gp_convert(self, cg):
+        be, AMB, g = self.be, self.AMB, self._gp32
+        nl, S, d0 = len(self.disc), self.gs, self.disc[0]
         be.sqnorm(g.G0, AMB, d0.k_pad, self.acc, L.ACC_GP, scale=1.0 / (cg * S * S), dyn=self._dI2)
         if g.cast is None:
             code = {torch.bfloat16: L.BF16, torch.float16: L.F16}[self.dtype]
@@ -1335,6 +1401,12 @@
             rows = [[src.data_ptr(), src.stride(0), c, dst.data_ptr(), dst.stride(0), code] for src, c, dst in items]
             g.cast = (torch.tensor(rows, dtype=torch.int64, device=self.dev), items)
         be.gather_multi(g.cast[0], g.cast[1], None, (0, 0), AMB)
+
+    def _gp_backward(self, s):
+        be, AMB, g = self.be, self.AMB, self._gp32
+        Rd, nl, S = 3 * AMB, len(self.disc), self.gs
+        bits = L.AUX_RELU_BITS
+        d0 = self.disc[0]
         for l in range(nl - 1, 0, -1):
             self._dgrad(self.disc[l], self.dZd[l], self.dZd[l - 1], Rd, self.Hd[l - 1], self.disc[l - 1].act)
         self._nt(self.G0, d0.Ws, self.dGp[0], AMB, d0.n_pad, d0.k_pad, aux=g.bits[0], aux_mode=bits)
diff --git a/ase_amd/lib.py b/ase_amd/lib.py
--- a/ase_amd/lib.py
+++ b/ase_amd/lib.py
@@ -30,6 +30,8 @@
 
 SIGNATURES = {
     "ase_hip_gemm_nt": [_p, _i64, _p, _i64, _p, _i64, _p, _p, _i64, _i, _i, _p, _i, _p, _i64, _i, _i, _i, _i, _i, _i, _f, _p, _i, _p],
+    "ase_hip_gemm_nt_ex": [_p, _i64, _p, _i64, _p, _i64, _p, _p, _i64, _i, _i, _p, _i, _p, _i64, _i, _i, _i, _i, _i, _i, _f, _p, _i,
+                           _p, _i, _f, _p, _i64, _i, _p, _d, _p, _p],
     "ase_hip_gemm_tn": [_p, _i64, _p, _i64, _p, _p, _i, _i, _i, _i, _i, _i, _i, _i, _f, _p, _i, _p],
     "ase_hip_refresh_shadow": [_p, _i, _i, _p, _i64, _p, _i64, _i, _i, _i, _p],
     "ase_hip_refresh_shadow_multi": [_p, _i, _i, _p],
@@ -67,6 +69,7 @@
     "ase_hip_sample_latents": [_p, _i, _i, _p, _i64, _i, _p, _i64, _i, _p],
     "ase_hip_rms_moments_multi": [_p, _p, _p, _p, _p, _p, _i, _i, _i, _p, _p],
     "ase_hip_rms_normalize_multi": [_p, _p, _p, _p, _p, _p, _p, _p, _p, _i, _i, _i, _i, _p],
+    "ase_hip_rms_normalize_multi_v2": [_p, _p, _p, _p, _p, _p, _p, _p, _p, _p, _p, _i, _i, _i, _i, _p],
     "ase_hip_normalize_rows": [_p, _i64, _p, _i64, _i, _i, _p],
     "ase_hip_sample_actions": [_p, _i64, _p, _i64, _p, _p, _p, _p, _p, _p, _p, _i, _i, _i, _p],
     "ase_hip_debug_nt_profile": [_p],
@@ -82,6 +85,7 @@
     "ase_hip_clip_frames": [_p] * 6 + [_i] + [_p] * 4 + [_i, _i, _p, _p, _i] + [_p] * 7,
     "ase_hip_gemm_nt_kernel_id": [_i, _i, _i, _i],
     "ase_hip_apply_multi": [_p, _i, _p, _p, _i, _p],
+    "ase_hip_apply_multi_v2": [_p, _i, _p, _p, _p, _i, _p],
     "ase_hip_gemm_tn_grouped_plan": [_p, _i, _i, _p, _i, _p, _p, _i, _p],
     "ase_hip_prog_create": [_p],
     "ase_hip_prog_destroy": [_p],
diff --git a/include/ase_hip.h b/include/ase_hip.h
--- a/include/ase_hip.h
+++ b/include/ase_hip.h
@@ -32,6 +32,13 @@
                     float* colsum, int colsum_n, void* mask_out, int64_t ldmask, int M, int N, int K, int act,
                     int aux_mode, int out_f32, float alpha, float* alpha_dev, int dtype, void* stream);
 
+int ase_hip_gemm_nt_ex(const void* A, int64_t lda, const void* B, int64_t ldb, void* C, int64_t ldc,
+                       const float* bias, const void* aux, int64_t ldaux, int aux_split, int aux_delta,
+                       float* colsum, int colsum_n, void* mask_out, int64_t ldmask, int M, int N, int K, int act,
+                       int aux_mode, int out_f32, float alpha, float* alpha_dev, int dtype,
+                       const float* seed_w, int seed_n, float seed_scale, void* twin, int64_t ldtwin, int twin_dtype,
+                       double* sq_acc, double sq_scale, const float* sq_dyn, void* stream);
+
 int ase_hip_gemm_tn(const void* A, int64_t lda, const void* B, int64_t ldb, float* G, float* gbias,
                     int bias_rows, int M, int N, int K, int n_real, int k_real, int split_src, int split_dst,
                     float alpha, const float* alpha_dev, int dtype, void* stream);
@@ -59,6 +66,11 @@
                                 const int* remap_h, const int* remap_n, const float* const* means,
                                 const float* const* stds, void* const* outs, const int64_t* ld_outs, int n_streams, int D,
                                 int M, int dtype, void* stream);
+int ase_hip_rms_normalize_multi_v2(const float* const* srcs, const int64_t* ld_srcs, const int32_t* const* idxs,
+                                   const int* remap_h, const int* remap_n, const float* const* means,
+                                   const float* const* stds, void* const* outs, const int64_t* ld_outs,
+                                   float* const* outs32, const int64_t* ld_outs32, int n_streams, int D, int M, int dtype,
+                                   void* stream);
 
 int ase_hip_rms_finalize(double* state, int D, const double* sums, const int32_t* counts ,
                          int n_streams, float* mean_out, float* std_out, void* stream);
@@ -197,6 +209,8 @@
 
 int ase_hip_apply_multi(const int64_t* desc, int n_layers, const double* opt_state, double* acc, int dtype,
                         void* stream);
+int ase_hip_apply_multi_v2(const int64_t* desc, int n_layers, const int64_t* desc2, const double* opt_state, double* acc,
+                           int dtype, void* stream);
 
 
 int ase_hip_build_amp_obs(const float* root_pos, const float* root_rot, const float* root_vel,
```

Result: faster. 1.810 million samples/s (median of 6 runs) (+3.7%).
